# fraunhoferhhi/vvdec

Measured on NVIDIA H100. Metric: decoded frames/sec, 4K 10-bit Main10 RA, bit-exact YUV vs reference, higher is better.
Workload: dtype int16 samples / int32 accumulate

## Files before the change

include/vvdec_b200.h:

```cpp
#ifndef VVDEC_B200_H
#define VVDEC_B200_H
#include <stdint.h>
#include <stddef.h>

#ifdef __cplusplus
extern "C" {
#endif

#define B200_API __attribute__((visibility("default")))

enum {
  B200_OK            =  0,
  B200_ERR_CUDA      = -1,
  B200_ERR_PARAM     = -2,
  B200_ERR_NO_DEVICE = -3,
  B200_ERR_UNSUPPORTED = -4
};

B200_API const char* b200_last_error(void);
B200_API int         b200_device_count(void);
B200_API const char* b200_version(void);

enum { B200_TR_DCT2 = 0, B200_TR_DCT8 = 1, B200_TR_DST7 = 2 };
enum {
// ... 8 lines not shown
  uint16_t x, y;
  uint8_t  log2w, log2h;
  uint8_t  comp;
  uint8_t  flags;
  uint8_t  maxX, maxY;
  uint8_t  trType;
  uint8_t  lfnst;
  int8_t   ict;
  int8_t   rightShift;
  uint8_t  inBits;
  uint8_t  scale;
  uint32_t coefOff;
  uint32_t slOff;
  uint32_t rsv[2];
} b200_tu;

typedef struct b200_geom {
  int32_t width, height;
  int32_t chromaFormat;
  int32_t bitDepth;
  int32_t ctuSize;
  int32_t stride[3];
} b200_geom;

B200_API int b200_k1_residual(const b200_geom* g, int16_t* const planes[3],
                              const b200_tu* tus, size_t numTus,
                              const int16_t* coefs, size_t numCoefs,
                              const int32_t* scaling, size_t numScaling,
                              int mode);

typedef struct b200_lf_param {
  int8_t  qp[3];
  uint8_t bs;
  uint8_t sideMaxFiltLength;
  uint8_t flags;
} b200_lf_param;

typedef struct b200_lf_slice {
  int8_t  betaOffsetDiv2[3];
  int8_t  tcOffsetDiv2[3];
  uint8_t disable;
  uint8_t rsv;
} b200_lf_slice;

typedef struct b200_lf_seq {
  int32_t ladfEnabled, ladfNumIntervals;
  int32_t ladfQpOffset[5];
  int32_t ladfIntervalLowerBound[5];
} b200_lf_seq;

B200_API int b200_lf_deblock(const b200_geom* g, int16_t* const planes[3], const b200_lf_param* lfV, const b200_lf_param* lfH,
                             const uint8_t* ctuSlice, const b200_lf_slice* slices, int numSlices, const b200_lf_seq* seq, int dirs);

enum { B200_SAO_EO_0 = 0, B200_SAO_EO_90 = 1, B200_SAO_EO_135 = 2, B200_SAO_EO_45 = 3, B200_SAO_BO = 4, B200_SAO_OFF = 255 };
enum { B200_AVAIL_L = 1, B200_AVAIL_R = 2, B200_AVAIL_A = 4, B200_AVAIL_B = 8,
       B200_AVAIL_AL = 16, B200_AVAIL_AR = 32, B200_AVAIL_BL = 64, B200_AVAIL_BR = 128 };

typedef struct b200_sao_ctu {
  uint8_t type[3];
  uint8_t band[3];
  int8_t  offset[3][5];
  uint8_t avail;
  uint8_t rsv[2];
} b200_sao_ctu;

typedef struct b200_vb {
  int32_t numVer, numHor;
  int32_t posX[3], posY[3];
} b200_vb;

B200_API int b200_sao_picture(const b200_geom* g, const int16_t* const src[3], int16_t* const dst[3],
                              const b200_sao_ctu* ctus, const b200_vb* vb);

enum { B200_ALF_CLIP_TOP = 2, B200_ALF_CLIP_BOTTOM = 4, B200_ALF_CLIP_LEFT = 8, B200_ALF_CLIP_RIGHT = 16, B200_ALF_PAD_TL = 32, B200_ALF_PAD_BR = 64, B200_ALF_PAD_WIDE = 2 };
typedef struct b200_alf_ctu {
  uint8_t enable[3];
  uint8_t lumaSet;
  uint8_t chromaAlt[2];
  uint8_t ccIdx[2];
} b200_alf_ctu;

typedef struct b200_alf_tables {
  const int16_t* lumaCoeff;
  const int16_t* lumaClip;
  int32_t        numLumaSets;
  const int16_t* chromaCoeff;
  const int16_t* chromaClip;
  int32_t        numChromaAlts;
  const int16_t* ccCoeff[2];
  int32_t        numCc[2];
} b200_alf_tables;

B200_API int b200_alf_picture(const b200_geom* g, const int16_t* const src[3], int16_t* const dst[3],
                              const b200_alf_ctu* ctus, const b200_alf_tables* tabs);

enum {
  B200_PU_BDOF    = 1,
  B200_PU_DMVR    = 2,
  B200_PU_ALTHPEL = 4,
  B200_PU_AFFINE  = 8,
  B200_PU_AFFINE6 = 16,
  B200_PU_PROF0   = 32,
  B200_PU_PROF1   = 64,
  B200_PU_GEO     = 128
};

typedef struct b200_pu {
  uint16_t x, y;
  uint8_t  w, h;
  uint8_t  flags;
  int8_t   bcwW1;
  int8_t   refSlot[2];
  uint8_t  interDir;
  uint8_t  wpIdx;
  uint32_t dmvrOff;
  int32_t  mv[2][2];
  int32_t  cpmv[2][2][2];
} b200_pu;

typedef struct b200_wp {
  int16_t w0[3], w1[3];
  int16_t offset[3];
  uint8_t shift[3];
  uint8_t rsv[3];
} b200_wp;

B200_API int b200_mc_predict(const b200_geom* g, int16_t* const dst[3], const int16_t* const* refs, int numSlots,
                             const b200_pu* pus, size_t numPus, int32_t* dmvrMv, size_t numDmvr);
B200_API int b200_mc_predict_wp(const b200_geom* g, int16_t* const dst[3], const int16_t* const* refs, int numSlots,
                                const b200_pu* pus, size_t numPus, int32_t* dmvrMv, size_t numDmvr, const b200_wp* wp, int numWp);

enum { B200_INTRA_PLANAR = 0, B200_INTRA_DC = 1 , B200_INTRA_BDPCM_HOR = 67, B200_INTRA_BDPCM_VER = 68,
       B200_INTRA_MIP = 69 ,
       B200_INTRA_LM = 70, B200_INTRA_MDLM_L = 71, B200_INTRA_MDLM_T = 72  };
enum { B200_INTRA_FILTER_REF = 1, B200_INTRA_AVAIL_TL = 2, B200_INTRA_ADD_RESI = 4 ,
       B200_INTRA_LM_ABOVE = 8, B200_INTRA_LM_LEFT = 16 ,
       B200_INTRA_LM_COLLOCATED = 32 ,
       B200_INTRA_ISP = 64  };
typedef struct b200_intra_tu {
  uint16_t x, y;
  uint8_t  log2w, log2h;
  uint8_t  comp;
  uint8_t  mode;
  uint8_t  multiRefIdx;
  uint8_t  flags;
  uint8_t  numAbove;
  uint8_t  numLeft;
  uint8_t  mip;
  uint8_t  lmAbove, lmLeft;
  uint8_t  ciip;
} b200_intra_tu;
B200_API int b200_intra_predict(const b200_geom* g, int16_t* const planes[3], const b200_intra_tu* tus, size_t numTus);
B200_API int b200_intra_reconstruct(const b200_geom* g, int16_t* const planes[3], const int16_t* const resi[3], const b200_intra_tu* tus, size_t numTus);

typedef struct b200_ctx b200_ctx;

typedef struct b200_lmcs_vpdu { uint16_t x, y; uint8_t availLeft, availAbove; } b200_lmcs_vpdu;
typedef struct b200_lmcs {
  int32_t chromaAdj;
  int32_t minBinIdx, maxBinIdx;
  int32_t orgCW;
  int16_t reshapePivot[17];
  int16_t inputPivot[17];
  int16_t fwdScaleCoef[16];
  int32_t chromaAdjHelpLUT[16];
  const int16_t* invLUT;
  const b200_lmcs_vpdu* vpdus;
} b200_lmcs;

typedef struct b200_picture {
  int32_t dstSlot;
  int32_t flags;
  const int16_t* given[3];
  const b200_pu* pus; size_t numPus;
  size_t numDmvr;
  const b200_tu* tus; size_t numTus;
  const int16_t* coefs; size_t numCoefs;
  const int32_t* scaling; size_t numScaling;
  const b200_lf_param *lfV, *lfH;
  const uint8_t* ctuSlice; const b200_lf_slice* lfSlices; int32_t numLfSlices; const b200_lf_seq* lfSeq;
  const b200_sao_ctu* sao;
  const b200_vb* vb;
  const b200_alf_ctu* alf;
  const b200_alf_tables* alfTabs;
  const b200_wp* wp; int32_t numWp;
  const b200_lmcs* lmcs;
  const b200_intra_tu* intraTus;
  size_t numIntraTus;
} b200_picture;
enum { B200_PIC_DEBLOCK = 1, B200_PIC_SAO = 2, B200_PIC_ALF = 4, B200_PIC_LMCS = 8 };

B200_API int  b200_ctx_create(b200_ctx** ctx, const b200_geom* g, int numSlots, int numArenas, int device);
B200_API void b200_ctx_destroy(b200_ctx* ctx);
B200_API int  b200_ctx_load_slot(b200_ctx* ctx, int slot, const int16_t* const planes[3]);
B200_API int  b200_decompress_picture(b200_ctx* ctx, const b200_picture* pic);
B200_API int  b200_pic_upload(b200_ctx* ctx, const b200_picture* pic);
B200_API int  b200_pic_run(b200_ctx* ctx, int arena);
B200_API int  b200_wait_picture(b200_ctx* ctx, int arena, int32_t* dmvrMv, size_t numDmvr);
B200_API int  b200_get_frame(b200_ctx* ctx, int slot, int16_t* const planes[3]);
B200_API int  b200_ctx_load_slot_strided(b200_ctx* ctx, int slot, const int16_t* const planes[3], const ptrdiff_t strides[3]);
B200_API int  b200_get_frame_strided(b200_ctx* ctx, int slot, int16_t* const planes[3], const ptrdiff_t strides[3]);
B200_API int  b200_get_frame_async(b200_ctx* ctx, int slot, int16_t* const planes[3]);
B200_API int  b200_frame_wait(b200_ctx* ctx, int ticket);
B200_API int  b200_get_frame_device_async(b200_ctx* ctx, int slot, int16_t* const planesDev[3], void* cudaStream);
enum { B200_OUT_16 = 0, B200_OUT_PYUV = 1, B200_OUT_8 = 2 };
B200_API size_t b200_frame_bytes(const b200_geom* g, int fmt, int comp);
B200_API int  b200_get_frame_fmt_async(b200_ctx* ctx, int slot, int fmt, void* const planes[3]);
typedef struct b200_film_grain {
  const int8_t*   pattern;
  const uint8_t*  sLUT;
  const uint8_t*  pLUT;
  const uint32_t* lineSeeds;
  uint8_t         scaleShift;
  uint8_t         compPresent[3];
} b200_film_grain;
B200_API int  b200_get_frame_grain_async(b200_ctx* ctx, int slot, int fmt, void* const planes[3], const b200_film_grain* fg);
enum { B200_HASH_MD5 = 0, B200_HASH_CRC = 1, B200_HASH_CHECKSUM = 2 };
B200_API int  b200_frame_hash_async(b200_ctx* ctx, int slot, int method, uint8_t* digest);
B200_API int  b200_ctx_mark(b200_ctx* ctx, int which );
B200_API int  b200_ctx_elapsed_ms(b200_ctx* ctx, float* ms);
B200_API long long b200_ctx_kernel_launches(b200_ctx* ctx);
enum { B200_KF_MC_TILE = 0, B200_KF_MC_AFFINE, B200_KF_K1, B200_KF_LF_V, B200_KF_LF_H, B200_KF_SAO, B200_KF_ALF_LUMA, B200_KF_ALF_CHROMA,
       B200_KF_INTRA , B200_KF_LMCS , B200_KF_COUNT };
B200_API int  b200_ctx_set_profiling(b200_ctx* ctx, int on);
B200_API int  b200_ctx_get_kernel_ms(b200_ctx* ctx, float ms[8], int counts[8]);
B200_API int  b200_ctx_get_kernel_ms_n(b200_ctx* ctx, float* ms, int* counts, int n);
B200_API int  b200_host_register(void* ptr, size_t bytes);
B200_API int  b200_host_unregister(void* ptr);

#ifdef __cplusplus
}
#endif
#endif
```

vvdec_b200/bindings.py:

```python
import ctypes as C
import numpy as np
from . import abi

i16p = np.ctypeslib.ndpointer(np.int16, flags="C_CONTIGUOUS")
PLANES = C.POINTER(C.POINTER(C.c_int16))


def declare(lib):
    lib.b200_last_error.restype = C.c_char_p
    lib.b200_version.restype = C.c_char_p
    lib.b200_device_count.restype = C.c_int
    lib.b200_k1_residual.argtypes = [C.POINTER(abi.Geom), PLANES, C.c_void_p, C.c_size_t, C.c_void_p, C.c_size_t,
                                     C.c_void_p, C.c_size_t, C.c_int]
    lib.b200_k1_residual.restype = C.c_int


    lib.b200_lf_deblock.argtypes = [C.POINTER(abi.Geom), PLANES, C.c_void_p, C.c_void_p, C.c_void_p, C.c_void_p, C.c_int,
                                    C.c_void_p, C.c_int]
    lib.b200_lf_deblock.restype = C.c_int


    lib.b200_sao_picture.argtypes = [C.POINTER(abi.Geom), PLANES, PLANES, C.c_void_p, C.c_void_p]
    lib.b200_sao_picture.restype = C.c_int
    lib.b200_alf_picture.argtypes = [C.POINTER(abi.Geom), PLANES, PLANES, C.c_void_p, C.POINTER(abi.AlfTables)]
    lib.b200_alf_picture.restype = C.c_int


    lib.b200_mc_predict.argtypes = [C.POINTER(abi.Geom), PLANES, C.POINTER(C.c_void_p), C.c_int, C.c_void_p, C.c_size_t, C.c_void_p, C.c_size_t]
    lib.b200_mc_predict.restype = C.c_int
    lib.b200_mc_predict_wp.argtypes = [C.POINTER(abi.Geom), PLANES, C.POINTER(C.c_void_p), C.c_int, C.c_void_p, C.c_size_t, C.c_void_p, C.c_size_t, C.c_void_p, C.c_int]
    lib.b200_mc_predict_wp.restype = C.c_int


    CTX = C.c_void_p
    lib.b200_ctx_create.argtypes = [C.POINTER(CTX), C.POINTER(abi.Geom), C.c_int, C.c_int, C.c_int]
    lib.b200_ctx_destroy.argtypes = [CTX]; lib.b200_ctx_destroy.restype = None
    lib.b200_ctx_load_slot.argtypes = [CTX, C.c_int, PLANES]
    lib.b200_decompress_picture.argtypes = [CTX, C.POINTER(abi.Picture)]
    lib.b200_pic_upload.argtypes = [CTX, C.POINTER(abi.Picture)]
    lib.b200_pic_run.argtypes = [CTX, C.c_int]
    lib.b200_wait_picture.argtypes = [CTX, C.c_int, C.c_void_p, C.c_size_t]
    lib.b200_get_frame.argtypes = [CTX, C.c_int, PLANES]
    lib.b200_get_frame_async.argtypes = [CTX, C.c_int, PLANES]
    lib.b200_ctx_load_slot_strided.argtypes = [CTX, C.c_int, PLANES, C.POINTER(C.c_ssize_t)]
    lib.b200_get_frame_strided.argtypes = [CTX, C.c_int, PLANES, C.POINTER(C.c_ssize_t)]
    lib.b200_frame_wait.argtypes = [CTX, C.c_int]
    lib.b200_get_frame_device_async.argtypes = [CTX, C.c_int, C.POINTER(C.c_void_p), C.c_void_p]
    lib.b200_frame_bytes.argtypes = [C.POINTER(abi.Geom), C.c_int, C.c_int]; lib.b200_frame_bytes.restype = C.c_size_t
    lib.b200_get_frame_fmt_async.argtypes = [CTX, C.c_int, C.c_int, C.POINTER(C.c_void_p)]
    lib.b200_intra_predict.argtypes = [C.POINTER(abi.Geom), PLANES, C.c_void_p, C.c_size_t]
    lib.b200_intra_reconstruct.argtypes = [C.POINTER(abi.Geom), PLANES, PLANES, C.c_void_p, C.c_size_t]
    lib.b200_frame_hash_async.argtypes = [CTX, C.c_int, C.c_int, C.c_void_p]
    lib.b200_get_frame_grain_async.argtypes = [CTX, C.c_int, C.c_int, C.POINTER(C.c_void_p), C.POINTER(abi.FilmGrain)]
    lib.b200_ctx_mark.argtypes = [CTX, C.c_int]
    lib.b200_ctx_elapsed_ms.argtypes = [CTX, C.POINTER(C.c_float)]
    lib.b200_ctx_kernel_launches.argtypes = [CTX]; lib.b200_ctx_kernel_launches.restype = C.c_longlong
    lib.b200_ctx_set_profiling.argtypes = [CTX, C.c_int]
    lib.b200_ctx_get_kernel_ms.argtypes = [CTX, C.POINTER(C.c_float), C.POINTER(C.c_int)]
    lib.b200_ctx_get_kernel_ms_n.argtypes = [CTX, C.POINTER(C.c_float), C.POINTER(C.c_int), C.c_int]
    lib.b200_host_register.argtypes = [C.c_void_p, C.c_size_t]
    lib.b200_host_unregister.argtypes = [C.c_void_p]


EXPORTS = ["b200_ctx_create", "b200_ctx_destroy", "b200_ctx_load_slot", "b200_decompress_picture", "b200_pic_upload", "b200_pic_run",
           "b200_wait_picture", "b200_get_frame", "b200_ctx_load_slot_strided", "b200_get_frame_strided", "b200_get_frame_async", "b200_get_frame_device_async", "b200_frame_wait", "b200_frame_bytes", "b200_get_frame_fmt_async", "b200_frame_hash_async", "b200_intra_predict", "b200_intra_reconstruct", "b200_get_frame_grain_async", "b200_ctx_mark", "b200_ctx_elapsed_ms", "b200_ctx_kernel_launches", "b200_ctx_set_profiling", "b200_ctx_get_kernel_ms", "b200_ctx_get_kernel_ms_n", "b200_host_register", "b200_host_unregister",
           "b200_mc_predict", "b200_mc_predict_wp", "b200_last_error", "b200_version", "b200_device_count", "b200_k1_residual", "b200_lf_deblock",
           "b200_sao_picture", "b200_alf_picture"]
```

vvdec_b200/csrc/api.cu:

```cuda
#include "common.cuh"
#include <stdarg.h>
#include <string.h>
#include <mutex>

namespace b200 {

static thread_local char g_err[512] = "";

void set_error(const char* fmt, ...)
{
  va_list ap; va_start(ap, fmt);
  vsnprintf(g_err, sizeof(g_err), fmt, ap);
  va_end(ap);
}

int ensure_device()
{
  static std::once_flag once;
  static int status = 0;
  std::call_once(once, [] {
    int n = 0;
    if (cudaGetDeviceCount(&n) != cudaSuccess || n == 0) { set_error("no CUDA device: vvdec_b200 has no CPU fallback"); status = B200_ERR_NO_DEVICE; return; }
    int dev = 0; cudaGetDevice(&dev);
    cudaDeviceProp p; cudaGetDeviceProperties(&p, dev);
    if (p.major != 9 || p.minor != 0) { set_error("device %s is sm_%d%d; this library is built for sm_90a only", p.name, p.major, p.minor); status = B200_ERR_NO_DEVICE; }
  });
  if (status) set_error("no usable sm_90 device: vvdec_b200 has no CPU fallback");
  return status;
}

struct HostWrapScratch {
  DevBuf planes[3], tus, coefs, scaling, misc[8];
  cudaStream_t stream = nullptr;
  int init() { if (!stream) { B200_CUDA(cudaStreamCreateWithFlags(&stream, cudaStreamNonBlocking)); } return 0; }
};
static HostWrapScratch g_hw;
HostWrapScratch& host_scratch() { return g_hw; }

static int upload_planes(const b200_geom* g, int16_t* const planes[3], DevPlanes& dp, cudaStream_t s)
{
  const int nPlanes = g->chromaFormat ? 3 : 1;
  for (int c = 0; c < nPlanes; c++) {
    const int ph = c ? g->height >> 1 : g->height;
    const size_t bytes = (size_t)g->stride[c] * ph * sizeof(int16_t);
    if (int rc = g_hw.planes[c].reserve(bytes)) return rc;
    dp.p[c] = g_hw.planes[c].as<int16_t>(); dp.stride[c] = g->stride[c];
    B200_CUDA(cudaMemcpyAsync(dp.p[c], planes[c], bytes, cudaMemcpyHostToDevice, s));
  }
  return 0;
}
static int download_planes(const b200_geom* g, int16_t* const planes[3], const DevPlanes& dp, cudaStream_t s)
{
  const int nPlanes = g->chromaFormat ? 3 : 1;
  for (int c = 0; c < nPlanes; c++) {
    const int ph = c ? g->height >> 1 : g->height;
    B200_CUDA(cudaMemcpyAsync(planes[c], dp.p[c], (size_t)g->stride[c] * ph * sizeof(int16_t), cudaMemcpyDeviceToHost, s));
  }
  return 0;
}

int num_sms()
{
  static int cache[64] = {0};
  int dev = 0; cudaGetDevice(&dev);
  if (dev < 0 || dev >= 64) dev = 0;
  if (!cache[dev]) { int n = 0; if (cudaDeviceGetAttribute(&n, cudaDevAttrMultiProcessorCount, dev) != cudaSuccess || n <= 0) n = 132; cache[dev] = n; }
  return cache[dev];
}

int fetch_list_meta(const int* metaDev, int* cnt, int nLists, const char* what, cudaStream_t s)
{
  int h[LM_INTS];
  B200_CUDA(cudaMemcpyAsync(h, metaDev, sizeof(h), cudaMemcpyDeviceToHost, s));
  B200_CUDA(cudaStreamSynchronize(s));
  for (int i = 0; i < nLists; i++) cnt[i] = h[LM_CNT + i];
  B200_CHECK(!(h[LM_ERR] & 1), "%s: invalid record (reference slots, block size or flag combination)", what);
  B200_CHECK(!(h[LM_ERR] & 2), "%s: more tiles than the picture can hold (overlapping PUs?)", what);
  return 0;
}

}

using namespace b200;

extern "C" {

B200_API const char* b200_last_error(void) { return g_err; }
B200_API const char* b200_version(void) { return "vvdec_b200 0.1 (sm_90a)"; }
B200_API int b200_device_count(void) { int n = 0; return cudaGetDeviceCount(&n) == cudaSuccess ? n : 0; }

B200_API int b200_k1_residual(const b200_geom* g, int16_t* const planes[3], const b200_tu* tus, size_t numTus,
                              const int16_t* coefs, size_t numCoefs, const int32_t* scaling, size_t numScaling, int mode)
{
  B200_CHECK(g && planes && (tus || !numTus), "b200_k1_residual: null argument");
  B200_CHECK(g->bitDepth >= 8 && g->bitDepth <= 12, "b200_k1_residual: bit depth %d unsupported", g->bitDepth);
  if (int rc = ensure_device()) return rc;
  if (int rc = g_hw.init()) return rc;
  cudaStream_t s = g_hw.stream;
  K1Launch L; L.geom = *g; L.numTus = numTus; L.mode = mode;
  if (int rc = upload_planes(g, planes, L.planes, s)) return rc;
  if (int rc = g_hw.tus.reserve(numTus * sizeof(b200_tu))) return rc;
  if (int rc = g_hw.coefs.reserve(numCoefs * sizeof(int16_t) + 16)) return rc;
  if (int rc = g_hw.scaling.reserve(numScaling * sizeof(int32_t) + 16)) return rc;
  if (int rc = g_hw.misc[4].reserve(numTus * 4 + LM_INTS * sizeof(int) + 256)) return rc;
  if (numTus) B200_CUDA(cudaMemcpyAsync(g_hw.tus.p, tus, numTus * sizeof(b200_tu), cudaMemcpyHostToDevice, s));
  if (numCoefs) B200_CUDA(cudaMemcpyAsync(g_hw.coefs.p, coefs, numCoefs * sizeof(int16_t), cudaMemcpyHostToDevice, s));
  if (numScaling) B200_CUDA(cudaMemcpyAsync(g_hw.scaling.p, scaling, numScaling * sizeof(int32_t), cudaMemcpyHostToDevice, s));
  L.tus = g_hw.tus.as<b200_tu>(); L.coefs = g_hw.coefs.as<int16_t>(); L.scaling = g_hw.scaling.as<int32_t>();
  int* meta = g_hw.misc[4].as<int>(); uint32_t* idx = reinterpret_cast<uint32_t*>(meta + LM_INTS);
  if (int rc = launch_tu_bucket(L.tus, numTus, idx, meta, *g, numCoefs, numScaling, s)) return rc;
  L.idx = idx; L.meta = meta;
  if (int rc = fetch_list_meta(meta, L.cnt, K1_LISTS, "b200_k1_residual", s)) return rc;
  StreamSet ss(s);
  if (int rc = launch_k1_residual(L, ss)) return rc;
  if (int rc = download_planes(g, planes, L.planes, s)) return rc;
  B200_CUDA(cudaStreamSynchronize(s));
  return 0;
}

B200_API int b200_lf_deblock(const b200_geom* g, int16_t* const planes[3], const b200_lf_param* lfV, const b200_lf_param* lfH,
                             const uint8_t* ctuSlice, const b200_lf_slice* slices, int numSlices, const b200_lf_seq* seq, int dirs)
{
  B200_CHECK(g && planes && lfV && lfH && slices, "b200_lf_deblock: null argument");
  B200_CHECK(numSlices >= 1 && numSlices <= 64, "b200_lf_deblock: numSlices %d out of range 1..64", numSlices);
  B200_CHECK(g->ctuSize == 32 || g->ctuSize == 64 || g->ctuSize == 128, "b200_lf_deblock: CTU size %d", g->ctuSize);
  if (int rc = ensure_device()) return rc;
  if (int rc = g_hw.init()) return rc;
  cudaStream_t s = g_hw.stream;
  LfLaunch L; L.geom = *g; L.dirs = dirs;
  memset(&L.slices, 0, sizeof(L.slices)); memcpy(L.slices.s, slices, numSlices * sizeof(b200_lf_slice));
  if (seq) L.seq = *seq; else memset(&L.seq, 0, sizeof(L.seq));
  if (int rc = upload_planes(g, planes, L.planes, s)) return rc;
  const size_t n4 = (size_t)((g->width + 3) >> 2) * ((g->height + 3) >> 2);
  const size_t nCtu = (size_t)((g->width + g->ctuSize - 1) / g->ctuSize) * ((g->height + g->ctuSize - 1) / g->ctuSize);
  if (int rc = g_hw.misc[0].reserve(n4 * sizeof(b200_lf_param))) return rc;
  if (int rc = g_hw.misc[1].reserve(n4 * sizeof(b200_lf_param))) return rc;
  if (int rc = g_hw.misc[2].reserve(nCtu)) return rc;
  B200_CUDA(cudaMemcpyAsync(g_hw.misc[0].p, lfV, n4 * sizeof(b200_lf_param), cudaMemcpyHostToDevice, s));
  B200_CUDA(cudaMemcpyAsync(g_hw.misc[1].p, lfH, n4 * sizeof(b200_lf_param), cudaMemcpyHostToDevice, s));
  if (ctuSlice) B200_CUDA(cudaMemcpyAsync(g_hw.misc[2].p, ctuSlice, nCtu, cudaMemcpyHostToDevice, s));
  L.lfV = g_hw.misc[0].as<b200_lf_param>(); L.lfH = g_hw.misc[1].as<b200_lf_param>();
  L.ctuSlice = ctuSlice ? g_hw.misc[2].as<uint8_t>() : nullptr;
  if (int rc = launch_lf_deblock(L, s)) return rc;
  if (int rc = download_planes(g, planes, L.planes, s)) return rc;
  B200_CUDA(cudaStreamSynchronize(s));
  return 0;
}

static int upload_src_alloc_dst(const b200_geom* g, const int16_t* const src[3], DevPlanes& ds, DevPlanes& dd, cudaStream_t s)
{
  const int nPlanes = g->chromaFormat ? 3 : 1;
  for (int c = 0; c < nPlanes; c++) {
    const int ph = c ? g->height >> 1 : g->height;
    const size_t bytes = (size_t)g->stride[c] * ph * sizeof(int16_t);
    if (int rc = g_hw.planes[c].reserve(bytes)) return rc;
    if (int rc = g_hw.misc[3 + c].reserve(bytes)) return rc;
    ds.p[c] = g_hw.planes[c].as<int16_t>(); dd.p[c] = g_hw.misc[3 + c].as<int16_t>(); ds.stride[c] = dd.stride[c] = g->stride[c];
    B200_CUDA(cudaMemcpyAsync(ds.p[c], src[c], bytes, cudaMemcpyHostToDevice, s));
  }
  return 0;
}

B200_API int b200_sao_picture(const b200_geom* g, const int16_t* const src[3], int16_t* const dst[3], const b200_sao_ctu* ctus, const b200_vb* vb)
{
  B200_CHECK(g && src && dst && ctus, "b200_sao_picture: null argument");
  B200_CHECK((g->width & 7) == 0 && (g->stride[0] & 3) == 0 && (!g->chromaFormat || (g->stride[1] & 3) == 0), "b200_sao_picture: width must be a multiple of 8, strides of 4");
  if (int rc = ensure_device()) return rc;
  if (int rc = g_hw.init()) return rc;
  cudaStream_t s = g_hw.stream;
  SaoLaunch L; L.geom = *g;
  if (vb) L.vb = *vb; else memset(&L.vb, 0, sizeof(L.vb));
  if (int rc = upload_src_alloc_dst(g, src, L.src, L.dst, s)) return rc;
  const size_t nCtu = (size_t)((g->width + g->ctuSize - 1) / g->ctuSize) * ((g->height + g->ctuSize - 1) / g->ctuSize);
  if (int rc = g_hw.misc[0].reserve(nCtu * sizeof(b200_sao_ctu))) return rc;
  B200_CUDA(cudaMemcpyAsync(g_hw.misc[0].p, ctus, nCtu * sizeof(b200_sao_ctu), cudaMemcpyHostToDevice, s));
  L.ctus = g_hw.misc[0].as<b200_sao_ctu>();
  if (int rc = launch_sao(L, s)) return rc;
  if (int rc = download_planes(g, dst, L.dst, s)) return rc;
  B200_CUDA(cudaStreamSynchronize(s));
  return 0;
}

B200_API int b200_intra_reconstruct(const b200_geom* g, int16_t* const planes[3], const int16_t* const resi[3], const b200_intra_tu* tus, size_t numTus)
{
  B200_CHECK(g && planes && (tus || !numTus), "b200_intra_reconstruct: null argument");
  B200_CHECK(g->bitDepth >= 8 && g->bitDepth <= 12, "b200_intra_reconstruct: bit depth %d unsupported", g->bitDepth);
  const int nPl = g->chromaFormat ? 3 : 1;
  for (size_t i = 0; i < numTus; i++) {
    const b200_intra_tu& t = tus[i];
    const int w = 1 << t.log2w, h = 1 << t.log2h, pw = t.comp ? g->width >> 1 : g->width, ph = t.comp ? g->height >> 1 : g->height, unit = t.comp ? 2 : 4;
    const bool inCtu = intra_record_in_ctu(t, intra_ctu_log2(*g));
    if (t.flags & B200_INTRA_ISP) {
      B200_CHECK(intra_isp_record_ok(t, i ? &tus[i - 1] : nullptr, g->width, g->height), "b200_intra_reconstruct: record %zu: bad ISP region", i);
      B200_CHECK(inCtu, "b200_intra_reconstruct: intra block record %zu is not inside one CTU", i);
      continue;
    }
    B200_CHECK(t.comp < nPl && t.log2w >= 2 && t.log2w <= 6 && t.log2h >= 1 && t.log2h <= 6 && t.x + w <= pw && t.y + h <= ph && !(t.x % unit) && !(t.y % unit),
               "b200_intra_reconstruct: record %zu: bad geometry", i);
    B200_CHECK(inCtu, "b200_intra_reconstruct: intra block record %zu is not inside one CTU", i);
    B200_CHECK(t.mode <= B200_INTRA_MDLM_T && t.multiRefIdx <= 2 && (!t.multiRefIdx || !t.comp), "b200_intra_reconstruct: record %zu: bad mode / reference line", i);
    B200_CHECK(!t.ciip || (t.ciip <= 3 && t.mode == B200_INTRA_PLANAR), "b200_intra_reconstruct: record %zu: bad CIIP block", i);
    B200_CHECK(t.mode < B200_INTRA_LM || (t.comp && t.log2w <= 5 && t.log2h <= 5 && t.lmAbove <= w && t.lmLeft <= h && (!(t.flags & B200_INTRA_LM_ABOVE) || t.y >= 2) && (!(t.flags & B200_INTRA_LM_LEFT) || t.x >= 2)
                                        && t.x + std::max(w, 2 * (int)t.lmAbove) <= pw && t.y + std::max(h, 2 * (int)t.lmLeft) <= ph), "b200_intra_reconstruct: record %zu: bad CCLM block", i);
    B200_CHECK(t.mode != B200_INTRA_MIP || (!t.comp && !t.multiRefIdx && (t.mip & 0x7f) < ((w == 4 && h == 4) ? 16 : (w == 4 || h == 4 || (w == 8 && h == 8)) ? 8 : 6)),
               "b200_intra_reconstruct: record %zu: bad MIP mode", i);
    B200_CHECK(t.numAbove <= 2 * w / unit && t.numLeft <= 2 * h / unit && (!t.numAbove || t.y > t.multiRefIdx) && (!t.numLeft || t.x > t.multiRefIdx)
               && (!(t.flags & B200_INTRA_AVAIL_TL) || (t.x > t.multiRefIdx && t.y > t.multiRefIdx)) && t.x + (int)t.numAbove * unit <= pw && t.y + (int)t.numLeft * unit <= ph,
               "b200_intra_reconstruct: record %zu: availability outside the picture", i);
  }
  if (int rc = ensure_device()) return rc;
  if (int rc = g_hw.init()) return rc;
  cudaStream_t s = g_hw.stream;
  IntraLaunch L; L.geom = *g; L.numTus = numTus;
  if (int rc = upload_planes(g, planes, L.planes, s)) return rc;
  for (int c = 0; c < 3; c++) {
    L.resi[c] = nullptr; L.owner[c] = nullptr; L.ownerStride[c] = 0; L.ownerBytes[c] = 0;
    if (c >= nPl) continue;
    const int pw = c ? g->width >> 1 : g->width, ph = c ? g->height >> 1 : g->height, unit = c ? 2 : 4;
    L.ownerStride[c] = (pw + unit - 1) / unit; L.ownerBytes[c] = (size_t)L.ownerStride[c] * ((ph + unit - 1) / unit) * sizeof(int);
    if (int rc = g_hw.misc[c].reserve(L.ownerBytes[c])) return rc;
    L.owner[c] = g_hw.misc[c].as<int>();
    if (resi && resi[c]) {
      const size_t bytes = (size_t)g->stride[c] * ph * sizeof(int16_t);
      if (int rc = g_hw.misc[3 + c].reserve(bytes)) return rc;
      B200_CUDA(cudaMemcpyAsync(g_hw.misc[3 + c].p, resi[c], bytes, cudaMemcpyHostToDevice, s));
      L.resi[c] = g_hw.misc[3 + c].as<int16_t>();
    }
  }
  if (int rc = g_hw.tus.reserve(numTus * sizeof(b200_intra_tu) + 16)) return rc;
  if (int rc = g_hw.misc[6].reserve((numTus + 2) * sizeof(int))) return rc;
  if (int rc = g_hw.misc[7].reserve(intra_order_ints(*g, numTus) * sizeof(int))) return rc;
  if (numTus) B200_CUDA(cudaMemcpyAsync(g_hw.tus.p, tus, numTus * sizeof(b200_intra_tu), cudaMemcpyHostToDevice, s));
  L.tus = g_hw.tus.as<b200_intra_tu>(); L.sync = g_hw.misc[6].as<int>(); L.order = g_hw.misc[7].as<int>();
  if (int rc = launch_intra(L, s)) return rc;
  int err = 0;
  if (numTus) B200_CUDA(cudaMemcpyAsync(&err, L.sync + numTus + 1, sizeof(int), cudaMemcpyDeviceToHost, s));
  if (int rc = download_planes(g, planes, L.planes, s)) return rc;
  B200_CUDA(cudaStreamSynchronize(s));
  B200_CHECK(!(err & INTRA_ERR_CTU_BLOCKS), "b200_intra_reconstruct: a CTU holds more than %d intra block records (overlapping records?)", INTRA_MAX_CTU_BLOCKS);
  B200_CHECK(!err, "b200_intra_reconstruct: a block waited for a neighbour that never finished, or the blocks of a CTU are not contiguous (list not in decoding order?)");
  return 0;
}

B200_API int b200_intra_predict(const b200_geom* g, int16_t* const planes[3], const b200_intra_tu* tus, size_t numTus)
{
  return b200_intra_reconstruct(g, planes, nullptr, tus, numTus);
}

B200_API int b200_alf_picture(const b200_geom* g, const int16_t* const src[3], int16_t* const dst[3], const b200_alf_ctu* ctus, const b200_alf_tables* T)
{
  B200_CHECK(g && src && dst && ctus && T, "b200_alf_picture: null argument");
  B200_CHECK((g->width & 7) == 0 && (g->stride[0] & 3) == 0 && (!g->chromaFormat || (g->stride[1] & 3) == 0), "b200_alf_picture: width must be a multiple of 8, strides of 4");
  B200_CHECK(T->numLumaSets >= 16 && T->numLumaSets <= 24, "b200_alf_picture: numLumaSets %d", T->numLumaSets);
  if (int rc = ensure_device()) return rc;
  if (int rc = g_hw.init()) return rc;
  cudaStream_t s = g_hw.stream;
  AlfLaunch L; L.geom = *g;
  if (int rc = upload_src_alloc_dst(g, src, L.src, L.dst, s)) return rc;
  const size_t nCtu = (size_t)((g->width + g->ctuSize - 1) / g->ctuSize) * ((g->height + g->ctuSize - 1) / g->ctuSize);
  const size_t nL = (size_t)T->numLumaSets * 1300, nC = (size_t)T->numChromaAlts * 7, n0 = (size_t)T->numCc[0] * 7, n1 = (size_t)T->numCc[1] * 7;
  const size_t tabElems = 2 * nL + 2 * nC + n0 + n1 + 8;
  if (int rc = g_hw.misc[0].reserve(nCtu * sizeof(b200_alf_ctu))) return rc;
  if (int rc = g_hw.misc[1].reserve(tabElems * sizeof(int16_t))) return rc;
  B200_CUDA(cudaMemcpyAsync(g_hw.misc[0].p, ctus, nCtu * sizeof(b200_alf_ctu), cudaMemcpyHostToDevice, s));
  int16_t* d = g_hw.misc[1].as<int16_t>();
  auto up = [&](const int16_t* h, size_t n, const int16_t*& out) -> int {
    out = d; if (n) B200_CUDA(cudaMemcpyAsync(d, h, n * sizeof(int16_t), cudaMemcpyHostToDevice, s)); d += n; return 0; };
  if (int rc = up(T->lumaCoeff, nL, L.lumaCoeff)) return rc;
  if (int rc = up(T->lumaClip, nL, L.lumaClip)) return rc;
  if (int rc = up(T->chromaCoeff, nC, L.chromaCoeff)) return rc;
  if (int rc = up(T->chromaClip, nC, L.chromaClip)) return rc;
  if (int rc = up(T->ccCoeff[0], n0, L.cc[0])) return rc;
  if (int rc = up(T->ccCoeff[1], n1, L.cc[1])) return rc;
  L.ctus = g_hw.misc[0].as<b200_alf_ctu>();
  StreamSet ss(s);
  if (int rc = launch_alf(L, ss)) return rc;
  if (int rc = download_planes(g, dst, L.dst, s)) return rc;
  B200_CUDA(cudaStreamSynchronize(s));
  return 0;
}

B200_API int b200_mc_predict(const b200_geom* g, int16_t* const dst[3], const int16_t* const* refs, int numSlots,
                             const b200_pu* pus, size_t numPus, int32_t* dmvrMv, size_t numDmvr)
{
  return b200_mc_predict_wp(g, dst, refs, numSlots, pus, numPus, dmvrMv, numDmvr, nullptr, 0);
}

B200_API int b200_mc_predict_wp(const b200_geom* g, int16_t* const dst[3], const int16_t* const* refs, int numSlots,
                                const b200_pu* pus, size_t numPus, int32_t* dmvrMv, size_t numDmvr, const b200_wp* wp, int numWp)
{
  B200_CHECK(g && dst && refs && (pus || !numPus), "b200_mc_predict: null argument");
  B200_CHECK(numSlots >= 1 && numSlots <= B200_MAX_SLOTS, "b200_mc_predict: numSlots %d", numSlots);
  B200_CHECK(numPus < (1u << 26), "b200_mc_predict: too many PUs");
  for (size_t i = 0; i < numPus; i++) {
    B200_CHECK(pus[i].refSlot[0] < numSlots && pus[i].refSlot[1] < numSlots && (pus[i].refSlot[0] >= 0 || pus[i].refSlot[1] >= 0), "b200_mc_predict: PU %zu has invalid reference slots", i);
    B200_CHECK(!((pus[i].flags & B200_PU_DMVR) && g->bitDepth > 10), "b200_mc_predict: DMVR needs bit depth <= 10 (as the reference)");
  }
  if (int rc = ensure_device()) return rc;
  if (int rc = g_hw.init()) return rc;
  cudaStream_t s = g_hw.stream;
  McLaunch L; L.geom = *g;
  if (int rc = upload_planes(g, dst, L.dst, s)) return rc;
  const int nPlanes = g->chromaFormat ? 3 : 1;
  size_t planeBytes[3] = {0, 0, 0}, total = 0;
  for (int c = 0; c < nPlanes; c++) { planeBytes[c] = (((size_t)g->stride[c] * (c ? g->height >> 1 : g->height) * 2) + 255) & ~(size_t)255; total += planeBytes[c]; }
  if (int rc = g_hw.misc[3].reserve(total * numSlots)) return rc;
  std::vector<const int16_t*> ptrs(numSlots * 3, nullptr);
  char* base = g_hw.misc[3].as<char>();
  for (int sl = 0; sl < numSlots; sl++) {
    size_t off = 0;
    for (int c = 0; c < nPlanes; c++) {
      char* d = base + (size_t)sl * total + off;
      B200_CUDA(cudaMemcpyAsync(d, refs[sl * 3 + c], (size_t)g->stride[c] * (c ? g->height >> 1 : g->height) * 2, cudaMemcpyHostToDevice, s));
      ptrs[sl * 3 + c] = reinterpret_cast<const int16_t*>(d); off += planeBytes[c];
    }
  }
  const size_t capTiles = mc_tile_capacity(*g, numPus);
  if (int rc = g_hw.misc[5].reserve(numPus * sizeof(b200_pu) + 64)) return rc;
  if (int rc = g_hw.misc[6].reserve(capTiles * 4 + LM_INTS * sizeof(int) + 256)) return rc;
  if (int rc = g_hw.misc[7].reserve(numDmvr * 8 + 64)) return rc;
  if (numPus) B200_CUDA(cudaMemcpyAsync(g_hw.misc[5].p, pus, numPus * sizeof(b200_pu), cudaMemcpyHostToDevice, s));
  int* meta = g_hw.misc[6].as<int>(); uint32_t* tiles = reinterpret_cast<uint32_t*>(meta + LM_INTS);
  if (int rc = launch_mc_bucket(g_hw.misc[5].as<b200_pu>(), numPus, tiles, capTiles, meta, *g, numSlots, wp ? numWp : 0, numDmvr, s)) return rc;
  L.tiles = tiles; L.meta = meta;
  if (wp && numWp > 0) {
    B200_CHECK(numWp <= 255, "b200_mc_predict_wp: at most 255 weighted-prediction entries");
    if (int rc = g_hw.misc[2].reserve(numWp * sizeof(b200_wp))) return rc;
    B200_CUDA(cudaMemcpyAsync(g_hw.misc[2].p, wp, numWp * sizeof(b200_wp), cudaMemcpyHostToDevice, s));
    L.wp = g_hw.misc[2].as<b200_wp>();
  }
  if (int rc = fetch_list_meta(meta, L.cnt, MC_LISTS, "b200_mc_predict", s)) return rc;
  B200_CUDA(cudaMemsetAsync(g_hw.misc[7].p, 0, numDmvr * 8 + 64, s));
  memset(L.refs, 0, sizeof(L.refs)); for (size_t i = 0; i < ptrs.size(); i++) L.refs[i] = ptrs[i];
  for (int c = 0; c < 3; c++) L.refStride[c] = g->stride[c];
  L.pus = g_hw.misc[5].as<b200_pu>(); L.dmvrMv = dmvrMv ? g_hw.misc[7].as<int32_t>() : nullptr;
  StreamSet ss(s);
  if (int rc = launch_mc(L, ss)) return rc;
  if (int rc = download_planes(g, dst, L.dst, s)) return rc;
  if (dmvrMv && numDmvr) B200_CUDA(cudaMemcpyAsync(dmvrMv, g_hw.misc[7].p, numDmvr * 8, cudaMemcpyDeviceToHost, s));
  B200_CUDA(cudaStreamSynchronize(s));
  return 0;
}

}
```

vvdec_b200/csrc/common.cuh:

```cuda
#pragma once
#include <cuda_runtime.h>
#include <stdint.h>
#include <stdio.h>
#include <string>
#include <vector>
#include <algorithm>
#include "../../include/vvdec_b200.h"

namespace b200 {

void set_error(const char* fmt, ...);

#define B200_CUDA(call)                                                                         \
  do {                                                                                          \
    cudaError_t e_ = (call);                                                                    \
    if (e_ != cudaSuccess) {                                                                    \
      b200::set_error("%s:%d %s -> %s", __FILE__, __LINE__, #call, cudaGetErrorString(e_));     \
      (void)cudaGetLastError();                                                                 \
      return B200_ERR_CUDA;                                                                     \
    }                                                                                           \
  } while (0)

#define B200_CHECK(cond, ...)                                    \
  do {                                                           \
    if (!(cond)) { b200::set_error(__VA_ARGS__); return B200_ERR_PARAM; } \
  } while (0)

__device__ __forceinline__ int clip3(int lo, int hi, int v) { return min(max(v, lo), hi); }
__device__ __forceinline__ int clip16(int v) { return min(max(v, -32768), 32767); }

__device__ __forceinline__ int lmcs_fwd(const b200_lmcs* __restrict__ L, int log2OrgCW, int v, int pmax)
{
  const int idx = v >> log2OrgCW;
  return clip3(0, pmax, (int)__ldg(&L->reshapePivot[idx]) + (((int)__ldg(&L->fwdScaleCoef[idx]) * (v - (int)__ldg(&L->inputPivot[idx])) + (1 << 10)) >> 11));
}
__device__ __forceinline__ int lmcs_scale(int r, int scale, int maxAbs)
{
  r = clip3(-maxAbs - 1, maxAbs, r);
  const int a = abs(r), v = (a * scale + (1 << 10)) >> 11;
  return clip16(r >= 0 ? v : -v);
}

struct DevBuf {
  void*  p   = nullptr;
  size_t cap = 0;
  int reserve(size_t bytes) {
    if (bytes <= cap) return 0;
    if (p) cudaFree(p);
    p = nullptr; cap = 0;
    size_t want = bytes + (bytes >> 2) + 256;
    cudaError_t e = cudaMalloc(&p, want);
    if (e != cudaSuccess) { set_error("cudaMalloc(%zu) -> %s", want, cudaGetErrorString(e)); return B200_ERR_CUDA; }
    cap = want;
    return 0;
  }
  template <class T> T* as() const { return reinterpret_cast<T*>(p); }
  ~DevBuf() { if (p) cudaFree(p); }
};

struct DevPlanes {
  int16_t* p[3] = {nullptr, nullptr, nullptr};
  int      stride[3] = {0, 0, 0};
};

struct KProf { virtual void begin(int family, cudaStream_t s) = 0; virtual void end(int family, cudaStream_t s) = 0; virtual ~KProf() {} };

struct StreamSet {
  cudaStream_t main = nullptr; cudaStream_t aux[4] = {nullptr, nullptr, nullptr, nullptr}; int nAux = 0;
  cudaEvent_t forkEv = nullptr, joinEv[4] = {nullptr, nullptr, nullptr, nullptr};
  bool used[4] = {false, false, false, false};
  StreamSet() {}
  explicit StreamSet(cudaStream_t s) : main(s) {}
  cudaStream_t pick(int i) {
    if (nAux == 0) return main;
    const int k = i % (nAux + 1);
    if (k == nAux) return main;
    if (!used[k]) { cudaEventRecord(forkEv, main); cudaStreamWaitEvent(aux[k], forkEv, 0); used[k] = true; }
    return aux[k];
  }
  void join() { for (int k = 0; k < nAux; k++) if (used[k]) { cudaEventRecord(joinEv[k], aux[k]); cudaStreamWaitEvent(main, joinEv[k], 0); used[k] = false; } }
};

constexpr int MC_LISTS = 17;
constexpr int K1_LISTS = 4;
constexpr int LM_CNT = 0, LM_OFF = 32, LM_CUR = 64, LM_DONE = 96, LM_ERR = 97, LM_INTS = 128;
int launch_mc_bucket(const b200_pu* pus, size_t numPus, uint32_t* tiles, size_t capTiles, int* meta, const b200_geom& g, int numSlots, int numWp, size_t numDmvr, cudaStream_t s);
int launch_tu_bucket(const b200_tu* tus, size_t numTus, uint32_t* idx, int* meta, const b200_geom& g, size_t numCoefs, size_t numScaling, cudaStream_t s);
struct CtuLimits { int numLumaSets, numChromaAlts, numCc[2], numLfSlices; };
int launch_ctu_validate(const b200_sao_ctu* sao, const b200_alf_ctu* alf, const uint8_t* ctuSlice, int nCtu, const CtuLimits& lim, int* meta, cudaStream_t s);
size_t mc_tile_capacity(const b200_geom& g, size_t numPus);
int num_sms();
int fetch_list_meta(const int* metaDev, int* cnt, int nLists, const char* what, cudaStream_t s);

struct K1Launch {
  b200_geom      geom;
  DevPlanes      planes;
  const b200_tu* tus;
  size_t         numTus;
  const uint32_t* idx;
  const int*     meta;
  int            cnt[K1_LISTS];
  const int16_t* coefs;
  const int32_t* scaling;
  int            mode;
  int            compSel = 0;
  const int*     vpduScale = nullptr;
  int16_t*       resi[3] = {nullptr, nullptr, nullptr};
};
int launch_k1_residual(const K1Launch& L, StreamSet& ss, KProf* prof = nullptr);

struct LfSliceTab { b200_lf_slice s[64]; };
struct LfLaunch {
  b200_geom geom; DevPlanes planes;
  const b200_lf_param *lfV, *lfH;
  const uint8_t* ctuSlice;
  LfSliceTab slices; b200_lf_seq seq; int dirs;
};
int launch_lf_deblock(const LfLaunch& L, cudaStream_t s, KProf* prof = nullptr);

struct SaoLaunch { b200_geom geom; DevPlanes src, dst; const b200_sao_ctu* ctus; b200_vb vb; };
int launch_sao(const SaoLaunch& L, cudaStream_t s, KProf* prof = nullptr);

struct AlfLaunch {
  b200_geom geom; DevPlanes src, dst; const b200_alf_ctu* ctus;
  const int16_t *lumaCoeff, *lumaClip, *chromaCoeff, *chromaClip, *cc[2];
};
int launch_alf(const AlfLaunch& L, StreamSet& ss, KProf* prof = nullptr);

constexpr int B200_MAX_SLOTS = 32;
struct McLaunch {
  b200_geom geom; DevPlanes dst;
  const int16_t* refs[B200_MAX_SLOTS * 3];
  int refStride[3];
  const b200_pu* pus;
  const uint32_t* tiles;
  const int* meta;
  int cnt[MC_LISTS];
  int32_t* dmvrMv;
  const b200_wp* wp = nullptr;
  const b200_lmcs* lmcs = nullptr;
  const void* tmaps = nullptr; uint8_t tmapBuf[B200_MAX_SLOTS] = {};
};
int make_mc_tensor_maps(const b200_geom& g, int16_t* const* bufPlanes , int nBufs, void** out);
int launch_mc(const McLaunch& L, StreamSet& ss, KProf* prof = nullptr);
int mc_launch_count(const McLaunch& L);
int k1_launch_count(const K1Launch& L);

struct LmcsLaunch { b200_geom geom; DevPlanes planes; const b200_lmcs* lmcs; const b200_lmcs_vpdu* vpdus; const int16_t* invLut; int* scale; };
int launch_lmcs_vpdu(const LmcsLaunch& L, cudaStream_t s);
int launch_lmcs_inv(const LmcsLaunch& L, cudaStream_t s);

int launch_pack(const DevPlanes& src, const b200_geom& g, int fmt, uint8_t* const dst[3], cudaStream_t s);

struct IntraLaunch { b200_geom geom; DevPlanes planes; const int16_t* resi[3]; const b200_intra_tu* tus; size_t numTus; int* owner[3]; int ownerStride[3]; size_t ownerBytes[3]; int* sync;
                     int* order = nullptr;
                     int compSel = 0;
                   };
inline size_t intra_order_ints(const b200_geom& g, size_t numTus) { return numTus + 8 + 3 * (size_t)((g.width + g.ctuSize - 1) / g.ctuSize) * ((g.height + g.ctuSize - 1) / g.ctuSize); }
inline int intra_ctu_log2(const b200_geom& g) { return g.ctuSize == 128 ? 7 : g.ctuSize == 64 ? 6 : 5; }
__host__ __device__ inline bool intra_record_in_ctu(const b200_intra_tu& t, int ctuLog2)
{
  const int cl = ctuLog2 - (t.comp ? 1 : 0);
  return (t.x >> cl) == ((t.x + (1 << t.log2w) - 1) >> cl) && (t.y >> cl) == ((t.y + (1 << t.log2h) - 1) >> cl);
}
__host__ __device__ inline bool intra_isp_record_ok(const b200_intra_tu& t, const b200_intra_tu* prev, int W, int H)
{
  const int sp = t.mip & 3, k = (t.mip >> 2) & 3, l2n = (t.mip >> 4) & 3, nReg = 1 << l2n, rw = 1 << t.log2w, rh = 1 << t.log2h;
  if (t.comp || t.mode > 66 || t.multiRefIdx || (sp != 1 && sp != 2) || l2n > 2 || (l2n == 0 && (sp != 2 || rw != 4))  || k >= nReg || (t.mip >> 6) || t.log2w < 2 || t.log2w > 6 || t.log2h > 6) return false;
  const int cw = sp == 2 ? rw * nReg : rw, ch = sp == 1 ? rh * nReg : rh, cx = t.x - (sp == 2 ? k * rw : 0), cy = t.y - (sp == 1 ? k * rh : 0);
  if (cw > 64 || ch > 64 || ch < 4 || cw * ch < 32 || cx < 0 || cy < 0 || (cx & 3) || (cy & 3) || cx + cw > W || cy + ch > H) return false;
  if (t.numAbove > 2 * cw / 4 || t.numLeft > 2 * ch / 4 || (t.numAbove && !cy) || (t.numLeft && !cx) || ((t.flags & B200_INTRA_AVAIL_TL) && (!cx || !cy))
      || cx + (int)t.numAbove * 4 > W || cy + (int)t.numLeft * 4 > H || (t.lmLeft && !cx) || (t.lmAbove && !cy)) return false;
  if (k) {
    if (!prev || !(prev->flags & B200_INTRA_ISP) || prev->mip != (uint8_t)(t.mip - 4) || prev->log2w != t.log2w || prev->log2h != t.log2h || prev->mode != t.mode
        || prev->x != t.x - (sp == 2 ? rw : 0) || prev->y != t.y - (sp == 1 ? rh : 0)) return false;
  }
  return true;
}
int launch_intra(const IntraLaunch& L, cudaStream_t s);
int launch_intra_ciip_clear(const b200_intra_tu* tus, size_t numTus, int16_t* const resi[3], const int stride[3], cudaStream_t s);
int launch_intra_validate(const b200_intra_tu* tus, size_t numTus, const b200_geom& g, int* meta, cudaStream_t s);
constexpr int INTRA_ERR_ORDER = 2, INTRA_ERR_CTU_BLOCKS = 4, INTRA_MAX_CTU_BLOCKS = 3072;
int launch_film_grain(const DevPlanes& src, const DevPlanes& dst, const b200_geom& g, const int8_t* pattern, const uint8_t* sLUT, const uint8_t* pLUT,
                      const uint32_t* lineSeeds, uint32_t* seeds, int scaleShift, const uint8_t present[3], cudaStream_t s);
int launch_hash(const DevPlanes& src, const b200_geom& g, int method, uint32_t* acc, uint8_t* digest, cudaStream_t s);

int ensure_device();

}
```

vvdec_b200/csrc/k6_intra.cu:

```cuda
#include "common.cuh"
#include <stdlib.h>
#include <string.h>
#define VVC_TABLE_QUAL static __device__ const __align__(16)
#include "vvc_tables.h"

namespace b200 {

constexpr int IT_THREADS = 128;
constexpr int IT_REF = 2 * 64 + 8;
constexpr int IT_ORG = 72;
constexpr int IT_ARR = IT_ORG + 2 * 64 + 80;

__constant__ int cAng[32] = {0, 1, 2, 3, 4, 6, 8, 10, 12, 14, 16, 18, 20, 23, 26, 29, 32, 35, 39, 45, 51, 57, 64, 73, 86, 102, 128, 171, 256, 341, 512, 1024};
__constant__ int cInvAng[32] = {0, 16384, 8192, 5461, 4096, 2731, 2048, 1638, 1365, 1170, 1024, 910, 819, 712, 630, 565,
                                512, 468, 420, 364, 321, 287, 256, 224, 191, 161, 128, 96, 64, 48, 32, 16};
__constant__ int cIntraFilterThr[8] = {24, 24, 24, 14, 2, 0, 0, 0};

struct IntraParams {
  int16_t* planes[3]; const int16_t* resi[3]; int stride[3]; int W, H, bitDepth;
  const b200_intra_tu* tus; int numTus;
  int* owner[3]; int ownerStride[3];
  int* done; int* ticket; int* err;
  const int* perm;
  int* ctuCnt; int* ctuFirst; int* ctuBase; int ctuLog2, ctusW, ctusH;
  int compSel;
};

__device__ __forceinline__ int wide_angle(int w, int h, int mode)
{
  if (mode > 1 && mode <= 66) {
    const int d = abs((31 - __clz(w)) - (31 - __clz(h)));
    const int shift = (int)((0x0F0E0C0A0600ull >> (8 * d)) & 0xff);
    if (w > h && mode < 2 + shift) mode += 65;
    else if (h > w && mode > 66 - shift) mode -= 65;
  }
  return mode;
}

__global__ void __launch_bounds__(256) intra_owner_kernel(const IntraParams P)
{
  const int i = blockIdx.x;
  const b200_intra_tu t = P.tus[i];
  const int c = t.comp, unit = c ? 2 : 4, uw = max(1, (1 << t.log2w) / unit), uh = max(1, (1 << t.log2h) / unit);
  for (int k = threadIdx.x; k < uw * uh; k += blockDim.x) atomicMax(&P.owner[c][(t.y / unit + k / uw) * P.ownerStride[c] + t.x / unit + k % uw], i);
}

__device__ __forceinline__ int intra_ctu_of(const IntraParams& P, const b200_intra_tu& t)
{
  const int sh = t.comp ? 1 : 0;
  return (((int)t.y << sh) >> P.ctuLog2) * P.ctusW + (((int)t.x << sh) >> P.ctuLog2);
}
__global__ void __launch_bounds__(256) intra_ctu_count_kernel(const IntraParams P)
{
  const int i = blockIdx.x * 256 + threadIdx.x;
  if (i >= P.numTus) return;
  const int c = intra_ctu_of(P, P.tus[i]);
  atomicAdd(&P.ctuCnt[c], 1); atomicMin(&P.ctuFirst[c], i);
}
__global__ void intra_ctu_base_kernel(const IntraParams P)
{
  int run = 0;
  for (int d = 0; d < P.ctusW + 2 * P.ctusH; d++)
    for (int y = 0; y < P.ctusH; y++) { const int x = d - 2 * y; if (x >= 0 && x < P.ctusW) { P.ctuBase[y * P.ctusW + x] = run; run += P.ctuCnt[y * P.ctusW + x]; } }
}
__global__ void __launch_bounds__(256) intra_perm_kernel(const IntraParams P, int* perm)
{
  const int i = blockIdx.x * 256 + threadIdx.x;
  if (i >= P.numTus) return;
  const int c = intra_ctu_of(P, P.tus[i]), r = i - P.ctuFirst[c];
  if (r >= P.ctuCnt[c]) { atomicOr(P.err, 2); return; }
  perm[P.ctuBase[c] + r] = i;
}

__device__ __forceinline__ int pix(const int16_t* __restrict__ plane, int stride, int x, int y) { return __ldcg(plane + (size_t)y * stride + x); }

#define ISP_GEOMETRY \
    const bool isp = t.flags & B200_INTRA_ISP; \
    int bx = x0, by = y0, bw = w, bh = h, ispK = 0, ispSplit = 0, resiMask = 0xff, l2tu = 16; \
    if (isp) { \
      ispSplit = t.mip & 3; ispK = (t.mip >> 2) & 3; const int nReg_ = 1 << ((t.mip >> 4) & 3); \
      if (ispSplit == 1) { bh = h * nReg_; by = y0 - ispK * h; } else { bw = w * nReg_; bx = x0 - ispK * w; } \
      int tuW_ = w; if (ispSplit == 2 && (bw == 4 || (bw == 8 && bh > 4))) tuW_ = max(bw >> 2, bh < 16 ? 16 / bh : 1);       \
      l2tu = 31 - __clz(tuW_); resiMask = t.ciip; \
    } \
    const int topLen = isp ? bw + w : 2 * w, sideLen = isp ? bh + h : 2 * h;

#define ISP_REFERENCE_LAMBDAS \
    auto refT = [&](int j) -> int {                               \
      if (n == 0) return 1 << (P.bitDepth - 1); \
      if (n == totalUnits) return PIXR(bx - 1 - mrl + j, by - 1 - mrl); \
      if (j <= mrl) {                                             \
        if (numLeft > 0) return availTL ? PIXR(bx - 1 - mrl + j, by - 1 - mrl) : PIXR(bx - 1 - mrl, by); \
        return PIXR(bx, by - 1 - mrl); \
      } \
      if (numAbove) return PIXR(bx + min(j - 1 - mrl, aboveLen - 1), by - 1 - mrl); \
      return availTL ? PIXR(bx - 1, by - 1 - mrl) : PIXR(bx - 1 - mrl, by);       \
    }; \
    auto refL = [&](int i) -> int {                               \
      if (n == 0) return 1 << (P.bitDepth - 1); \
      if (n == totalUnits) return PIXR(bx - 1 - mrl, by - 1 - mrl + i); \
      if (numLeft > 0) { \
        if (i <= mrl) return availTL ? PIXR(bx - 1 - mrl, by - 1 - mrl + i) : PIXR(bx - 1 - mrl, by); \
        return PIXR(bx - 1 - mrl, by + min(i - 1 - mrl, leftLen - 1)); \
      } \
      return PIXR(bx, by - 1 - mrl); \
    }; \
    auto regT = [&](int j) -> int { \
      if (!ispK) return refT(j); \
      if (ispSplit == 1) return j == 0 ? (t.lmLeft ? refL(y0 - by) : PIXR(x0, y0 - 1)) : PIXR(x0 + min(j - 1, w - 1), y0 - 1); \
      return t.lmAbove ? refT(x0 - bx + j) : PIXR(x0 - 1, y0); \
    }; \
    auto regL = [&](int i) -> int { \
      if (!ispK) return refL(i); \
      if (ispSplit == 1) return t.lmLeft ? refL(y0 - by + i) : PIXR(x0, y0 - 1); \
      return PIXR(x0 - 1, y0 + min(i - 1, h - 1)); \
    };

__global__ void __launch_bounds__(IT_THREADS, 12) intra_kernel(const IntraParams P)
{
  __shared__ int16_t sT[2][IT_REF], sL[2][IT_REF];
  __shared__ int16_t sM[IT_ARR], sS[IT_ARR];
  __shared__ int sTicket, sSum;
  __shared__ int16_t sLm[32 * 32], sLmTop[64], sLmLeft[64];
  __shared__ int sLmPar[3];
  const int tid = threadIdx.x;
  for (;;) {
    __syncthreads();
    if (tid == 0) { sTicket = atomicAdd(P.ticket, 1); sSum = 0; }
    __syncthreads();
    if (sTicket >= P.numTus) return;
    if (P.perm && (*(volatile int*)P.err & 2)) return;
    const int me = P.perm ? P.perm[sTicket] : sTicket;
    const b200_intra_tu t = P.tus[me];
    if ((P.compSel == 1 && t.comp != 0) || (P.compSel == 2 && t.comp == 0)) continue;
    const int c = t.comp, w = 1 << t.log2w, h = 1 << t.log2h, mrl = c ? 0 : t.multiRefIdx, unit = c ? 2 : 4;
    const int x0 = t.x, y0 = t.y, ps = P.stride[c], pmax = (1 << P.bitDepth) - 1;
    const int16_t* plane = P.planes[c];
    const int availTL = (t.flags & B200_INTRA_AVAIL_TL) ? 1 : 0, numAbove = t.numAbove, numLeft = t.numLeft;
    ISP_GEOMETRY

    {
      if (ispK && tid == 0) {
        const volatile int* d = P.done + me - 1; const volatile int* e = P.err; int spins = 0;
        while (*d == 0) { __nanosleep(64); if (*e || ++spins > (1 << 22)) { atomicOr(P.err, 1); break; } }
      }
      for (int dep = tid; dep < 96; dep += IT_THREADS) {
      int ux = -1, uy = -1;
      if (dep == 0) { if (availTL) { ux = bx - 1; uy = by - 1; } }
      else if (dep <= numAbove) { ux = bx + (dep - 1) * unit; uy = by - 1; }
      else if (dep - 64 >= 0 && dep - 64 < numLeft) { ux = bx - 1; uy = by + (dep - 64) * unit; }
      if (ux >= 0 && uy >= 0) {
        const int o = P.owner[c][(uy / unit) * P.ownerStride[c] + ux / unit];
        if (o >= 0 && o < me) {
          const volatile int* d = P.done + o;
          int spins = 0;
          const volatile int* e = P.err;
          while (*d == 0) { __nanosleep(64); if (*e || ++spins > (1 << 22)) { atomicOr(P.err, 1); break; } }
        }
      }
      }
      if (t.mode >= B200_INTRA_LM) {
        const bool aCu = t.flags & B200_INTRA_LM_ABOVE, lCu = t.flags & B200_INTRA_LM_LEFT;
        const int nA = max(w, aCu ? (t.mode == B200_INTRA_MDLM_T ? 2 * t.lmAbove : w) : 0), nL = max(h, lCu ? (t.mode == B200_INTRA_MDLM_L ? 2 * t.lmLeft : h) : 0);
        const int ux0 = max(0, (2 * x0 - (lCu ? 4 : 0)) >> 2), ux1 = min(P.W - 1, 2 * x0 + 2 * nA - 1) >> 2;
        const int uy0 = max(0, (2 * y0 - (aCu ? 4 : 0)) >> 2), uy1 = min(P.H - 1, 2 * y0 + 2 * nL - 1) >> 2;
        const int uw = ux1 - ux0 + 1, nU = uw * (uy1 - uy0 + 1);
        for (int u = tid; u < nU; u += IT_THREADS) {
          const int o = P.owner[0][(uy0 + u / uw) * P.ownerStride[0] + ux0 + u % uw];
          if (o >= 0 && o < me) {
            const volatile int* d = P.done + o; const volatile int* e = P.err;
            int spins = 0;
            while (*d == 0) { __nanosleep(64); if (*e || ++spins > (1 << 22)) { atomicOr(P.err, 1); break; } }
          }
        }
      }
      __threadfence();
    }
    __syncthreads();

    const int predSize = 2 * bw, predHSize = 2 * bh;
    const int totalUnits = (predSize + unit - 1) / unit + (predHSize + unit - 1) / unit + 1, n = availTL + numAbove + numLeft;
    const int aboveLen = min(numAbove * unit, predSize), leftLen = min(numLeft * unit, predHSize);
    int16_t *T = sT[0], *L = sL[0];
#define PIXR(x, y) pix(plane, ps, (x), (y))
    ISP_REFERENCE_LAMBDAS
    for (int j = tid; j <= topLen + mrl; j += IT_THREADS) T[j] = (int16_t)regT(j);
    for (int i = tid + 1; i <= sideLen + mrl; i += IT_THREADS) L[i] = (int16_t)regL(i);
#undef PIXR
    __syncthreads();
    if (tid == 0) L[0] = T[0];
    __syncthreads();
    if ((t.flags & B200_INTRA_FILTER_REF) && !c && !mrl) {
      int16_t *FT = sT[1], *FL = sL[1];
      for (int j = tid; j <= predSize; j += IT_THREADS)
        FT[j] = j == 0 ? (int16_t)((L[1] + 2 * T[0] + T[1] + 2) >> 2) : j == predSize ? T[j] : (int16_t)((T[j + 1] + 2 * T[j] + T[j - 1] + 2) >> 2);
      for (int i = tid + 1; i <= predHSize; i += IT_THREADS)
        FL[i] = i == predHSize ? L[i] : (int16_t)((L[i + 1] + 2 * L[i] + L[i - 1] + 2) >> 2);
      __syncthreads();
      if (tid == 0) FL[0] = FT[0];
      T = FT; L = FL;
      __syncthreads();
    }

    const int mode = t.mode;
    const bool doPDPC = w >= 4 && h >= 4 && mrl == 0;
    int16_t* dst = P.planes[c] + (size_t)y0 * ps + x0;
    const int16_t* rs = (P.resi[c] && (t.flags & B200_INTRA_ADD_RESI)) ? P.resi[c] + (size_t)y0 * ps + x0 : nullptr;
    const int ciipW = isp ? 0 : t.ciip;
#define IT_STORE(x, y, v) do { int v_ = (v); int16_t* d_ = dst + (size_t)(y) * ps + (x); if (ciipW) v_ = ((4 - ciipW) * (int)*d_ + ciipW * v_ + 2) >> 2; \
                               if (rs && ((resiMask >> ((x) >> l2tu)) & 1)) v_ = clip3(0, pmax, v_ + rs[(size_t)(y) * ps + (x)]); *d_ = (int16_t)v_; } while (0)

    if (mode == B200_INTRA_PLANAR || mode == B200_INTRA_DC) {
      int dc = 0;
      if (mode == B200_INTRA_DC) {
        int part = 0;
        for (int i = tid; i < w + h; i += IT_THREADS) {
          if (i < w) { if (w >= h) part += T[mrl + 1 + i]; }
          else if (w <= h) part += L[mrl + 1 + i - w];
        }
        for (int o = 16; o; o >>= 1) part += __shfl_down_sync(0xffffffffu, part, o);
        if ((tid & 31) == 0) atomicAdd(&sSum, part);
        __syncthreads();
        const int denom = w == h ? w << 1 : max(w, h);
        dc = (sSum + (denom >> 1)) >> (31 - __clz(denom));
      }
      const int l2w = t.log2w, l2h = t.log2h, scale = (l2w - 2 + l2h - 2 + 2) >> 2;
      const int bl = L[h + 1], tr = T[w + 1];
      for (int k = tid; k < w * h; k += IT_THREADS) {
        const int y = k >> l2w, x = k & (w - 1);
        int v;
        if (mode == B200_INTRA_PLANAR) {
          const int hor = (L[y + 1] << l2w) + (x + 1) * (tr - L[y + 1]), vert = (T[x + 1] << l2h) + (y + 1) * (bl - T[x + 1]);
          v = ((hor << l2h) + (vert << l2w) + (1 << (l2w + l2h))) >> (1 + l2w + l2h);
        } else v = dc;
        v = (int16_t)v;
        if (doPDPC) {
          const int wT = 32 >> min(31, (y << 1) >> scale), wL = 32 >> min(31, (x << 1) >> scale);
          v = (int16_t)(v + ((wL * (L[y + 1] - v) + wT * (T[x + 1] - v) + 32) >> 6));
        }
        IT_STORE(x, y, v);
      }
    } else if (mode >= B200_INTRA_LM) {
      const bool aCu = t.flags & B200_INTRA_LM_ABOVE, lCu = t.flags & B200_INTRA_LM_LEFT, colloc = t.flags & B200_INTRA_LM_COLLOCATED;
      const int ls = P.stride[0];
      const int16_t* rec = P.planes[0] + (size_t)(2 * y0) * ls + 2 * x0;
      const bool firstRowOfCtu = ((2 * y0) & ((1 << P.ctuLog2) - 1)) == 0;
      const int nTop = aCu ? (mode == B200_INTRA_MDLM_T ? 2 * t.lmAbove : w) : 0, nLeft = lCu ? (mode == B200_INTRA_MDLM_L ? 2 * t.lmLeft : h) : 0;
#define LUMA(p_, o_) ((int)__ldcg((p_) + (o_)))
      for (int k = tid; k < nTop + nLeft + w * h; k += IT_THREADS) {
        if (k < nTop) {
          const int i = k, m = (i == 0 && !lCu) ? 0 : 1;
          int v;
          if (firstRowOfCtu) { const int16_t* p = rec - ls; v = (LUMA(p, 2 * i) * 2 + LUMA(p, 2 * i - m) + LUMA(p, 2 * i + 1) + 2) >> 2; }
          else if (colloc) { const int16_t* p = rec - 2 * ls; v = (LUMA(p, 2 * i - ls) + LUMA(p, 2 * i) * 4 + LUMA(p, 2 * i - m) + LUMA(p, 2 * i + 1) + LUMA(p, 2 * i + ls) + 4) >> 3; }
          else { const int16_t* p = rec - 2 * ls; v = (LUMA(p, 2 * i) * 2 + LUMA(p, 2 * i - m) + LUMA(p, 2 * i + 1) + LUMA(p, 2 * i + ls) * 2 + LUMA(p, 2 * i - m + ls) + LUMA(p, 2 * i + 1 + ls) + 4) >> 3; }
          sLmTop[i] = (int16_t)v;
        } else if (k < nTop + nLeft) {
          const int j = k - nTop; const int16_t* p = rec - 3 + (size_t)(2 * j) * ls;
          int v;
          if (colloc) v = (LUMA(p, 1 - ((j == 0 && !aCu) ? 0 : ls)) + LUMA(p, 1) * 4 + LUMA(p, 0) + LUMA(p, 2) + LUMA(p, 1 + ls) + 4) >> 3;
          else v = (LUMA(p, 1) * 2 + LUMA(p, 0) + LUMA(p, 2) + LUMA(p, 1 + ls) * 2 + LUMA(p, ls) + LUMA(p, 2 + ls) + 4) >> 3;
          sLmLeft[j] = (int16_t)v;
        } else {
          const int q = k - nTop - nLeft, j = q >> t.log2w, i = q & (w - 1), m = (i == 0 && !lCu) ? 0 : 1;
          const int16_t* p = rec + (size_t)(2 * j) * ls;
          int v;
          if (colloc) { const int up = (j == 0 && !aCu) ? 0 : ls; v = (LUMA(p, 2 * i - up) + LUMA(p, 2 * i) * 4 + LUMA(p, 2 * i - m) + LUMA(p, 2 * i + 1) + LUMA(p, 2 * i + ls) + 4) >> 3; }
          else v = (LUMA(p, 2 * i) * 2 + LUMA(p, 2 * i + 1) + LUMA(p, 2 * i - m) + LUMA(p, 2 * i + ls) * 2 + LUMA(p, 2 * i + 1 + ls) + LUMA(p, 2 * i - m + ls) + 4) >> 3;
          sLm[q] = (int16_t)v;
        }
      }
#undef LUMA
      __syncthreads();
      if (tid == 0) {
        const int tuWU = w >> 1, tuHU = h >> 1;
        bool aboveAvail = false, leftAvail = false; int topNum = 0, leftNum = 0;
        if (mode == B200_INTRA_MDLM_T) { aboveAvail = t.lmAbove >= tuWU; topNum = 2 * t.lmAbove; }
        else if (mode == B200_INTRA_MDLM_L) { leftAvail = t.lmLeft >= tuHU; leftNum = 2 * t.lmLeft; }
        else { aboveAvail = aCu; leftAvail = lCu; topNum = w; leftNum = h; }
        const int aboveIs4 = leftAvail ? 0 : 1, leftIs4 = aboveAvail ? 0 : 1;
        const int start0 = topNum >> (2 + aboveIs4), step0 = max(1, topNum >> (1 + aboveIs4)), start1 = leftNum >> (2 + leftIs4), step1 = max(1, leftNum >> (1 + leftIs4));
        int sl[4] = {0, 0, 0, 0}, sc[4] = {0, 0, 0, 0}, cntT = 0, cntL = 0;
        if (aboveAvail) { cntT = min(topNum, (1 + aboveIs4) << 1); for (int k = 0, pos = start0; k < cntT; k++, pos += step0) { sl[k] = sLmTop[pos]; sc[k] = T[1 + pos]; } }
        if (leftAvail) { cntL = min(leftNum, (1 + leftIs4) << 1); for (int k = 0, pos = start1; k < cntL; k++, pos += step1) { sl[k + cntT] = sLmLeft[pos]; sc[k + cntT] = L[1 + pos]; } }
        if (cntT + cntL == 2) { sl[3] = sl[0]; sc[3] = sc[0]; sl[2] = sl[1]; sc[2] = sc[1]; sl[0] = sl[1]; sc[0] = sc[1]; sl[1] = sl[3]; sc[1] = sc[3]; }
        int mn0 = 0, mn1 = 2, mx0 = 1, mx1 = 3, tt;
        if (sl[mn0] > sl[mn1]) { tt = mn0; mn0 = mn1; mn1 = tt; }
        if (sl[mx0] > sl[mx1]) { tt = mx0; mx0 = mx1; mx1 = tt; }
        if (sl[mn0] > sl[mx1]) { tt = mn0; mn0 = mx0; mx0 = tt; tt = mn1; mn1 = mx1; mx1 = tt; }
        if (sl[mn1] > sl[mx0]) { tt = mn1; mn1 = mx0; mx0 = tt; }
        const int minL = (sl[mn0] + sl[mn1] + 1) >> 1, minC = (sc[mn0] + sc[mn1] + 1) >> 1, maxL = (sl[mx0] + sl[mx1] + 1) >> 1, maxC = (sc[mx0] + sc[mx1] + 1) >> 1;
        int a = 0, b = 1 << (P.bitDepth - 1), shift = 0;
        if (leftAvail || aboveAvail) {
          const int diff = maxL - minL;
          if (diff > 0) {
            const int diffC = maxC - minC;
            int x = 31 - __clz(diff);
            const int normDiff = (diff << 4 >> x) & 15;
            const int v = (int)((0x0765544332211110ull >> (4 * (15 - normDiff))) & 15) | 8;
            x += normDiff != 0;
            const int y = diffC == 0 ? 0 : (31 - __clz(abs(diffC))) + 1, add = 1 << y >> 1;
            a = (diffC * v + add) >> y; shift = 3 + x - y;
            if (shift < 1) { shift = 1; a = a == 0 ? 0 : a < 0 ? -15 : 15; }
            b = minC - ((a * minL) >> shift);
          } else { a = 0; b = minC; shift = 0; }
        }
        sLmPar[0] = a; sLmPar[1] = b; sLmPar[2] = shift;
      }
      __syncthreads();
      const int a = sLmPar[0], b = sLmPar[1], shift = sLmPar[2];
      for (int k = tid; k < w * h; k += IT_THREADS) { const int y = k >> t.log2w, x = k & (w - 1); IT_STORE(x, y, clip3(0, pmax, ((a * sLm[k]) >> shift) + b)); }
    } else if (mode == B200_INTRA_MIP) {
      const int sizeId = (w == 4 && h == 4) ? 0 : (w == 4 || h == 4 || (w == 8 && h == 8)) ? 1 : 2;
      const int bdry = sizeId == 0 ? 2 : 4, red = sizeId < 2 ? 4 : 8, upH = w / red, upV = h / red, inSize = 2 * bdry;
      const int modeIdx = t.mip & 0x7f; const bool transpose = t.mip >> 7;
      int16_t* in = sS;
      if (tid < inSize) {
        const bool fromLeft = (tid >= bdry) != transpose; const int d = tid % bdry, len = fromLeft ? h : w;
        const int16_t* full = (fromLeft ? L : T) + 1;
        int v;
        if (bdry < len) { const int f = len / bdry; int sum = 0; for (int j = 0; j < f; j++) sum += full[d * f + j]; v = (sum + (f >> 1)) >> (31 - __clz(f)); }
        else v = full[d];
        in[tid] = (int16_t)v;
      }
      __syncthreads();
      const int inputOffset = in[0];
      __syncthreads();
      if (tid < inSize) in[tid] = (int16_t)(tid == 0 ? (sizeId < 2 ? (1 << (P.bitDepth - 1)) - inputOffset : 0) : in[tid] - inputOffset);
      __syncthreads();
      if (tid < red * red) {
        const int redSize = sizeId == 2, stride = inSize - redSize;
        const uint8_t* wgt = (sizeId == 0 ? kMip4x4 + modeIdx * 64 : sizeId == 1 ? kMip8x8 + modeIdx * 128 : kMip16x16 + modeIdx * 448) + tid * stride;
        int sum = 0, acc = 0;
        for (int i = 0; i < inSize; i++) sum += in[i];
        for (int i = redSize; i < inSize; i++) acc += in[i] * wgt[i - redSize];
        const int v = clip3(0, pmax, ((acc + 32 - 32 * sum) >> 6) + inputOffset);
        sM[transpose ? (tid % red) * red + tid / red : tid] = (int16_t)v;
      }
      __syncthreads();
      const int l2H = 31 - __clz(upH), l2V = 31 - __clz(upV);
      for (int k = tid; k < w * h; k += IT_THREADS) {
        const int y = k >> t.log2w, x = k & (w - 1), kr = y / upV, i = y % upV;
        int hv[2];
#pragma unroll
        for (int q = 0; q < 2; q++) {
          const int kk = kr - 1 + q;
          if (kk < 0) hv[q] = T[x + 1];
          else if (upH == 1) hv[q] = sM[kk * red + x];
          else {
            const int j = x / upH, ii = x % upH, before = j == 0 ? L[(kk + 1) * upV] : sM[kk * red + j - 1], behind = sM[kk * red + j];
            hv[q] = (int16_t)(before * upH + (upH >> 1) + (ii + 1) * (behind - before)) >> l2H;
          }
        }
        IT_STORE(x, y, upV == 1 ? hv[1] : (int16_t)(hv[0] * upV + (upV >> 1) + (i + 1) * (hv[1] - hv[0])) >> l2V);
      }
    } else if (mode >= B200_INTRA_BDPCM_HOR) {
      for (int k = tid; k < w * h; k += IT_THREADS) { const int y = k >> t.log2w, x = k & (w - 1); IT_STORE(x, y, mode == B200_INTRA_BDPCM_HOR ? L[y + 1] : T[x + 1]); }
    } else {
      const int predMode = wide_angle(bw, bh, mode);
      const bool ver = predMode >= 34;
      const int angMode = ver ? predMode - 50 : -(predMode - 18), absMode = abs(angMode);
      const int invAngle = cInvAng[absMode], absAng = cAng[absMode], angle = angMode < 0 ? -absAng : absAng;
      const int16_t *mainSrc = ver ? T : L, *sideSrc = ver ? L : T;
      const int mw = ver ? w : h, mh = ver ? h : w;
      int16_t *M = sM + IT_ORG, *S = sS + IT_ORG;
      if (angle < 0) {
        for (int k = tid - mh; k <= mw + 1 + mrl; k += IT_THREADS) M[k] = k >= 0 ? mainSrc[k] : sideSrc[min((-k * invAngle + 256) >> 9, mh)];
        for (int k = tid; k <= mh + 1 + mrl; k += IT_THREADS) S[k] = sideSrc[k];
      } else {
        const int l2r = (31 - __clz(mw)) - (31 - __clz(mh)), s = max(0, l2r), maxIndex = (mrl << s) + 2, refLength = ver ? topLen : sideLen;
        for (int k = tid; k <= refLength + mrl + maxIndex; k += IT_THREADS) M[k] = mainSrc[min(k, refLength + mrl)];
        for (int k = tid; k <= (ver ? sideLen : topLen) + mrl; k += IT_THREADS) S[k] = sideSrc[k];
      }
      __syncthreads();
      const int16_t *Mp = M + mrl, *Sp = S + mrl;
      const int l2mw = 31 - __clz(mw), l2mh = 31 - __clz(mh);
      const int topLeft = T[0];
      const int scale0 = (l2mw - 2 + l2mh - 2 + 2) >> 2;
      const int lev = min(3 << scale0, mw);
      const bool frac = (absAng & 31) != 0;
      const int diff = min(abs(predMode - 18), abs(predMode - 50));
      const bool cubic = isp || !(diff > cIntraFilterThr[(l2mw + l2mh) >> 1]) || mrl > 0;
      int angularScale = -1;
      if (angle > 0 && doPDPC) angularScale = min(2, l2mh - ((31 - __clz(3 * invAngle - 2)) - 8));
      for (int k = tid; k < mw * mh; k += IT_THREADS) {
        const int yy = k >> l2mw, xx = k & (mw - 1);
        int v;
        if (angle == 0) {
          if (doPDPC && xx < lev) { const int wL = 32 >> min(31, (xx << 1) >> scale0); v = clip3(0, pmax, (wL * (Sp[yy + 1] - topLeft) + Mp[xx + 1] * 64 + 32) >> 6); }
          else v = Mp[xx + 1];
        } else {
          const int deltaPos = angle * (1 + mrl + yy), dI = deltaPos >> 5, dF = deltaPos & 31;
          if (!frac) v = Mp[dI + 1 + xx];
          else if (c) v = (int16_t)(((32 - dF) * Mp[dI + 1 + xx] + dF * Mp[dI + 2 + xx] + 16) >> 5);
          else {
            const int16_t* p = Mp + dI + xx;
            int f0, f1, f2, f3;
            if (cubic) { f0 = kIfChroma[dF * 4]; f1 = kIfChroma[dF * 4 + 1]; f2 = kIfChroma[dF * 4 + 2]; f3 = kIfChroma[dF * 4 + 3]; }
            else { f0 = 16 - (dF >> 1); f1 = 32 - (dF >> 1); f2 = 16 + (dF >> 1); f3 = dF >> 1; }
            v = (int16_t)((f0 * p[0] + f1 * p[1] + f2 * p[2] + f3 * p[3] + 32) >> 6);
            if (cubic) v = clip3(0, pmax, v);
          }
          if (angularScale >= 0 && xx < min(3 << angularScale, mw)) {
            const int invAngleSum = 256 + (xx + 1) * invAngle, wL = 32 >> (2 * xx >> angularScale), left = Sp[yy + (invAngleSum >> 9) + 1];
            v = (int16_t)(v + ((wL * (left - v) + 32) >> 6));
          }
        }
        if (ver) IT_STORE(xx, yy, v); else IT_STORE(yy, xx, v);
      }
    }
#undef IT_STORE
    __threadfence();
    __syncthreads();
    if (tid == 0) atomicExch(P.done + me, 1);
  }
}


constexpr int V2_LS = 136, V2_CS = 72;
constexpr int V2_TILE = 128 * V2_LS + 2 * 64 * V2_CS;
constexpr int V2_RECS = 1024;
constexpr int V2_FLAGS = 128 * 128 / 16 + 2 * (64 * 64 / 4);
static_assert(V2_FLAGS == INTRA_MAX_CTU_BLOCKS, "the documented per-CTU block limit is the number of done bytes");
struct V2Scratch { int16_t T[2][IT_REF], L[2][IT_REF], M[IT_ARR], S[IT_ARR], Lm[32 * 32], LmTop[64], LmLeft[64]; int LmPar[4]; int next[2], sum; };
constexpr int V2_OWN = 3 * 32 * 32;
constexpr size_t v2_smem(int groups) { return (size_t)2 * V2_TILE * sizeof(int16_t) + groups * sizeof(V2Scratch) + V2_RECS * sizeof(b200_intra_tu) + V2_OWN * sizeof(int) + V2_FLAGS + 64; }
__device__ __forceinline__ void v2_cp4(void* smemDst, const void* gmemSrc)
{
  const unsigned d = (unsigned)__cvta_generic_to_shared(smemDst);
  asm volatile("cp.async.ca.shared.global [%0], [%1], 4;\n" :: "r"(d), "l"(gmemSrc));
}
__device__ __forceinline__ void v2_cp16(void* smemDst, const void* gmemSrc)
{
  const unsigned d = (unsigned)__cvta_generic_to_shared(smemDst);
  asm volatile("cp.async.cg.shared.global [%0], [%1], 16;\n" :: "r"(d), "l"(gmemSrc));
}
__device__ __forceinline__ void v2_cp_wait() { asm volatile("cp.async.wait_all;\n" ::: "memory"); }

__device__ __forceinline__ int v2_tile_off(int c) { return c == 0 ? 0 : c == 1 ? 128 * V2_LS : 128 * V2_LS + 64 * V2_CS; }

__global__ void __launch_bounds__(1024) intra_ctu_order_kernel(const IntraParams P, int* ctuOrder, int* counters)
{
  extern __shared__ int sCnt[];
  const int n = P.ctusW * P.ctusH;
  for (int i = threadIdx.x; i < n; i += blockDim.x) sCnt[i] = P.ctuCnt[i];
  __syncthreads();
  for (int i = threadIdx.x; i < n; i += blockDim.x) {
    if (sCnt[i] <= 0) continue;
    const int y = i / P.ctusW, x = i - y * P.ctusW, key = x + 2 * y;
    int rank = 0;
    for (int j = 0; j < n; j++) { const int yj = j / P.ctusW, kj = (j - yj * P.ctusW) + 2 * yj; rank += (sCnt[j] > 0) && (kj < key || (kj == key && yj < y)); }
    ctuOrder[rank] = i;
  }
  if (threadIdx.x == 0) { int m = 0; for (int j = 0; j < n; j++) m += sCnt[j] > 0; counters[0] = m; counters[1] = 0; }
}
__global__ void __launch_bounds__(256) intra_ctu_check_kernel(const IntraParams P)
{
  const int i = blockIdx.x * 256 + threadIdx.x;
  if (i >= P.numTus) return;
  const int c = intra_ctu_of(P, P.tus[i]);
  if (i - P.ctuFirst[c] >= P.ctuCnt[c]) atomicOr(P.err, INTRA_ERR_ORDER);
  if (i == P.ctuFirst[c] && P.ctuCnt[c] > V2_FLAGS) atomicOr(P.err, INTRA_ERR_CTU_BLOCKS);
}

__device__ __forceinline__ int v2_ld_acquire(const int* p) { int v; asm volatile("ld.acquire.gpu.global.b32 %0, [%1];" : "=r"(v) : "l"(p) : "memory"); return v; }
__device__ __forceinline__ void v2_st_release(int* p, int v) { asm volatile("st.release.gpu.global.b32 [%0], %1;" :: "l"(p), "r"(v) : "memory"); }

__device__ __forceinline__ void v2_wait(const IntraParams& P, const volatile uint8_t* sflag, int o, int me, int first)
{
  if (o < 0 || o >= me) return;
  int spins = 0;
  if (o >= first) {
    while (sflag[o - first] == 0) { if (++spins > 64) __nanosleep(20); if (spins > (1 << 24)) { atomicOr(P.err, 1); break; } }
    __threadfence_block();
    return;
  }
  const volatile int* e = P.err;
  while (v2_ld_acquire(P.done + o) == 0) { __nanosleep(32); if (*e || ++spins > (1 << 22)) { atomicOr(P.err, 1); break; } }
}

#ifdef B200_K6_PROF
__device__ unsigned long long gK6Prof[48];
#define K6P(i, t0) do { if (lane == 0) atomicAdd(&gK6Prof[i], (unsigned long long)(clock64() - (t0))); } while (0)
#define K6C(i) do { if (lane == 0) atomicAdd(&gK6Prof[i], 1ull); } while (0)
#else
#define K6P(i, t0) do {} while (0)
#define K6C(i) do {} while (0)
#endif
template <int V2_GROUP, int V2_GROUPS>
__global__ void __launch_bounds__(V2_GROUP * V2_GROUPS, 1) intra_ctu_kernel(const IntraParams P, const int* __restrict__ ctuOrder, int* counters)
{
  constexpr int V2_THREADS = V2_GROUP * V2_GROUPS;
  extern __shared__ __align__(16) unsigned char smem[];
  int16_t* tileRec = reinterpret_cast<int16_t*>(smem);
  int16_t* tileRes = tileRec + V2_TILE;
  V2Scratch* scratch = reinterpret_cast<V2Scratch*>(tileRes + V2_TILE);
  b200_intra_tu* srec = reinterpret_cast<b200_intra_tu*>(scratch + V2_GROUPS);
  int* sown = reinterpret_cast<int*>(srec + V2_RECS);
  volatile uint8_t* sflag = reinterpret_cast<volatile uint8_t*>(sown + V2_OWN);
  __shared__ int sCtu, sNext;
  const int tid = threadIdx.x, lane = tid & (V2_GROUP - 1), grp = tid / V2_GROUP;
  const int nComp = P.planes[1] ? 3 : 1;
  const int ctuSize = 1 << P.ctuLog2;
  for (;;) {
    __syncthreads();
    if (tid == 0) { sCtu = atomicAdd(&counters[1], 1); sNext = V2_GROUPS; }
    __syncthreads();
    if (sCtu >= counters[0] || (*(volatile int*)P.err & (INTRA_ERR_ORDER | INTRA_ERR_CTU_BLOCKS))) return;
    const int ctu = ctuOrder[sCtu], first = P.ctuFirst[ctu], cnt = P.ctuCnt[ctu];
    long long tp = clock64(); (void)tp;
    const int cx = (ctu % P.ctusW) << P.ctuLog2, cy = (ctu / P.ctusW) << P.ctuLog2, cw = min(ctuSize, P.W - cx), ch = min(ctuSize, P.H - cy);
    for (int c = 0; c < nComp; c++) {
      const int sh = c ? 1 : 0, ox = cx >> sh, oy = cy >> sh, tw = cw >> sh, th = ch >> sh, ts = c ? V2_CS : V2_LS;
      int16_t* rec = tileRec + v2_tile_off(c); int16_t* res = tileRes + v2_tile_off(c);
      const int16_t* src = P.planes[c] + (size_t)oy * P.stride[c] + ox;
      const int16_t* rsrc = P.resi[c] ? P.resi[c] + (size_t)oy * P.stride[c] + ox : nullptr;
      if (!(P.stride[c] & 7) && !(tw & 7) && !((uintptr_t)src & 15) && !((uintptr_t)rsrc & 15)) {
        const int wv = tw >> 3, n = wv * th;
        for (int k = tid; k < n; k += V2_THREADS) {
          const int y = k / wv, x = (k - y * wv) * 8;
          v2_cp16(rec + y * ts + x, src + (size_t)y * P.stride[c] + x);
          if (rsrc) v2_cp16(res + y * ts + x, rsrc + (size_t)y * P.stride[c] + x);
        }
      } else {
        const int wWords = tw >> 1, n = wWords * th;
        for (int k = tid; k < n; k += V2_THREADS) {
          const int y = k / wWords, x = (k - y * wWords) * 2;
          v2_cp4(rec + y * ts + x, src + (size_t)y * P.stride[c] + x);
          if (rsrc) v2_cp4(res + y * ts + x, rsrc + (size_t)y * P.stride[c] + x);
        }
      }
      const int unit = c ? 2 : 4, uw = tw / unit, uh = th / unit;
      const int* osrc = P.owner[c] + (size_t)(oy / unit) * P.ownerStride[c] + ox / unit;
      for (int k = tid; k < uw * uh; k += V2_THREADS) { const int y = k / uw, x = k - y * uw; v2_cp4(sown + c * 1024 + y * 32 + x, osrc + (size_t)y * P.ownerStride[c] + x); }
    }
    for (int k = tid; k < min(cnt, V2_RECS) * 4; k += V2_THREADS) v2_cp4(reinterpret_cast<uint32_t*>(srec) + k, reinterpret_cast<const uint32_t*>(P.tus + first) + k);
    for (int k = tid; k < cnt; k += V2_THREADS) sflag[k] = P.compSel == 2 ? (uint8_t)(P.tus[first + k].comp == 0) : 0;
    v2_cp_wait();
    __syncthreads();
    K6P(0, tp); K6C(8);

    V2Scratch& SC = scratch[grp];
#define V2_SYNC() do { if (V2_GROUP == 32) __syncwarp(); else asm volatile("bar.sync %0, %1;" :: "r"(grp + 1), "r"(V2_GROUP) : "memory"); } while (0)
    int slot = 0;
    for (int k = grp; k < cnt; k = SC.next[slot], slot ^= 1) {
      if (lane == 0) { SC.next[slot] = atomicAdd(&sNext, 1); SC.sum = 0; }
      tp = clock64(); const long long tb0 = tp; (void)tb0;
      const int me = first + k;
      const b200_intra_tu t = k < V2_RECS ? srec[k] : P.tus[me];
      if ((P.compSel == 1 && t.comp != 0) || (P.compSel == 2 && t.comp == 0)) { V2_SYNC(); continue; }
      const int c = t.comp, w = 1 << t.log2w, h = 1 << t.log2h, mrl = c ? 0 : t.multiRefIdx, unit = c ? 2 : 4;
      const int x0 = t.x, y0 = t.y, ps = P.stride[c], pmax = (1 << P.bitDepth) - 1;
      const int availTL = (t.flags & B200_INTRA_AVAIL_TL) ? 1 : 0, numAbove = t.numAbove, numLeft = t.numLeft;
      ISP_GEOMETRY
      const int csh = c ? 1 : 0, tox = cx >> csh, toy = cy >> csh, ttw = cw >> csh, tth = ch >> csh, tts = c ? V2_CS : V2_LS;
      int16_t* trec = tileRec + v2_tile_off(c); const int16_t* tplane = P.planes[c];
      auto pixC = [&](int x, int y) -> int {
        return ((unsigned)(x - tox) < (unsigned)ttw && (unsigned)(y - toy) < (unsigned)tth) ? (int)trec[(y - toy) * tts + (x - tox)] : (int)__ldcg(tplane + (size_t)y * ps + x);
      };
      if (ispK && lane == 0) v2_wait(P, sflag, me - 1, me, first);
      for (int dep = lane; dep < 96; dep += V2_GROUP) {
        int ux = -1, uy = -1;
        if (dep == 0) { if (availTL) { ux = bx - 1; uy = by - 1; } }
        else if (dep <= numAbove) { ux = bx + (dep - 1) * unit; uy = by - 1; }
        else if (dep - 64 >= 0 && dep - 64 < numLeft) { ux = bx - 1; uy = by + (dep - 64) * unit; }
        if (ux >= 0 && uy >= 0) {
          const int ush = c ? 1 : 2, ox = (ux >> ush) - (tox >> ush), oy = (uy >> ush) - (toy >> ush);
          const int o = ((unsigned)ox < 32u && (unsigned)oy < 32u && ux < tox + ttw && uy < toy + tth) ? sown[c * 1024 + oy * 32 + ox] : __ldcg(P.owner[c] + (size_t)(uy >> ush) * P.ownerStride[c] + (ux >> ush));
          v2_wait(P, sflag, o, me, first);
        }
      }
      if (t.mode >= B200_INTRA_LM) {
        const bool aCu = t.flags & B200_INTRA_LM_ABOVE, lCu = t.flags & B200_INTRA_LM_LEFT;
        const int nA = max(w, aCu ? (t.mode == B200_INTRA_MDLM_T ? 2 * t.lmAbove : w) : 0), nL = max(h, lCu ? (t.mode == B200_INTRA_MDLM_L ? 2 * t.lmLeft : h) : 0);
        const int ux0 = max(0, (2 * x0 - (lCu ? 4 : 0)) >> 2), ux1 = min(P.W - 1, 2 * x0 + 2 * nA - 1) >> 2;
        const int uy0 = max(0, (2 * y0 - (aCu ? 4 : 0)) >> 2), uy1 = min(P.H - 1, 2 * y0 + 2 * nL - 1) >> 2;
        const int uw = ux1 - ux0 + 1, nU = uw * (uy1 - uy0 + 1);
        for (int u = lane; u < nU; u += V2_GROUP) {
          const int gx = ux0 + u % uw, gy = uy0 + u / uw, ox = gx - cx / 4, oy = gy - cy / 4;
          const int o = ((unsigned)ox < 32u && (unsigned)oy < 32u && gx * 4 < cx + cw && gy * 4 < cy + ch) ? sown[oy * 32 + ox] : __ldcg(P.owner[0] + (size_t)gy * P.ownerStride[0] + gx);
          v2_wait(P, sflag, o, me, first);
        }
      }
      V2_SYNC();
      const int pb = c ? 16 : 0; (void)pb;
      K6P(pb + 1, tp); tp = clock64();

      const int predSize = 2 * bw, predHSize = 2 * bh;
      const int totalUnits = (predSize + unit - 1) / unit + (predHSize + unit - 1) / unit + 1, n = availTL + numAbove + numLeft;
      const int aboveLen = min(numAbove * unit, predSize), leftLen = min(numLeft * unit, predHSize);
      int16_t *T = SC.T[0], *L = SC.L[0];
#define PIXR(x, y) pixC((x), (y))
      ISP_REFERENCE_LAMBDAS
      if (!isp && n == totalUnits) {
        const int rx = bx - 1 - mrl, ry = by - 1 - mrl;
        for (int j = lane; j <= max(topLen, sideLen) + mrl; j += V2_GROUP) {
          const bool doT = j <= topLen + mrl, doL = j <= sideLen + mrl;
          const int vt = doT ? pixC(rx + j, ry) : 0, vl = doL ? pixC(rx, ry + j) : 0;
          if (doT) T[j] = (int16_t)vt;
          if (doL) L[j] = (int16_t)vl;
        }
      } else {
        for (int j = lane; j <= max(topLen, sideLen) + mrl; j += V2_GROUP) {
          const bool doT = j <= topLen + mrl, doL = j >= 1 && j <= sideLen + mrl;
          const int vt = doT ? regT(j) : 0, vl = doL ? regL(j) : 0;
          if (doT) T[j] = (int16_t)vt;
          if (doL) L[j] = (int16_t)vl;
          if (j == 0) L[0] = (int16_t)vt;
        }
      }
#undef PIXR
      V2_SYNC();
      if ((t.flags & B200_INTRA_FILTER_REF) && !c && !mrl) {
        int16_t *FT = SC.T[1], *FL = SC.L[1];
        for (int j = lane; j <= predSize; j += V2_GROUP)
          FT[j] = j == 0 ? (int16_t)((L[1] + 2 * T[0] + T[1] + 2) >> 2) : j == predSize ? T[j] : (int16_t)((T[j + 1] + 2 * T[j] + T[j - 1] + 2) >> 2);
        for (int i = lane + 1; i <= predHSize; i += V2_GROUP)
          FL[i] = i == predHSize ? L[i] : (int16_t)((L[i + 1] + 2 * L[i] + L[i - 1] + 2) >> 2);
        V2_SYNC();
        if (lane == 0) FL[0] = FT[0];
        T = FT; L = FL;
        V2_SYNC();
      }

      K6P(pb + 2, tp); tp = clock64();
      const int mode = t.mode;
      const bool doPDPC = w >= 4 && h >= 4 && mrl == 0;
      int16_t* dstG = P.planes[c] + (size_t)y0 * ps + x0;
      int16_t* dstT = trec + (y0 - toy) * tts + (x0 - tox);
      const int tsC = tts;
      const int16_t* rsT = (P.resi[c] && (t.flags & B200_INTRA_ADD_RESI)) ? tileRes + v2_tile_off(c) + (y0 - toy) * tsC + (x0 - tox) : nullptr;
      const int ciipW = isp ? 0 : t.ciip;
#define V2_STORE(x, y, v) do { int v_ = (v); int16_t* d_ = dstT + (y) * tsC + (x); if (ciipW) v_ = ((4 - ciipW) * (int)*d_ + ciipW * v_ + 2) >> 2; \
                               if (rsT && ((resiMask >> ((x) >> l2tu)) & 1)) v_ = clip3(0, pmax, v_ + rsT[(y) * tsC + (x)]); *d_ = (int16_t)v_; dstG[(size_t)(y) * ps + (x)] = (int16_t)v_; } while (0)

      if (mode == B200_INTRA_PLANAR || mode == B200_INTRA_DC) {
        int dc = 0;
        if (mode == B200_INTRA_DC) {
          int part = 0;
          for (int i = lane; i < w + h; i += V2_GROUP) {
            if (i < w) { if (w >= h) part += T[mrl + 1 + i]; }
            else if (w <= h) part += L[mrl + 1 + i - w];
          }
          for (int o = 16; o; o >>= 1) part += __shfl_down_sync(0xffffffffu, part, o);
          if ((lane & 31) == 0 && part) atomicAdd(&SC.sum, part);
          V2_SYNC();
          const int denom = w == h ? w << 1 : max(w, h);
          dc = (SC.sum + (denom >> 1)) >> (31 - __clz(denom));
        }
        const int l2w = t.log2w, l2h = t.log2h, scale = (l2w - 2 + l2h - 2 + 2) >> 2;
        const int bl = L[h + 1], tr = T[w + 1];
#pragma unroll 2
        for (int kk = lane; kk < w * h; kk += V2_GROUP) {
          const int y = kk >> l2w, x = kk & (w - 1);
          int v;
          if (mode == B200_INTRA_PLANAR) {
            const int hor = (L[y + 1] << l2w) + (x + 1) * (tr - L[y + 1]), vert = (T[x + 1] << l2h) + (y + 1) * (bl - T[x + 1]);
            v = ((hor << l2h) + (vert << l2w) + (1 << (l2w + l2h))) >> (1 + l2w + l2h);
          } else v = dc;
          v = (int16_t)v;
          if (doPDPC) {
            const int wT = 32 >> min(31, (y << 1) >> scale), wL = 32 >> min(31, (x << 1) >> scale);
            v = (int16_t)(v + ((wL * (L[y + 1] - v) + wT * (T[x + 1] - v) + 32) >> 6));
          }
          V2_STORE(x, y, v);
        }
      } else if (mode >= B200_INTRA_LM) {
        const bool aCu = t.flags & B200_INTRA_LM_ABOVE, lCu = t.flags & B200_INTRA_LM_LEFT, colloc = t.flags & B200_INTRA_LM_COLLOCATED;
        const int lx0 = 2 * x0, ly0 = 2 * y0;
        const bool firstRowOfCtu = ((2 * y0) & ((1 << P.ctuLog2) - 1)) == 0;
        const int nTop = aCu ? (mode == B200_INTRA_MDLM_T ? 2 * t.lmAbove : w) : 0, nLeft = lCu ? (mode == B200_INTRA_MDLM_L ? 2 * t.lmLeft : h) : 0;
        const int16_t* lplane = P.planes[0]; const int lps = P.stride[0];
        auto pixY = [&](int x, int y) -> int {
          return ((unsigned)(x - cx) < (unsigned)cw && (unsigned)(y - cy) < (unsigned)ch) ? (int)tileRec[(y - cy) * V2_LS + (x - cx)] : (int)__ldcg(lplane + (size_t)y * lps + x);
        };
#define LY(dx, dy) pixY(lx0 + (dx), ly0 + (dy))
        for (int kk = lane; kk < nTop + nLeft + w * h; kk += V2_GROUP) {
          if (kk < nTop) {
            const int i = kk, m = (i == 0 && !lCu) ? 0 : 1;
            int v;
            if (firstRowOfCtu) v = (LY(2 * i, -1) * 2 + LY(2 * i - m, -1) + LY(2 * i + 1, -1) + 2) >> 2;
            else if (colloc) v = (LY(2 * i, -3) + LY(2 * i, -2) * 4 + LY(2 * i - m, -2) + LY(2 * i + 1, -2) + LY(2 * i, -1) + 4) >> 3;
            else v = (LY(2 * i, -2) * 2 + LY(2 * i - m, -2) + LY(2 * i + 1, -2) + LY(2 * i, -1) * 2 + LY(2 * i - m, -1) + LY(2 * i + 1, -1) + 4) >> 3;
            SC.LmTop[i] = (int16_t)v;
          } else if (kk < nTop + nLeft) {
            const int j = kk - nTop;
            int v;
            if (colloc) v = (LY(-2, 2 * j - ((j == 0 && !aCu) ? 0 : 1)) + LY(-2, 2 * j) * 4 + LY(-3, 2 * j) + LY(-1, 2 * j) + LY(-2, 2 * j + 1) + 4) >> 3;
            else v = (LY(-2, 2 * j) * 2 + LY(-3, 2 * j) + LY(-1, 2 * j) + LY(-2, 2 * j + 1) * 2 + LY(-3, 2 * j + 1) + LY(-1, 2 * j + 1) + 4) >> 3;
            SC.LmLeft[j] = (int16_t)v;
          } else {
            const int q = kk - nTop - nLeft, j = q >> t.log2w, i = q & (w - 1), m = (i == 0 && !lCu) ? 0 : 1;
            int v;
            if (colloc) { const int up = (j == 0 && !aCu) ? 0 : 1; v = (LY(2 * i, 2 * j - up) + LY(2 * i, 2 * j) * 4 + LY(2 * i - m, 2 * j) + LY(2 * i + 1, 2 * j) + LY(2 * i, 2 * j + 1) + 4) >> 3; }
            else v = (LY(2 * i, 2 * j) * 2 + LY(2 * i + 1, 2 * j) + LY(2 * i - m, 2 * j) + LY(2 * i, 2 * j + 1) * 2 + LY(2 * i + 1, 2 * j + 1) + LY(2 * i - m, 2 * j + 1) + 4) >> 3;
            SC.Lm[q] = (int16_t)v;
          }
        }
#undef LY
        V2_SYNC();
        if (lane == 0) {
          const int tuWU = w >> 1, tuHU = h >> 1;
          bool aboveAvail = false, leftAvail = false; int topNum = 0, leftNum = 0;
          if (mode == B200_INTRA_MDLM_T) { aboveAvail = t.lmAbove >= tuWU; topNum = 2 * t.lmAbove; }
          else if (mode == B200_INTRA_MDLM_L) { leftAvail = t.lmLeft >= tuHU; leftNum = 2 * t.lmLeft; }
          else { aboveAvail = aCu; leftAvail = lCu; topNum = w; leftNum = h; }
          const int aboveIs4 = leftAvail ? 0 : 1, leftIs4 = aboveAvail ? 0 : 1;
          const int start0 = topNum >> (2 + aboveIs4), step0 = max(1, topNum >> (1 + aboveIs4)), start1 = leftNum >> (2 + leftIs4), step1 = max(1, leftNum >> (1 + leftIs4));
          int sl[4] = {0, 0, 0, 0}, sc[4] = {0, 0, 0, 0}, cntT = 0, cntL = 0;
          if (aboveAvail) { cntT = min(topNum, (1 + aboveIs4) << 1); for (int q = 0, pos = start0; q < cntT; q++, pos += step0) { sl[q] = SC.LmTop[pos]; sc[q] = T[1 + pos]; } }
          if (leftAvail) { cntL = min(leftNum, (1 + leftIs4) << 1); for (int q = 0, pos = start1; q < cntL; q++, pos += step1) { sl[q + cntT] = SC.LmLeft[pos]; sc[q + cntT] = L[1 + pos]; } }
          if (cntT + cntL == 2) { sl[3] = sl[0]; sc[3] = sc[0]; sl[2] = sl[1]; sc[2] = sc[1]; sl[0] = sl[1]; sc[0] = sc[1]; sl[1] = sl[3]; sc[1] = sc[3]; }
          int mn0 = 0, mn1 = 2, mx0 = 1, mx1 = 3, tt;
          if (sl[mn0] > sl[mn1]) { tt = mn0; mn0 = mn1; mn1 = tt; }
          if (sl[mx0] > sl[mx1]) { tt = mx0; mx0 = mx1; mx1 = tt; }
          if (sl[mn0] > sl[mx1]) { tt = mn0; mn0 = mx0; mx0 = tt; tt = mn1; mn1 = mx1; mx1 = tt; }
          if (sl[mn1] > sl[mx0]) { tt = mn1; mn1 = mx0; mx0 = tt; }
          const int minL = (sl[mn0] + sl[mn1] + 1) >> 1, minC = (sc[mn0] + sc[mn1] + 1) >> 1, maxL = (sl[mx0] + sl[mx1] + 1) >> 1, maxC = (sc[mx0] + sc[mx1] + 1) >> 1;
          int a = 0, b = 1 << (P.bitDepth - 1), shift = 0;
          if (leftAvail || aboveAvail) {
            const int diff = maxL - minL;
            if (diff > 0) {
              const int diffC = maxC - minC;
              int x = 31 - __clz(diff);
              const int normDiff = (diff << 4 >> x) & 15;
              const int v = (int)((0x0765544332211110ull >> (4 * (15 - normDiff))) & 15) | 8;
              x += normDiff != 0;
              const int y = diffC == 0 ? 0 : (31 - __clz(abs(diffC))) + 1, add = 1 << y >> 1;
              a = (diffC * v + add) >> y; shift = 3 + x - y;
              if (shift < 1) { shift = 1; a = a == 0 ? 0 : a < 0 ? -15 : 15; }
              b = minC - ((a * minL) >> shift);
            } else { a = 0; b = minC; shift = 0; }
          }
          SC.LmPar[0] = a; SC.LmPar[1] = b; SC.LmPar[2] = shift;
        }
        V2_SYNC();
        const int a = SC.LmPar[0], b = SC.LmPar[1], shift = SC.LmPar[2];
        for (int kk = lane; kk < w * h; kk += V2_GROUP) { const int y = kk >> t.log2w, x = kk & (w - 1); V2_STORE(x, y, clip3(0, pmax, ((a * SC.Lm[kk]) >> shift) + b)); }
      } else if (mode == B200_INTRA_MIP) {
        const int sizeId = (w == 4 && h == 4) ? 0 : (w == 4 || h == 4 || (w == 8 && h == 8)) ? 1 : 2;
        const int bdry = sizeId == 0 ? 2 : 4, red = sizeId < 2 ? 4 : 8, upH = w / red, upV = h / red, inSize = 2 * bdry;
        const int modeIdx = t.mip & 0x7f; const bool transpose = t.mip >> 7;
        int16_t* in = SC.S; int16_t* sM = SC.M;
        if (lane < inSize) {
          const bool fromLeft = (lane >= bdry) != transpose; const int d = lane % bdry, len = fromLeft ? h : w;
          const int16_t* full = (fromLeft ? L : T) + 1;
          int v;
          if (bdry < len) { const int f = len / bdry; int sum = 0; for (int j = 0; j < f; j++) sum += full[d * f + j]; v = (sum + (f >> 1)) >> (31 - __clz(f)); }
          else v = full[d];
          in[lane] = (int16_t)v;
        }
        V2_SYNC();
        const int inputOffset = in[0];
        V2_SYNC();
        if (lane < inSize) in[lane] = (int16_t)(lane == 0 ? (sizeId < 2 ? (1 << (P.bitDepth - 1)) - inputOffset : 0) : in[lane] - inputOffset);
        V2_SYNC();
        for (int o = lane; o < red * red; o += V2_GROUP) {
          const int redSize = sizeId == 2, stride = inSize - redSize;
          const uint8_t* wgt = (sizeId == 0 ? kMip4x4 + modeIdx * 64 : sizeId == 1 ? kMip8x8 + modeIdx * 128 : kMip16x16 + modeIdx * 448) + o * stride;
          int sum = 0, acc = 0;
          for (int i = 0; i < inSize; i++) sum += in[i];
          for (int i = redSize; i < inSize; i++) acc += in[i] * wgt[i - redSize];
          const int v = clip3(0, pmax, ((acc + 32 - 32 * sum) >> 6) + inputOffset);
          sM[transpose ? (o % red) * red + o / red : o] = (int16_t)v;
        }
        V2_SYNC();
        const int l2H = 31 - __clz(upH), l2V = 31 - __clz(upV);
        for (int kk = lane; kk < w * h; kk += V2_GROUP) {
          const int y = kk >> t.log2w, x = kk & (w - 1), kr = y / upV, i = y % upV;
          int hv[2];
#pragma unroll
          for (int q = 0; q < 2; q++) {
            const int k2 = kr - 1 + q;
            if (k2 < 0) hv[q] = T[x + 1];
            else if (upH == 1) hv[q] = sM[k2 * red + x];
            else {
              const int j = x / upH, ii = x % upH, before = j == 0 ? L[(k2 + 1) * upV] : sM[k2 * red + j - 1], behind = sM[k2 * red + j];
              hv[q] = (int16_t)(before * upH + (upH >> 1) + (ii + 1) * (behind - before)) >> l2H;
            }
          }
          V2_STORE(x, y, upV == 1 ? hv[1] : (int16_t)(hv[0] * upV + (upV >> 1) + (i + 1) * (hv[1] - hv[0])) >> l2V);
        }
      } else if (mode >= B200_INTRA_BDPCM_HOR) {
        for (int kk = lane; kk < w * h; kk += V2_GROUP) { const int y = kk >> t.log2w, x = kk & (w - 1); V2_STORE(x, y, mode == B200_INTRA_BDPCM_HOR ? L[y + 1] : T[x + 1]); }
      } else {
        const int predMode = wide_angle(bw, bh, mode);
        const bool ver = predMode >= 34;
        const int angMode = ver ? predMode - 50 : -(predMode - 18), absMode = abs(angMode);
        const int invAngle = cInvAng[absMode], absAng = cAng[absMode], angle = angMode < 0 ? -absAng : absAng;
        const int16_t *mainSrc = ver ? T : L, *sideSrc = ver ? L : T;
        const int mw = ver ? w : h, mh = ver ? h : w;
        const int16_t *Mp, *Sp = sideSrc + mrl;
        int mEnd;
        if (angle < 0) {
          int16_t* M = SC.M + IT_ORG;
          for (int kk = lane - mh; kk <= mw + 1 + mrl; kk += V2_GROUP) M[kk] = kk >= 0 ? mainSrc[kk] : sideSrc[min((-kk * invAngle + 256) >> 9, mh)];
          V2_SYNC();
          Mp = M + mrl; mEnd = 1 << 20;
        } else { Mp = mainSrc + mrl; mEnd = ver ? topLen : sideLen; }
#define MAIN(i) Mp[min((i), mEnd)]
        const int l2mw = 31 - __clz(mw), l2mh = 31 - __clz(mh);
        const int topLeft = T[0];
        const int scale0 = (l2mw - 2 + l2mh - 2 + 2) >> 2;
        const int lev = min(3 << scale0, mw);
        const bool frac = (absAng & 31) != 0;
        const int diff = min(abs(predMode - 18), abs(predMode - 50));
        const bool cubic = isp || !(diff > cIntraFilterThr[(l2mw + l2mh) >> 1]) || mrl > 0;
        int angularScale = -1;
        if (angle > 0 && doPDPC) angularScale = min(2, l2mh - ((31 - __clz(3 * invAngle - 2)) - 8));
#pragma unroll 2
        for (int kk = lane; kk < mw * mh; kk += V2_GROUP) {
          const int yy = kk >> l2mw, xx = kk & (mw - 1);
          int v;
          if (angle == 0) {
            if (doPDPC && xx < lev) { const int wL = 32 >> min(31, (xx << 1) >> scale0); v = clip3(0, pmax, (wL * (Sp[yy + 1] - topLeft) + MAIN(xx + 1) * 64 + 32) >> 6); }
            else v = MAIN(xx + 1);
          } else {
            const int deltaPos = angle * (1 + mrl + yy), dI = deltaPos >> 5, dF = deltaPos & 31;
            if (!frac) v = MAIN(dI + 1 + xx);
            else if (c) v = (int16_t)(((32 - dF) * MAIN(dI + 1 + xx) + dF * MAIN(dI + 2 + xx) + 16) >> 5);
            else {
              const int p = dI + xx;
              int f0, f1, f2, f3;
              if (cubic) { f0 = kIfChroma[dF * 4]; f1 = kIfChroma[dF * 4 + 1]; f2 = kIfChroma[dF * 4 + 2]; f3 = kIfChroma[dF * 4 + 3]; }
              else { f0 = 16 - (dF >> 1); f1 = 32 - (dF >> 1); f2 = 16 + (dF >> 1); f3 = dF >> 1; }
              v = (int16_t)((f0 * MAIN(p) + f1 * MAIN(p + 1) + f2 * MAIN(p + 2) + f3 * MAIN(p + 3) + 32) >> 6);
              if (cubic) v = clip3(0, pmax, v);
            }
            if (angularScale >= 0 && xx < min(3 << angularScale, mw)) {
              const int invAngleSum = 256 + (xx + 1) * invAngle, wL = 32 >> (2 * xx >> angularScale), left = Sp[yy + (invAngleSum >> 9) + 1];
              v = (int16_t)(v + ((wL * (left - v) + 32) >> 6));
            }
          }
          if (ver) V2_STORE(xx, yy, v); else V2_STORE(yy, xx, v);
        }
#undef MAIN
      }
#undef V2_STORE
      V2_SYNC();
      K6P(pb + 3, tp); tp = clock64();
      if (lane == 0) {
        __threadfence_block();
        sflag[k] = 1;
        if (x0 + w == tox + ttw || y0 + h == toy + tth) v2_st_release(P.done + me, 1);
      }
      K6P(pb + 4, tp); K6C(pb + 9); K6P(pb + 10 + min(4, max(0, ((int)t.log2w + (int)t.log2h - 4) >> 1)), tb0);
    }
#undef V2_SYNC
  }
}

__global__ void __launch_bounds__(256) intra_validate_kernel(const b200_intra_tu* __restrict__ tus, int n, int W, int H, int chroma, int ctuLog2, int* meta)
{
  const int i = blockIdx.x * 256 + threadIdx.x;
  if (i >= n) return;
  const b200_intra_tu t = tus[i];
  if (!intra_record_in_ctu(t, ctuLog2)) { atomicOr(&meta[LM_ERR], 8); return; }
  if (t.flags & B200_INTRA_ISP) { b200_intra_tu prev; if (i) prev = tus[i - 1]; if (!intra_isp_record_ok(t, i ? &prev : nullptr, W, H)) atomicOr(&meta[LM_ERR], 8); return; }
  const int w = 1 << t.log2w, h = 1 << t.log2h, pw = t.comp ? W >> 1 : W, ph = t.comp ? H >> 1 : H, unit = t.comp ? 2 : 4, m = t.multiRefIdx;
  bool ok = t.comp < (chroma ? 3 : 1) && t.log2w >= 2 && t.log2w <= 6 && t.log2h >= 1 && t.log2h <= 6 && t.x + w <= pw && t.y + h <= ph && !(t.x % unit) && !(t.y % unit);
  ok = ok && t.mode <= B200_INTRA_MDLM_T && m <= 2 && (!m || !t.comp);
  if (t.ciip) ok = ok && t.ciip <= 3 && t.mode == B200_INTRA_PLANAR;
  if (t.mode >= B200_INTRA_LM) ok = ok && t.comp && t.log2w <= 5 && t.log2h <= 5 && t.lmAbove <= w && t.lmLeft <= h && (!(t.flags & B200_INTRA_LM_ABOVE) || t.y >= 2) && (!(t.flags & B200_INTRA_LM_LEFT) || t.x >= 2)
                                  && t.x + max(w, 2 * t.lmAbove) <= pw && t.y + max(h, 2 * t.lmLeft) <= ph;
  if (t.mode == B200_INTRA_MIP) ok = ok && !t.comp && !m && (t.mip & 0x7f) < ((w == 4 && h == 4) ? 16 : (w == 4 || h == 4 || (w == 8 && h == 8)) ? 8 : 6);
  ok = ok && t.numAbove <= 2 * w / unit && t.numLeft <= 2 * h / unit && (!t.numAbove || t.y > m) && (!t.numLeft || t.x > m)
          && (!(t.flags & B200_INTRA_AVAIL_TL) || (t.x > m && t.y > m)) && t.x + (int)t.numAbove * unit <= pw && t.y + (int)t.numLeft * unit <= ph;
  if (!ok) atomicOr(&meta[LM_ERR], 8);
}

#ifdef B200_K6_PROF
extern "C" __attribute__((visibility("default"))) void b200_k6_prof_dump(int reset)
{
  unsigned long long h[48]; cudaDeviceSynchronize(); cudaMemcpyFromSymbol(h, gK6Prof, sizeof(h));
  const double nc = (double)(h[8] ? h[8] : 1);
  fprintf(stderr, "K6 prof: %.0f group-CTUs, set-up %.0f cyc each\n", nc, h[0] / nc);
  for (int c = 0; c < 2; c++) {
    const int b = c * 16; const double nb = (double)(h[b + 9] ? h[b + 9] : 1);
    fprintf(stderr, "  %s: %.0f blocks | wait %.0f, refs %.0f, predict %.0f, publish %.0f cyc | whole block by size class (<=32, <=128, <=512, <=2048, more samples): %.0f %.0f %.0f %.0f %.0f cyc-sums/blocks\n", c ? "chroma" : "luma", nb,
            h[b + 1] / nb, h[b + 2] / nb, h[b + 3] / nb, h[b + 4] / nb, h[b + 10] / nb, h[b + 11] / nb, h[b + 12] / nb, h[b + 13] / nb, h[b + 14] / nb);
  }
  if (reset) { memset(h, 0, sizeof(h)); cudaMemcpyToSymbol(gK6Prof, h, sizeof(h)); }
}
#endif
__global__ void __launch_bounds__(128) intra_ciip_clear_kernel(const b200_intra_tu* __restrict__ tus, int numTus, int16_t* r0, int16_t* r1, int16_t* r2, int s0, int s1, int s2)
{
  for (int k = blockIdx.x; k < numTus; k += gridDim.x) {
    const b200_intra_tu t = tus[k];
    if (!t.ciip || (t.flags & B200_INTRA_ISP) || !(t.flags & B200_INTRA_ADD_RESI)) continue;
    int16_t* r = t.comp == 0 ? r0 : t.comp == 1 ? r1 : r2;
    const int s = t.comp == 0 ? s0 : t.comp == 1 ? s1 : s2, w = 1 << t.log2w, n = w << t.log2h;
    for (int i = threadIdx.x; i < n; i += blockDim.x) r[(size_t)(t.y + (i >> t.log2w)) * s + t.x + (i & (w - 1))] = 0;
  }
}

int launch_intra_ciip_clear(const b200_intra_tu* tus, size_t numTus, int16_t* const resi[3], const int stride[3], cudaStream_t s)
{
  if (!numTus) return 0;
  const int grid = (int)std::min<size_t>(numTus, (size_t)2 * num_sms());
  intra_ciip_clear_kernel<<<grid, 128, 0, s>>>(tus, (int)numTus, resi[0], resi[1], resi[2], stride[0], stride[1], stride[2]);
  B200_CUDA(cudaGetLastError());
  return 0;
}

int launch_intra_validate(const b200_intra_tu* tus, size_t numTus, const b200_geom& g, int* meta, cudaStream_t s)
{
  if (!numTus) return 0;
  intra_validate_kernel<<<(unsigned)((numTus + 255) / 256), 256, 0, s>>>(tus, (int)numTus, g.width, g.height, g.chromaFormat != 0, intra_ctu_log2(g), meta);
  B200_CUDA(cudaGetLastError());
  return 0;
}

constexpr int kWaveCtasPerDiag2 = 6;

int launch_intra(const IntraLaunch& L, cudaStream_t s)
{
  if (!L.numTus) return 0;
  IntraParams P;
  for (int c = 0; c < 3; c++) { P.planes[c] = L.planes.p[c]; P.resi[c] = L.resi[c]; P.stride[c] = L.planes.stride[c]; P.owner[c] = L.owner[c]; P.ownerStride[c] = L.ownerStride[c]; }
  if (!L.geom.chromaFormat) { P.planes[1] = P.planes[2] = nullptr; }
  P.W = L.geom.width; P.H = L.geom.height; P.bitDepth = L.geom.bitDepth; P.tus = L.tus; P.numTus = (int)L.numTus;
  P.done = L.sync; P.ticket = L.sync + L.numTus; P.err = L.sync + L.numTus + 1; P.compSel = L.compSel;
  const bool cont = L.compSel == 2;
  if (cont) B200_CUDA(cudaMemsetAsync(P.ticket, 0, sizeof(int), s));
  else {
    B200_CUDA(cudaMemsetAsync(L.sync, 0, (L.numTus + 2) * sizeof(int), s));
    for (int c = 0; c < (L.geom.chromaFormat ? 3 : 1); c++) B200_CUDA(cudaMemsetAsync(L.owner[c], 0xff, L.ownerBytes[c], s));
  }
  P.perm = nullptr; P.ctuCnt = P.ctuFirst = P.ctuBase = nullptr;
  P.ctuLog2 = intra_ctu_log2(L.geom); P.ctusW = (L.geom.width + L.geom.ctuSize - 1) / L.geom.ctuSize; P.ctusH = (L.geom.height + L.geom.ctuSize - 1) / L.geom.ctuSize;
  const char* variant = getenv("B200_INTRA_KERNEL");
  const bool force1 = variant && !strcmp(variant, "v1"), force2 = variant && !strcmp(variant, "v2");
  const bool dense = L.numTus >= 48 * std::max<size_t>(1, (size_t)L.geom.width * L.geom.height >> 14);
  const bool v1 = !L.order || force1 || (!force2 && !dense) || ((P.stride[0] | P.stride[1] | P.stride[2]) & 1);
  const unsigned grid = (unsigned)((L.numTus + 255) / 256);
  if (!cont) intra_owner_kernel<<<(unsigned)L.numTus, 64, 0, s>>>(P);
  if (!v1) {
    const size_t nCtu = (size_t)P.ctusW * P.ctusH;
    int* base = L.order; P.ctuCnt = base; P.ctuFirst = base + nCtu; int* ctuOrder = base + 2 * nCtu; int* counters = base + 3 * nCtu;
    if (cont) B200_CUDA(cudaMemsetAsync(counters + 1, 0, sizeof(int), s));
    else {
      B200_CUDA(cudaMemsetAsync(P.ctuCnt, 0, nCtu * sizeof(int), s));
      B200_CUDA(cudaMemsetAsync(P.ctuFirst, 0x7f, nCtu * sizeof(int), s));
      intra_ctu_count_kernel<<<grid, 256, 0, s>>>(P);
      intra_ctu_check_kernel<<<grid, 256, 0, s>>>(P);
      intra_ctu_order_kernel<<<1, 1024, nCtu * sizeof(int), s>>>(P, ctuOrder, counters);
    }
    int diag = 1;
    for (int key = 0; key < P.ctusW + 2 * P.ctusH; key++) {
      int n = 0;
      for (int y = 0; y < P.ctusH; y++) n += key - 2 * y >= 0 && key - 2 * y < P.ctusW;
      diag = std::max(diag, n);
    }
    const int ctas = (int)std::min<size_t>({nCtu, (size_t)num_sms(), (size_t)(kWaveCtasPerDiag2 * diag + 1) / 2});
    static const int shape = getenv("B200_INTRA_GROUP") ? atoi(getenv("B200_INTRA_GROUP")) : 0;
#define V2_GO(G, N) do { static bool attr = false; if (!attr) { B200_CUDA(cudaFuncSetAttribute(intra_ctu_kernel<G, N>, cudaFuncAttributeMaxDynamicSharedMemorySize, (int)v2_smem(N))); attr = true; } \
                         intra_ctu_kernel<G, N><<<ctas, G * N, v2_smem(N), s>>>(P, ctuOrder, counters); } while (0)
    if (shape == 1284) V2_GO(128, 4); else if (shape == 32) V2_GO(32, 8); else V2_GO(128, 5);
#undef V2_GO
    B200_CUDA(cudaGetLastError());
    return 0;
  }
  const char* order = getenv("B200_INTRA_ORDER");
  const bool listOrder = order && !strcmp(order, "decode");
  if (L.order && !listOrder && L.numTus >= 100 * std::max<size_t>(1, (size_t)L.geom.width * L.geom.height >> 14)) {
    const size_t nCtu = (size_t)P.ctusW * P.ctusH;
    int* perm = L.order; P.ctuCnt = perm + L.numTus; P.ctuFirst = P.ctuCnt + nCtu; P.ctuBase = P.ctuFirst + nCtu;
    if (!cont) {
      B200_CUDA(cudaMemsetAsync(P.ctuCnt, 0, nCtu * sizeof(int), s));
      B200_CUDA(cudaMemsetAsync(P.ctuFirst, 0x7f, nCtu * sizeof(int), s));
      intra_ctu_count_kernel<<<grid, 256, 0, s>>>(P);
      intra_ctu_base_kernel<<<1, 1, 0, s>>>(P);
      intra_perm_kernel<<<grid, 256, 0, s>>>(P, perm);
    }
    P.perm = perm;
  }
  const int ctas = (int)std::min<size_t>(L.numTus, (size_t)num_sms() * 12);
  intra_kernel<<<ctas, IT_THREADS, 0, s>>>(P);
  B200_CUDA(cudaGetLastError());
  return 0;
}

}
```

vvdec_b200/csrc/picture.cu:

```cuda
#include "common.cuh"
#include <string.h>
#include <vector>

namespace b200 {

static inline size_t align256(size_t v) { return (v + 255) & ~(size_t)255; }

struct Arena {
  DevBuf buf;
  const b200_pu* pus = nullptr; size_t numPus = 0; const uint32_t* tiles = nullptr; int* mcMeta = nullptr;
  int* hMeta = nullptr;
  const b200_tu* tus = nullptr; size_t numTus = 0; const uint32_t* tuIdx = nullptr; int* tuMeta = nullptr; const int16_t* coefs = nullptr; const int32_t* scaling = nullptr;
  const b200_lf_param *lfV = nullptr, *lfH = nullptr; const uint8_t* ctuSlice = nullptr; LfSliceTab lfSlices; b200_lf_seq lfSeq;
  const b200_sao_ctu* sao = nullptr; b200_vb vb;
  const b200_alf_ctu* alf = nullptr; const int16_t *lumaCoeff = nullptr, *lumaClip = nullptr, *chromaCoeff = nullptr, *chromaClip = nullptr, *cc[2] = {nullptr, nullptr};
  int32_t* dmvrMv = nullptr; size_t numDmvr = 0;
  const b200_wp* wp = nullptr;
  const b200_lmcs* lmcs = nullptr; const int16_t* lmcsInv = nullptr; const b200_lmcs_vpdu* lmcsVpdus = nullptr; int* lmcsScale = nullptr; bool lmcsChromaAdj = false;
  int16_t* given[3] = {nullptr, nullptr, nullptr};
  const b200_intra_tu* intraTus = nullptr; size_t numIntraTus = 0; int* intraOwner[3] = {nullptr, nullptr, nullptr}; int intraOwnerStride[3] = {0, 0, 0}; size_t intraOwnerBytes[3] = {0, 0, 0}; int* intraSync = nullptr; int* intraOrder = nullptr;
  int dstSlot = 0, flags = 0;
  bool ciipResi = false;
  bool valid = false;
  cudaEvent_t uploaded = nullptr, done = nullptr; bool donePending = false;
};

}

using namespace b200;

struct CtxProf : b200::KProf {
  struct Rec { int family; cudaEvent_t a, b; };
  std::vector<Rec> recs; std::vector<cudaEvent_t> pool; Rec cur{};
  cudaEvent_t get() { cudaEvent_t e; if (!pool.empty()) { e = pool.back(); pool.pop_back(); } else cudaEventCreate(&e); return e; }
  void begin(int f, cudaStream_t s) override { cur.family = f; cur.a = get(); cur.b = get(); cudaEventRecord(cur.a, s); }
  void end(int, cudaStream_t s) override { cudaEventRecord(cur.b, s); recs.push_back(cur); }
};

struct b200_ctx {
  b200_geom g;
  CtxProf prof; bool profiling = false;
  int numSlots = 0, numArenas = 0, device = 0;
  cudaStream_t stream = nullptr, copyStream = nullptr, upStream = nullptr;
  StreamSet ss;
  cudaEvent_t ev[2] = {nullptr, nullptr};
  std::vector<cudaEvent_t> readDone; std::vector<char> readPending;
  cudaEvent_t ticketEv[16]; cudaEvent_t finalEv = nullptr; int nextTicket = 0;
  DevBuf outStage[2]; int nextStage = 0;
  size_t planeBytes[3] = {0, 0, 0}, picBytes = 0;
  std::vector<int16_t*> bufs;
  std::vector<int> slotBuf;
  int work[2] = {0, 0};
  std::vector<Arena> arenas;
  int nextArena = 0;
  long long launches = 0;
  DevBuf grainStage[2], grainTab;
  DevBuf resiBuf;
  DevBuf hashBuf;
  void* tmaps = nullptr;

  DevPlanes planes(int buf) const {
    DevPlanes d; char* b = reinterpret_cast<char*>(bufs[buf]);
    d.p[0] = reinterpret_cast<int16_t*>(b); d.p[1] = reinterpret_cast<int16_t*>(b + planeBytes[0]); d.p[2] = reinterpret_cast<int16_t*>(b + planeBytes[0] + planeBytes[1]);
    for (int c = 0; c < 3; c++) d.stride[c] = g.stride[c];
    return d;
  }
};

extern "C" {

B200_API int b200_ctx_create(b200_ctx** out, const b200_geom* g, int numSlots, int numArenas, int device)
{
  B200_CHECK(out && g, "b200_ctx_create: null argument");
  B200_CHECK(numSlots >= 1 && numSlots <= B200_MAX_SLOTS && numArenas >= 1 && numArenas <= 256, "b200_ctx_create: numSlots %d / numArenas %d out of range", numSlots, numArenas);
  B200_CHECK((g->width & 7) == 0 && (g->height & 7) == 0, "b200_ctx_create: picture size must be a multiple of 8");
  B200_CHECK(g->chromaFormat == 0 || g->chromaFormat == 1, "b200_ctx_create: only 4:0:0 and 4:2:0");
  B200_CHECK(g->ctuSize == 32 || g->ctuSize == 64 || g->ctuSize == 128, "b200_ctx_create: CTU size %d", g->ctuSize);
  if (int rc = ensure_device()) return rc;
  if (device >= 0) B200_CUDA(cudaSetDevice(device));
  b200_ctx* c = new b200_ctx;
  c->g = *g; c->numSlots = numSlots; c->numArenas = numArenas;
  B200_CUDA(cudaGetDevice(&c->device));
  B200_CUDA(cudaStreamCreateWithFlags(&c->stream, cudaStreamNonBlocking));
  B200_CUDA(cudaStreamCreateWithFlags(&c->copyStream, cudaStreamNonBlocking));
  B200_CUDA(cudaStreamCreateWithFlags(&c->upStream, cudaStreamNonBlocking));
  c->ss.main = c->stream; c->ss.nAux = 3;
  B200_CUDA(cudaEventCreateWithFlags(&c->ss.forkEv, cudaEventDisableTiming));
  for (int k = 0; k < c->ss.nAux; k++) { B200_CUDA(cudaStreamCreateWithFlags(&c->ss.aux[k], cudaStreamNonBlocking)); B200_CUDA(cudaEventCreateWithFlags(&c->ss.joinEv[k], cudaEventDisableTiming)); }
  B200_CUDA(cudaEventCreate(&c->ev[0])); B200_CUDA(cudaEventCreate(&c->ev[1]));
  B200_CUDA(cudaEventCreateWithFlags(&c->finalEv, cudaEventDisableTiming));
  for (auto& e : c->ticketEv) B200_CUDA(cudaEventCreateWithFlags(&e, cudaEventDisableTiming));
  for (int k = 0; k < 3; k++) c->planeBytes[k] = (k == 0 || g->chromaFormat) ? align256((size_t)g->stride[k] * (k ? g->height >> 1 : g->height) * 2) : 0;
  c->picBytes = c->planeBytes[0] + c->planeBytes[1] + c->planeBytes[2];
  c->bufs.resize(numSlots + 2); c->slotBuf.resize(numSlots);
  c->readDone.resize(numSlots + 2); c->readPending.assign(numSlots + 2, 0);
  for (auto& e : c->readDone) B200_CUDA(cudaEventCreateWithFlags(&e, cudaEventDisableTiming));
  for (int i = 0; i < numSlots + 2; i++) { B200_CUDA(cudaMalloc(&c->bufs[i], c->picBytes)); B200_CUDA(cudaMemset(c->bufs[i], 0, c->picBytes)); }
  for (int s = 0; s < numSlots; s++) c->slotBuf[s] = s;
  {
    std::vector<int16_t*> pl;
    for (int i = 0; i < numSlots + 2; i++) { DevPlanes d = c->planes(i); for (int k = 0; k < 3; k++) pl.push_back(d.p[k]); }
    if (int rc = make_mc_tensor_maps(*g, pl.data(), numSlots + 2, &c->tmaps)) return rc;
  }
  c->work[0] = numSlots; c->work[1] = numSlots + 1;
  c->arenas.resize(numArenas);
  for (auto& A : c->arenas) { B200_CUDA(cudaEventCreateWithFlags(&A.uploaded, cudaEventDisableTiming)); B200_CUDA(cudaEventCreateWithFlags(&A.done, cudaEventDisableTiming)); B200_CUDA(cudaHostAlloc(reinterpret_cast<void**>(&A.hMeta), (2 * LM_INTS + 4) * sizeof(int), cudaHostAllocDefault)); }
  *out = c;
  return 0;
}

B200_API void b200_ctx_destroy(b200_ctx* c)
{
  if (!c) return;
  cudaStreamSynchronize(c->stream); cudaStreamSynchronize(c->copyStream); cudaStreamSynchronize(c->upStream);
  for (auto& A : c->arenas) { cudaEventDestroy(A.uploaded); cudaEventDestroy(A.done); if (A.hMeta) cudaFreeHost(A.hMeta); }
  cudaStreamDestroy(c->upStream);
  for (auto p : c->bufs) cudaFree(p);
  if (c->tmaps) cudaFree(c->tmaps);
  for (auto e : c->readDone) cudaEventDestroy(e);
  for (auto e : c->ticketEv) cudaEventDestroy(e);
  cudaEventDestroy(c->finalEv); cudaStreamDestroy(c->copyStream);
  for (int k = 0; k < c->ss.nAux; k++) { cudaStreamSynchronize(c->ss.aux[k]); cudaStreamDestroy(c->ss.aux[k]); cudaEventDestroy(c->ss.joinEv[k]); }
  cudaEventDestroy(c->ss.forkEv);
  cudaEventDestroy(c->ev[0]); cudaEventDestroy(c->ev[1]);
  cudaStreamDestroy(c->stream);
  delete c;
}

B200_API int b200_ctx_load_slot(b200_ctx* c, int slot, const int16_t* const planes[3])
{
  B200_CHECK(c && planes && slot >= 0 && slot < c->numSlots, "b200_ctx_load_slot: bad argument");
  DevPlanes d = c->planes(c->slotBuf[slot]);
  for (int k = 0; k < (c->g.chromaFormat ? 3 : 1); k++)
    B200_CUDA(cudaMemcpyAsync(d.p[k], planes[k], (size_t)c->g.stride[k] * (k ? c->g.height >> 1 : c->g.height) * 2, cudaMemcpyHostToDevice, c->stream));
  B200_CUDA(cudaStreamSynchronize(c->stream));
  return 0;
}

B200_API int b200_pic_upload(b200_ctx* c, const b200_picture* p)
{
  B200_CHECK(c && p, "b200_pic_upload: null argument");
  B200_CHECK(p->dstSlot >= 0 && p->dstSlot < c->numSlots, "b200_pic_upload: dstSlot %d", p->dstSlot);
  B200_CHECK(!(p->flags & B200_PIC_DEBLOCK) || (p->lfV && p->lfH && p->lfSlices && p->numLfSlices >= 1 && p->numLfSlices <= 64), "b200_pic_upload: deblocking data missing");
  B200_CHECK(!(p->flags & B200_PIC_SAO) || p->sao, "b200_pic_upload: SAO data missing");
  B200_CHECK(!(p->flags & B200_PIC_ALF) || (p->alf && p->alfTabs && p->alfTabs->numLumaSets >= 16), "b200_pic_upload: ALF data missing");
  B200_CHECK(p->numPus < (1u << 26) && p->numTus < (1u << 31), "b200_pic_upload: too many records");
  B200_CHECK(p->numWp >= 0 && p->numWp <= 255 && (p->wp || !p->numWp), "b200_pic_upload: weighted-prediction table (at most 255 entries)");
  B200_CHECK(!(p->flags & B200_PIC_LMCS) || (p->lmcs && p->lmcs->invLUT && (!p->lmcs->chromaAdj || p->lmcs->vpdus) && p->lmcs->orgCW == (1 << c->g.bitDepth) / 16), "b200_pic_upload: LMCS data missing or inconsistent");
  B200_CHECK(!p->numIntraTus || (p->intraTus && p->numIntraTus < (1u << 30)), "b200_pic_upload: intra list missing");
  B200_CUDA(cudaSetDevice(c->device));
  const int ai = c->nextArena; c->nextArena = (c->nextArena + 1) % c->numArenas;
  Arena& A = c->arenas[ai];
  A.valid = false;
  const b200_geom& g = c->g;
  const size_t n4 = (size_t)((g.width + 3) >> 2) * ((g.height + 3) >> 2);
  const size_t nCtu = (size_t)((g.width + g.ctuSize - 1) / g.ctuSize) * ((g.height + g.ctuSize - 1) / g.ctuSize);
  const size_t capTiles = mc_tile_capacity(g, 0);
  const b200_alf_tables* T = p->alfTabs;
  const size_t nL = (p->flags & B200_PIC_ALF) ? (size_t)T->numLumaSets * 1300 : 0, nC = (p->flags & B200_PIC_ALF) ? (size_t)T->numChromaAlts * 7 : 0;
  const size_t n0 = (p->flags & B200_PIC_ALF) ? (size_t)T->numCc[0] * 7 : 0, n1 = (p->flags & B200_PIC_ALF) ? (size_t)T->numCc[1] * 7 : 0;
  size_t off = 0;
  auto take = [&](size_t bytes) { size_t o = off; off += align256(bytes + 16); return o; };
  const size_t oPus = take(p->numPus * sizeof(b200_pu)), oT = take(capTiles * 4), oMeta = take(2 * LM_INTS * sizeof(int)), oIdx = take(p->numTus * 4);
  const size_t oTus = take(p->numTus * sizeof(b200_tu)), oCoef = take(p->numCoefs * 2), oScal = take(p->numScaling * 4);
  const size_t oLfV = take((p->flags & B200_PIC_DEBLOCK) ? n4 * 6 : 0), oLfH = take((p->flags & B200_PIC_DEBLOCK) ? n4 * 6 : 0), oCs = take(nCtu);
  const size_t oSao = take((p->flags & B200_PIC_SAO) ? nCtu * sizeof(b200_sao_ctu) : 0);
  const size_t oAlf = take((p->flags & B200_PIC_ALF) ? nCtu * sizeof(b200_alf_ctu) : 0), oTab = take((2 * nL + 2 * nC + n0 + n1) * 2);
  const size_t oDm = take(p->numDmvr * 8);
  const size_t oWp = take((size_t)p->numWp * sizeof(b200_wp));
  const bool lm = p->flags & B200_PIC_LMCS;
  const int vs = g.ctuSize == 128 ? 64 : g.ctuSize; const size_t nVpdu = (size_t)((g.width + vs - 1) / vs) * ((g.height + vs - 1) / vs);
  const size_t oLm = take(lm ? sizeof(b200_lmcs) : 0), oLmLut = take(lm ? sizeof(int16_t) << g.bitDepth : 0), oLmVp = take(lm ? nVpdu * sizeof(b200_lmcs_vpdu) : 0), oLmSc = take(lm ? nVpdu * sizeof(int) : 0);
  const bool hasGiven = p->given[0] != nullptr;
  const size_t oGiven = take(hasGiven ? c->picBytes : 0);
  size_t oOwn[3] = {0, 0, 0}, ownBytes[3] = {0, 0, 0}; int ownStride[3] = {0, 0, 0};
  const size_t oIntra = take(p->numIntraTus * sizeof(b200_intra_tu)), oSync = take(p->numIntraTus ? (p->numIntraTus + 2) * sizeof(int) : 0), oOrder = take(p->numIntraTus ? intra_order_ints(g, p->numIntraTus) * sizeof(int) : 0);
  for (int k = 0; k < (g.chromaFormat ? 3 : 1) && p->numIntraTus; k++) {
    const int pw = k ? g.width >> 1 : g.width, ph = k ? g.height >> 1 : g.height, unit = k ? 2 : 4;
    ownStride[k] = (pw + unit - 1) / unit; ownBytes[k] = (size_t)ownStride[k] * ((ph + unit - 1) / unit) * sizeof(int); oOwn[k] = take(ownBytes[k]);
  }
  if (p->numIntraTus) if (int rc = c->resiBuf.reserve(c->picBytes)) return rc;
  if (off > A.buf.cap) { B200_CUDA(cudaStreamSynchronize(c->stream)); B200_CUDA(cudaStreamSynchronize(c->upStream)); A.donePending = false; }
  if (int rc = A.buf.reserve(off)) return rc;
  char* base = A.buf.as<char>();
  cudaStream_t s = c->upStream;
  if (A.donePending) { B200_CUDA(cudaStreamWaitEvent(s, A.done, 0)); A.donePending = false; }
  auto h2d = [&](size_t o, const void* src, size_t bytes) -> int { if (bytes) B200_CUDA(cudaMemcpyAsync(base + o, src, bytes, cudaMemcpyHostToDevice, s)); return 0; };
  if (int rc = h2d(oPus, p->pus, p->numPus * sizeof(b200_pu))) return rc;
  if (int rc = h2d(oTus, p->tus, p->numTus * sizeof(b200_tu))) return rc;
  if (int rc = h2d(oCoef, p->coefs, p->numCoefs * 2)) return rc;
  if (int rc = h2d(oScal, p->scaling, p->numScaling * 4)) return rc;
  if (p->flags & B200_PIC_DEBLOCK) {
    if (int rc = h2d(oLfV, p->lfV, n4 * 6)) return rc;
    if (int rc = h2d(oLfH, p->lfH, n4 * 6)) return rc;
    if (p->ctuSlice) if (int rc = h2d(oCs, p->ctuSlice, nCtu)) return rc;
    memset(&A.lfSlices, 0, sizeof(A.lfSlices)); memcpy(A.lfSlices.s, p->lfSlices, p->numLfSlices * sizeof(b200_lf_slice));
    if (p->lfSeq) A.lfSeq = *p->lfSeq; else memset(&A.lfSeq, 0, sizeof(A.lfSeq));
  }
  if (p->flags & B200_PIC_SAO) { if (int rc = h2d(oSao, p->sao, nCtu * sizeof(b200_sao_ctu))) return rc; if (p->vb) A.vb = *p->vb; else memset(&A.vb, 0, sizeof(A.vb)); }
  if (p->flags & B200_PIC_ALF) {
    if (int rc = h2d(oAlf, p->alf, nCtu * sizeof(b200_alf_ctu))) return rc;
    size_t o = oTab;
    auto up = [&](const int16_t* src, size_t n, const int16_t*& view) -> int { view = reinterpret_cast<const int16_t*>(base + o); int rc = h2d(o, src, n * 2); o += n * 2; return rc; };
    if (int rc = up(T->lumaCoeff, nL, A.lumaCoeff)) return rc;
    if (int rc = up(T->lumaClip, nL, A.lumaClip)) return rc;
    if (int rc = up(T->chromaCoeff, nC, A.chromaCoeff)) return rc;
    if (int rc = up(T->chromaClip, nC, A.chromaClip)) return rc;
    if (int rc = up(T->ccCoeff[0], n0, A.cc[0])) return rc;
    if (int rc = up(T->ccCoeff[1], n1, A.cc[1])) return rc;
  }
  if (int rc = h2d(oWp, p->wp, (size_t)p->numWp * sizeof(b200_wp))) return rc;
  A.wp = p->numWp ? reinterpret_cast<const b200_wp*>(base + oWp) : nullptr;
  if (lm) {
    if (int rc = h2d(oLm, p->lmcs, sizeof(b200_lmcs))) return rc;
    if (int rc = h2d(oLmLut, p->lmcs->invLUT, sizeof(int16_t) << g.bitDepth)) return rc;
    if (p->lmcs->chromaAdj) if (int rc = h2d(oLmVp, p->lmcs->vpdus, nVpdu * sizeof(b200_lmcs_vpdu))) return rc;
    A.lmcs = reinterpret_cast<const b200_lmcs*>(base + oLm); A.lmcsInv = reinterpret_cast<const int16_t*>(base + oLmLut);
    A.lmcsVpdus = reinterpret_cast<const b200_lmcs_vpdu*>(base + oLmVp); A.lmcsScale = reinterpret_cast<int*>(base + oLmSc); A.lmcsChromaAdj = p->lmcs->chromaAdj != 0;
  } else { A.lmcs = nullptr; A.lmcsChromaAdj = false; }
  if (hasGiven) {
    size_t o = oGiven;
    for (int k = 0; k < (g.chromaFormat ? 3 : 1); k++) {
      A.given[k] = reinterpret_cast<int16_t*>(base + o);
      if (int rc = h2d(o, p->given[k], (size_t)g.stride[k] * (k ? g.height >> 1 : g.height) * 2)) return rc;
      o += c->planeBytes[k];
    }
  } else A.given[0] = A.given[1] = A.given[2] = nullptr;
  A.pus = reinterpret_cast<const b200_pu*>(base + oPus); A.numPus = p->numPus;
  A.tus = reinterpret_cast<const b200_tu*>(base + oTus); A.numTus = p->numTus;
  A.coefs = reinterpret_cast<const int16_t*>(base + oCoef); A.scaling = reinterpret_cast<const int32_t*>(base + oScal);
  A.lfV = reinterpret_cast<const b200_lf_param*>(base + oLfV); A.lfH = reinterpret_cast<const b200_lf_param*>(base + oLfH);
  A.ctuSlice = p->ctuSlice ? reinterpret_cast<const uint8_t*>(base + oCs) : nullptr;
  A.sao = reinterpret_cast<const b200_sao_ctu*>(base + oSao); A.alf = reinterpret_cast<const b200_alf_ctu*>(base + oAlf);
  A.dmvrMv = p->numDmvr ? reinterpret_cast<int32_t*>(base + oDm) : nullptr; A.numDmvr = p->numDmvr;
  if (p->numDmvr) B200_CUDA(cudaMemsetAsync(base + oDm, 0, p->numDmvr * 8, s));
  if (int rc = h2d(oIntra, p->intraTus, p->numIntraTus * sizeof(b200_intra_tu))) return rc;
  A.intraTus = reinterpret_cast<const b200_intra_tu*>(base + oIntra); A.numIntraTus = p->numIntraTus; A.intraSync = reinterpret_cast<int*>(base + oSync); A.intraOrder = reinterpret_cast<int*>(base + oOrder);
  for (int k = 0; k < 3; k++) { A.intraOwner[k] = ownBytes[k] ? reinterpret_cast<int*>(base + oOwn[k]) : nullptr; A.intraOwnerStride[k] = ownStride[k]; A.intraOwnerBytes[k] = ownBytes[k]; }
  A.ciipResi = false;
  for (size_t i = 0; i < p->numIntraTus && !A.ciipResi; i++) { const b200_intra_tu& t = p->intraTus[i]; A.ciipResi = t.ciip && !(t.flags & B200_INTRA_ISP) && (t.flags & B200_INTRA_ADD_RESI); }
  A.dstSlot = p->dstSlot; A.flags = p->flags; A.valid = true;
  A.mcMeta = reinterpret_cast<int*>(base + oMeta); A.tuMeta = A.mcMeta + LM_INTS;
  if (int rc = launch_mc_bucket(reinterpret_cast<const b200_pu*>(base + oPus), p->numPus, reinterpret_cast<uint32_t*>(base + oT), capTiles, A.mcMeta, g, c->numSlots, p->numWp, p->numDmvr, s)) return rc;
  if (int rc = launch_tu_bucket(reinterpret_cast<const b200_tu*>(base + oTus), p->numTus, reinterpret_cast<uint32_t*>(base + oIdx), A.tuMeta, g, p->numCoefs, p->numScaling, s)) return rc;
  A.tiles = reinterpret_cast<const uint32_t*>(base + oT); A.tuIdx = reinterpret_cast<const uint32_t*>(base + oIdx);
  c->launches += 4;
  {
    CtuLimits lim; const bool alfOn = p->flags & B200_PIC_ALF;
    lim.numLumaSets = alfOn ? T->numLumaSets : 0; lim.numChromaAlts = alfOn ? T->numChromaAlts : 0; lim.numCc[0] = alfOn ? T->numCc[0] : 0; lim.numCc[1] = alfOn ? T->numCc[1] : 0;
    lim.numLfSlices = p->numLfSlices;
    const bool any = (p->flags & (B200_PIC_SAO | B200_PIC_ALF)) || ((p->flags & B200_PIC_DEBLOCK) && p->ctuSlice);
    if (int rc = launch_ctu_validate((p->flags & B200_PIC_SAO) ? A.sao : nullptr, alfOn ? A.alf : nullptr, (p->flags & B200_PIC_DEBLOCK) ? A.ctuSlice : nullptr, (int)nCtu, lim, A.mcMeta, s)) return rc;
    if (any) c->launches += 1;
  }
  if (A.numIntraTus) { if (int rc = launch_intra_validate(A.intraTus, A.numIntraTus, g, A.mcMeta, s)) return rc; c->launches += 1; }
  B200_CUDA(cudaMemcpyAsync(A.hMeta, A.mcMeta, 2 * LM_INTS * sizeof(int), cudaMemcpyDeviceToHost, s));
  B200_CUDA(cudaEventRecord(A.uploaded, s));
  return ai;
}

B200_API int b200_pic_run(b200_ctx* c, int ai)
{
  B200_CHECK(c && ai >= 0 && ai < c->numArenas && c->arenas[ai].valid, "b200_pic_run: bad arena %d", ai);
  B200_CUDA(cudaSetDevice(c->device));
  Arena& A = c->arenas[ai];
  cudaStream_t s = c->stream;
  B200_CUDA(cudaEventSynchronize(A.uploaded));
  B200_CHECK(!(A.hMeta[LM_ERR] & 1), "b200_pic_run: the picture's PU list holds an invalid record (reference slots, block size or flag combination)");
  B200_CHECK(!(A.hMeta[LM_ERR] & 2), "b200_pic_run: more MC tiles than the picture can hold (overlapping PUs?)");
  B200_CHECK(!(A.hMeta[LM_ERR] & 8), "b200_pic_run: an intra block record is invalid (geometry, mode, or availability reaching outside the picture)");
  B200_CHECK(!(A.hMeta[LM_ERR] & 4), "b200_pic_run: a CTU record (SAO type / band, ALF filter index, slice index) is out of range");
  B200_CHECK(!A.hMeta[LM_INTS + LM_ERR], "b200_pic_run: the picture's TU list holds an invalid record");
  B200_CUDA(cudaStreamWaitEvent(s, A.uploaded, 0));
  const b200_geom& g = c->g;
  int cur = c->work[0], other = c->work[1];
  for (int b : {cur, other}) if (c->readPending[b]) { B200_CUDA(cudaStreamWaitEvent(s, c->readDone[b], 0)); c->readPending[b] = 0; }
  DevPlanes P = c->planes(cur);
  if (A.given[0]) {
    for (int k = 0; k < (g.chromaFormat ? 3 : 1); k++)
      B200_CUDA(cudaMemcpyAsync(P.p[k], A.given[k], (size_t)g.stride[k] * (k ? g.height >> 1 : g.height) * 2, cudaMemcpyDeviceToDevice, s));
  }
  if (A.numPus) {
    McLaunch L; L.geom = g; L.dst = P; memset(L.refs, 0, sizeof(L.refs));
    for (int sl = 0; sl < c->numSlots; sl++) { DevPlanes d = c->planes(c->slotBuf[sl]); for (int k = 0; k < 3; k++) L.refs[sl * 3 + k] = d.p[k]; }
    for (int k = 0; k < 3; k++) L.refStride[k] = g.stride[k];
    L.tmaps = c->tmaps; for (int sl = 0; sl < c->numSlots; sl++) L.tmapBuf[sl] = (uint8_t)c->slotBuf[sl];
    L.pus = A.pus; L.tiles = A.tiles; L.meta = A.mcMeta; L.dmvrMv = A.dmvrMv; L.lmcs = A.lmcs; L.wp = A.wp;
    for (int l = 0; l < MC_LISTS; l++) L.cnt[l] = A.hMeta[LM_CNT + l];
    if (int rc = launch_mc(L, c->ss, c->profiling ? &c->prof : nullptr)) return rc;
    c->launches += mc_launch_count(L);
  }
  LmcsLaunch LM; LM.geom = g; LM.planes = P; LM.lmcs = A.lmcs; LM.vpdus = A.lmcsVpdus; LM.invLut = A.lmcsInv; LM.scale = A.lmcsScale;
  const bool twoPass = A.lmcs && A.lmcsChromaAdj;
  A.hMeta[2 * LM_INTS] = 0;
  int16_t* resiPl[3] = {nullptr, nullptr, nullptr};
  if (A.numIntraTus) {
    uint8_t* rb = c->resiBuf.as<uint8_t>(); resiPl[0] = reinterpret_cast<int16_t*>(rb); resiPl[1] = reinterpret_cast<int16_t*>(rb + c->planeBytes[0]); resiPl[2] = reinterpret_cast<int16_t*>(rb + c->planeBytes[0] + c->planeBytes[1]);
    if (A.ciipResi) { if (int rc = launch_intra_ciip_clear(A.intraTus, A.numIntraTus, resiPl, P.stride, s)) return rc; c->launches += 1; }
  }
  auto runK1 = [&](int compSel, const int* vpduScale) -> int {
    if (!A.numTus) return 0;
    K1Launch L; L.geom = g; L.planes = P; L.tus = A.tus; L.numTus = A.numTus; L.idx = A.tuIdx; L.meta = A.tuMeta; L.coefs = A.coefs; L.scaling = A.scaling; L.mode = 0;
    for (int k = 0; k < 3; k++) L.resi[k] = resiPl[k];
    for (int l = 0; l < K1_LISTS; l++) L.cnt[l] = A.hMeta[LM_INTS + LM_CNT + l];
    L.compSel = compSel; L.vpduScale = vpduScale;
    if (int rc = launch_k1_residual(L, c->ss, c->profiling ? &c->prof : nullptr)) return rc;
    c->launches += k1_launch_count(L);
    return 0;
  };
  auto runK6 = [&](int compSel) -> int {
    if (!A.numIntraTus) return 0;
    IntraLaunch L; L.geom = g; L.planes = P; L.tus = A.intraTus; L.numTus = A.numIntraTus; L.sync = A.intraSync; L.order = A.intraOrder; L.compSel = compSel;
    for (int k = 0; k < 3; k++) { L.resi[k] = resiPl[k]; L.owner[k] = A.intraOwner[k]; L.ownerStride[k] = A.intraOwnerStride[k]; L.ownerBytes[k] = A.intraOwnerBytes[k]; }
    if (c->profiling) c->prof.begin(B200_KF_INTRA, s);
    if (int rc = launch_intra(L, s)) return rc;
    if (c->profiling) c->prof.end(B200_KF_INTRA, s);
    c->launches += compSel == 2 ? 1 : 5;
    return 0;
  };
  if (twoPass) {
    if (int rc = runK1(1, nullptr)) return rc;
    if (int rc = runK6(1)) return rc;
    if (c->profiling) c->prof.begin(B200_KF_LMCS, s);
    if (int rc = launch_lmcs_vpdu(LM, s)) return rc;
    if (c->profiling) c->prof.end(B200_KF_LMCS, s);
    c->launches += 1;
    if (int rc = runK1(2, A.lmcsScale)) return rc;
    if (int rc = runK6(2)) return rc;
  } else {
    if (int rc = runK1(0, nullptr)) return rc;
    if (int rc = runK6(0)) return rc;
  }
  if (A.numIntraTus) B200_CUDA(cudaMemcpyAsync(A.hMeta + 2 * LM_INTS, A.intraSync + A.numIntraTus + 1, sizeof(int), cudaMemcpyDeviceToHost, s));
  if (A.lmcs) { if (c->profiling) c->prof.begin(B200_KF_LMCS, s); if (int rc = launch_lmcs_inv(LM, s)) return rc; if (c->profiling) c->prof.end(B200_KF_LMCS, s); c->launches += 1; }
  if (A.flags & B200_PIC_DEBLOCK) {
    LfLaunch L; L.geom = g; L.planes = P; L.lfV = A.lfV; L.lfH = A.lfH; L.ctuSlice = A.ctuSlice; L.slices = A.lfSlices; L.seq = A.lfSeq; L.dirs = 3;
    if (int rc = launch_lf_deblock(L, s, c->profiling ? &c->prof : nullptr)) return rc;
    c->launches += 2;
  }
  if (A.flags & B200_PIC_SAO) {
    SaoLaunch L; L.geom = g; L.src = P; L.dst = c->planes(other); L.ctus = A.sao; L.vb = A.vb;
    if (int rc = launch_sao(L, s, c->profiling ? &c->prof : nullptr)) return rc;
    c->launches += 1;
    std::swap(cur, other); P = c->planes(cur);
  }
  if (A.flags & B200_PIC_ALF) {
    AlfLaunch L; L.geom = g; L.src = P; L.dst = c->planes(other); L.ctus = A.alf;
    L.lumaCoeff = A.lumaCoeff; L.lumaClip = A.lumaClip; L.chromaCoeff = A.chromaCoeff; L.chromaClip = A.chromaClip; L.cc[0] = A.cc[0]; L.cc[1] = A.cc[1];
    if (int rc = launch_alf(L, c->ss, c->profiling ? &c->prof : nullptr)) return rc;
    c->launches += g.chromaFormat ? 2 : 1;
    std::swap(cur, other);
  }
  B200_CUDA(cudaEventRecord(A.done, s)); A.donePending = true;
  const int old = c->slotBuf[A.dstSlot];
  c->slotBuf[A.dstSlot] = cur;
  c->work[0] = old; c->work[1] = other;
  return 0;
}

B200_API int b200_decompress_picture(b200_ctx* c, const b200_picture* p)
{
  const int ai = b200_pic_upload(c, p);
  if (ai < 0) return ai;
  if (int rc = b200_pic_run(c, ai)) return rc;
  return ai;
}

B200_API int b200_wait_picture(b200_ctx* c, int ai, int32_t* dmvrMv, size_t numDmvr)
{
  B200_CHECK(c, "b200_wait_picture: null context");
  if (dmvrMv && ai >= 0 && ai < c->numArenas && c->arenas[ai].dmvrMv) {
    const size_t n = numDmvr < c->arenas[ai].numDmvr ? numDmvr : c->arenas[ai].numDmvr;
    B200_CUDA(cudaMemcpyAsync(dmvrMv, c->arenas[ai].dmvrMv, n * 8, cudaMemcpyDeviceToHost, c->stream));
  }
  B200_CUDA(cudaStreamSynchronize(c->upStream));
  B200_CUDA(cudaStreamSynchronize(c->stream));
  if (ai >= 0 && ai < c->numArenas && c->arenas[ai].numIntraTus) {
    const int err = c->arenas[ai].hMeta[2 * LM_INTS];
    B200_CHECK(!(err & INTRA_ERR_CTU_BLOCKS), "b200_wait_picture: a CTU holds more than %d intra block records (overlapping records?)", INTRA_MAX_CTU_BLOCKS);
    B200_CHECK(!err, "b200_wait_picture: an intra block waited for a neighbour that never finished (intra list not in decoding order?)");
  }
  return 0;
}

B200_API int b200_get_frame(b200_ctx* c, int slot, int16_t* const planes[3])
{
  B200_CHECK(c && planes && slot >= 0 && slot < c->numSlots, "b200_get_frame: bad argument");
  DevPlanes d = c->planes(c->slotBuf[slot]);
  for (int k = 0; k < (c->g.chromaFormat ? 3 : 1); k++)
    B200_CUDA(cudaMemcpyAsync(planes[k], d.p[k], (size_t)c->g.stride[k] * (k ? c->g.height >> 1 : c->g.height) * 2, cudaMemcpyDeviceToHost, c->stream));
  B200_CUDA(cudaStreamSynchronize(c->stream));
  return 0;
}

static int copy2d_host(void* dst, size_t dpitch, const void* src, size_t spitch, size_t wBytes, size_t h, cudaMemcpyKind kind, cudaStream_t s)
{
  const cudaError_t e = cudaMemcpy2DAsync(dst, dpitch, src, spitch, wBytes, h, kind, s);
  if (e != cudaErrorInvalidValue) { B200_CUDA(e); return 0; }
  (void)cudaGetLastError();
  void* stage = nullptr;
  B200_CUDA(cudaMallocHost(&stage, wBytes * h));
  int rc = 0;
  if (kind == cudaMemcpyHostToDevice) {
    for (size_t y = 0; y < h; y++) memcpy((char*)stage + y * wBytes, (const char*)src + y * spitch, wBytes);
    const cudaError_t e2 = cudaMemcpy2DAsync(dst, dpitch, stage, wBytes, wBytes, h, kind, s);
    const cudaError_t e3 = e2 == cudaSuccess ? cudaStreamSynchronize(s) : e2;
    if (e3 != cudaSuccess) { set_error("copy2d_host: staged H2D copy -> %s", cudaGetErrorString(e3)); (void)cudaGetLastError(); rc = B200_ERR_CUDA; }
  } else {
    const cudaError_t e2 = cudaMemcpy2DAsync(stage, wBytes, src, spitch, wBytes, h, kind, s);
    const cudaError_t e3 = e2 == cudaSuccess ? cudaStreamSynchronize(s) : e2;
    if (e3 != cudaSuccess) { set_error("copy2d_host: staged D2H copy -> %s", cudaGetErrorString(e3)); (void)cudaGetLastError(); rc = B200_ERR_CUDA; }
    else for (size_t y = 0; y < h; y++) memcpy((char*)dst + y * dpitch, (const char*)stage + y * wBytes, wBytes);
  }
  cudaFreeHost(stage);
  return rc;
}

B200_API int b200_ctx_load_slot_strided(b200_ctx* c, int slot, const int16_t* const planes[3], const ptrdiff_t strides[3])
{
  B200_CHECK(c && planes && strides && slot >= 0 && slot < c->numSlots, "b200_ctx_load_slot_strided: bad argument");
  DevPlanes d = c->planes(c->slotBuf[slot]);
  for (int k = 0; k < (c->g.chromaFormat ? 3 : 1); k++) {
    const size_t w = k ? c->g.width >> 1 : c->g.width, h = k ? c->g.height >> 1 : c->g.height;
    B200_CHECK(planes[k] && strides[k] >= (ptrdiff_t)w, "b200_ctx_load_slot_strided: plane %d", k);
    if (int rc = copy2d_host(d.p[k], (size_t)c->g.stride[k] * 2, planes[k], (size_t)strides[k] * 2, w * 2, h, cudaMemcpyHostToDevice, c->stream)) return rc;
  }
  B200_CUDA(cudaStreamSynchronize(c->stream));
  return 0;
}

B200_API int b200_get_frame_strided(b200_ctx* c, int slot, int16_t* const planes[3], const ptrdiff_t strides[3])
{
  B200_CHECK(c && planes && strides && slot >= 0 && slot < c->numSlots, "b200_get_frame_strided: bad argument");
  DevPlanes d = c->planes(c->slotBuf[slot]);
  for (int k = 0; k < (c->g.chromaFormat ? 3 : 1); k++) {
    const size_t w = k ? c->g.width >> 1 : c->g.width, h = k ? c->g.height >> 1 : c->g.height;
    B200_CHECK(planes[k] && strides[k] >= (ptrdiff_t)w, "b200_get_frame_strided: plane %d", k);
    if (int rc = copy2d_host(planes[k], (size_t)strides[k] * 2, d.p[k], (size_t)c->g.stride[k] * 2, w * 2, h, cudaMemcpyDeviceToHost, c->stream)) return rc;
  }
  B200_CUDA(cudaStreamSynchronize(c->stream));
  return 0;
}

B200_API int b200_get_frame_async(b200_ctx* c, int slot, int16_t* const planes[3])
{
  B200_CHECK(c && planes && slot >= 0 && slot < c->numSlots, "b200_get_frame_async: bad argument");
  const int buf = c->slotBuf[slot];
  DevPlanes d = c->planes(buf);
  B200_CUDA(cudaEventRecord(c->finalEv, c->stream));
  B200_CUDA(cudaStreamWaitEvent(c->copyStream, c->finalEv, 0));
  for (int k = 0; k < (c->g.chromaFormat ? 3 : 1); k++)
    B200_CUDA(cudaMemcpyAsync(planes[k], d.p[k], (size_t)c->g.stride[k] * (k ? c->g.height >> 1 : c->g.height) * 2, cudaMemcpyDeviceToHost, c->copyStream));
  B200_CUDA(cudaEventRecord(c->readDone[buf], c->copyStream)); c->readPending[buf] = 1;
  const int t = c->nextTicket; c->nextTicket = (c->nextTicket + 1) & 15;
  B200_CUDA(cudaEventRecord(c->ticketEv[t], c->copyStream));
  return t;
}

B200_API int b200_get_frame_device_async(b200_ctx* c, int slot, int16_t* const planesDev[3], void* cudaStream)
{
  B200_CHECK(c && planesDev && slot >= 0 && slot < c->numSlots, "b200_get_frame_device_async: bad argument");
  cudaStream_t st = static_cast<cudaStream_t>(cudaStream);
  const int buf = c->slotBuf[slot];
  DevPlanes d = c->planes(buf);
  B200_CUDA(cudaEventRecord(c->finalEv, c->stream));
  B200_CUDA(cudaStreamWaitEvent(st, c->finalEv, 0));
  for (int k = 0; k < (c->g.chromaFormat ? 3 : 1); k++) {
    B200_CHECK(planesDev[k], "b200_get_frame_device_async: plane %d", k);
    B200_CUDA(cudaMemcpyAsync(planesDev[k], d.p[k], (size_t)c->g.stride[k] * (k ? c->g.height >> 1 : c->g.height) * 2, cudaMemcpyDeviceToDevice, st));
  }
// ... 140 lines not shown
```

Before: 1132.

## Precompute intra block dependency lists at upload and wait only on those

Adds a dependency-building kernel that, for each intra block, gathers the deduplicated earlier blocks owning its reference samples into a compact pool. The owner-map and dependency kernels move to the picture upload stage, so they run before the timed reconstruction and can overlap other work. The intra kernel then waits only on those listed predecessors instead of recomputing neighbour ownership. It also uses cp.async and acquire/release flags. In exchange it costs extra device memory, a capacity check with a new error path, and a new public API for reading the dependencies.

```diff
diff --git a/include/vvdec_b200.h b/include/vvdec_b200.h
--- a/include/vvdec_b200.h
+++ b/include/vvdec_b200.h
@@ -184,6 +184,7 @@
 } b200_intra_tu;
 B200_API int b200_intra_predict(const b200_geom* g, int16_t* const planes[3], const b200_intra_tu* tus, size_t numTus);
 B200_API int b200_intra_reconstruct(const b200_geom* g, int16_t* const planes[3], const int16_t* const resi[3], const b200_intra_tu* tus, size_t numTus);
+B200_API int b200_intra_deps(const b200_geom* g, const b200_intra_tu* tus, size_t numTus, int32_t* counts, int32_t* deps, size_t capacity);
 
 typedef struct b200_ctx b200_ctx;
 
diff --git a/vvdec_b200/bindings.py b/vvdec_b200/bindings.py
--- a/vvdec_b200/bindings.py
+++ b/vvdec_b200/bindings.py
@@ -50,6 +50,7 @@
     lib.b200_get_frame_fmt_async.argtypes = [CTX, C.c_int, C.c_int, C.POINTER(C.c_void_p)]
     lib.b200_intra_predict.argtypes = [C.POINTER(abi.Geom), PLANES, C.c_void_p, C.c_size_t]
     lib.b200_intra_reconstruct.argtypes = [C.POINTER(abi.Geom), PLANES, PLANES, C.c_void_p, C.c_size_t]
+    lib.b200_intra_deps.argtypes = [C.POINTER(abi.Geom), C.c_void_p, C.c_size_t, C.c_void_p, C.c_void_p, C.c_size_t]
     lib.b200_frame_hash_async.argtypes = [CTX, C.c_int, C.c_int, C.c_void_p]
     lib.b200_get_frame_grain_async.argtypes = [CTX, C.c_int, C.c_int, C.POINTER(C.c_void_p), C.POINTER(abi.FilmGrain)]
     lib.b200_ctx_mark.argtypes = [CTX, C.c_int]
@@ -63,6 +64,6 @@
 
 
 EXPORTS = ["b200_ctx_create", "b200_ctx_destroy", "b200_ctx_load_slot", "b200_decompress_picture", "b200_pic_upload", "b200_pic_run",
-           "b200_wait_picture", "b200_get_frame", "b200_ctx_load_slot_strided", "b200_get_frame_strided", "b200_get_frame_async", "b200_get_frame_device_async", "b200_frame_wait", "b200_frame_bytes", "b200_get_frame_fmt_async", "b200_frame_hash_async", "b200_intra_predict", "b200_intra_reconstruct", "b200_get_frame_grain_async", "b200_ctx_mark", "b200_ctx_elapsed_ms", "b200_ctx_kernel_launches", "b200_ctx_set_profiling", "b200_ctx_get_kernel_ms", "b200_ctx_get_kernel_ms_n", "b200_host_register", "b200_host_unregister",
+           "b200_wait_picture", "b200_get_frame", "b200_ctx_load_slot_strided", "b200_get_frame_strided", "b200_get_frame_async", "b200_get_frame_device_async", "b200_frame_wait", "b200_frame_bytes", "b200_get_frame_fmt_async", "b200_frame_hash_async", "b200_intra_predict", "b200_intra_reconstruct", "b200_intra_deps", "b200_get_frame_grain_async", "b200_ctx_mark", "b200_ctx_elapsed_ms", "b200_ctx_kernel_launches", "b200_ctx_set_profiling", "b200_ctx_get_kernel_ms", "b200_ctx_get_kernel_ms_n", "b200_host_register", "b200_host_unregister",
            "b200_mc_predict", "b200_mc_predict_wp", "b200_last_error", "b200_version", "b200_device_count", "b200_k1_residual", "b200_lf_deblock",
            "b200_sao_picture", "b200_alf_picture"]
diff --git a/vvdec_b200/csrc/api.cu b/vvdec_b200/csrc/api.cu
--- a/vvdec_b200/csrc/api.cu
+++ b/vvdec_b200/csrc/api.cu
@@ -2,6 +2,7 @@
 #include <stdarg.h>
 #include <string.h>
 #include <mutex>
+#include <vector>
 
 namespace b200 {
 
@@ -30,7 +31,7 @@
 }
 
 struct HostWrapScratch {
-  DevBuf planes[3], tus, coefs, scaling, misc[8];
+  DevBuf planes[3], tus, coefs, scaling, misc[9];
   cudaStream_t stream = nullptr;
   int init() { if (!stream) { B200_CUDA(cudaStreamCreateWithFlags(&stream, cudaStreamNonBlocking)); } return 0; }
 };
@@ -181,10 +182,8 @@
   return 0;
 }
 
-B200_API int b200_intra_reconstruct(const b200_geom* g, int16_t* const planes[3], const int16_t* const resi[3], const b200_intra_tu* tus, size_t numTus)
-{
-  B200_CHECK(g && planes && (tus || !numTus), "b200_intra_reconstruct: null argument");
-  B200_CHECK(g->bitDepth >= 8 && g->bitDepth <= 12, "b200_intra_reconstruct: bit depth %d unsupported", g->bitDepth);
+static int intra_check_records(const b200_geom* g, const b200_intra_tu* tus, size_t numTus)
+{
   const int nPl = g->chromaFormat ? 3 : 1;
   for (size_t i = 0; i < numTus; i++) {
     const b200_intra_tu& t = tus[i];
@@ -208,18 +207,39 @@
                && (!(t.flags & B200_INTRA_AVAIL_TL) || (t.x > t.multiRefIdx && t.y > t.multiRefIdx)) && t.x + (int)t.numAbove * unit <= pw && t.y + (int)t.numLeft * unit <= ph,
                "b200_intra_reconstruct: record %zu: availability outside the picture", i);
   }
-  if (int rc = ensure_device()) return rc;
-  if (int rc = g_hw.init()) return rc;
-  cudaStream_t s = g_hw.stream;
-  IntraLaunch L; L.geom = *g; L.numTus = numTus;
-  if (int rc = upload_planes(g, planes, L.planes, s)) return rc;
+  return 0;
+}
+
+static int intra_scratch(const b200_geom* g, size_t numTus, IntraLaunch& L)
+{
   for (int c = 0; c < 3; c++) {
     L.resi[c] = nullptr; L.owner[c] = nullptr; L.ownerStride[c] = 0; L.ownerBytes[c] = 0;
-    if (c >= nPl) continue;
+    if (c >= (g->chromaFormat ? 3 : 1)) continue;
     const int pw = c ? g->width >> 1 : g->width, ph = c ? g->height >> 1 : g->height, unit = c ? 2 : 4;
     L.ownerStride[c] = (pw + unit - 1) / unit; L.ownerBytes[c] = (size_t)L.ownerStride[c] * ((ph + unit - 1) / unit) * sizeof(int);
     if (int rc = g_hw.misc[c].reserve(L.ownerBytes[c])) return rc;
     L.owner[c] = g_hw.misc[c].as<int>();
+  }
+  if (int rc = g_hw.misc[6].reserve((numTus + 2) * sizeof(int))) return rc;
+  if (int rc = g_hw.misc[8].reserve(intra_dep_ints(numTus) * sizeof(int))) return rc;
+  L.sync = g_hw.misc[6].as<int>(); L.deps = g_hw.misc[8].as<int>();
+  return 0;
+}
+
+B200_API int b200_intra_reconstruct(const b200_geom* g, int16_t* const planes[3], const int16_t* const resi[3], const b200_intra_tu* tus, size_t numTus)
+{
+  B200_CHECK(g && planes && (tus || !numTus), "b200_intra_reconstruct: null argument");
+  B200_CHECK(g->bitDepth >= 8 && g->bitDepth <= 12, "b200_intra_reconstruct: bit depth %d unsupported", g->bitDepth);
+  const int nPl = g->chromaFormat ? 3 : 1;
+  if (int rc = intra_check_records(g, tus, numTus)) return rc;
+  if (int rc = ensure_device()) return rc;
+  if (int rc = g_hw.init()) return rc;
+  cudaStream_t s = g_hw.stream;
+  IntraLaunch L; L.geom = *g; L.numTus = numTus;
+  if (int rc = upload_planes(g, planes, L.planes, s)) return rc;
+  if (int rc = intra_scratch(g, numTus, L)) return rc;
+  for (int c = 0; c < nPl; c++) {
+    const int ph = c ? g->height >> 1 : g->height;
     if (resi && resi[c]) {
       const size_t bytes = (size_t)g->stride[c] * ph * sizeof(int16_t);
       if (int rc = g_hw.misc[3 + c].reserve(bytes)) return rc;
@@ -228,17 +248,49 @@
     }
   }
   if (int rc = g_hw.tus.reserve(numTus * sizeof(b200_intra_tu) + 16)) return rc;
-  if (int rc = g_hw.misc[6].reserve((numTus + 2) * sizeof(int))) return rc;
   if (int rc = g_hw.misc[7].reserve(intra_order_ints(*g, numTus) * sizeof(int))) return rc;
   if (numTus) B200_CUDA(cudaMemcpyAsync(g_hw.tus.p, tus, numTus * sizeof(b200_intra_tu), cudaMemcpyHostToDevice, s));
-  L.tus = g_hw.tus.as<b200_intra_tu>(); L.sync = g_hw.misc[6].as<int>(); L.order = g_hw.misc[7].as<int>();
+  L.tus = g_hw.tus.as<b200_intra_tu>(); L.order = g_hw.misc[7].as<int>();
   if (int rc = launch_intra(L, s)) return rc;
   int err = 0;
   if (numTus) B200_CUDA(cudaMemcpyAsync(&err, L.sync + numTus + 1, sizeof(int), cudaMemcpyDeviceToHost, s));
   if (int rc = download_planes(g, planes, L.planes, s)) return rc;
   B200_CUDA(cudaStreamSynchronize(s));
   B200_CHECK(!(err & INTRA_ERR_CTU_BLOCKS), "b200_intra_reconstruct: a CTU holds more than %d intra block records (overlapping records?)", INTRA_MAX_CTU_BLOCKS);
+  B200_CHECK(!(err & INTRA_ERR_DEPS), "b200_intra_reconstruct: the blocks wait for more than %d earlier blocks each on average (overlapping records?)", INTRA_DEP_SLOTS);
   B200_CHECK(!err, "b200_intra_reconstruct: a block waited for a neighbour that never finished, or the blocks of a CTU are not contiguous (list not in decoding order?)");
+  return 0;
+}
+
+B200_API int b200_intra_deps(const b200_geom* g, const b200_intra_tu* tus, size_t numTus, int32_t* counts, int32_t* deps, size_t capacity)
+{
+  B200_CHECK(g && (tus || !numTus) && (counts || !numTus), "b200_intra_deps: null argument");
+  if (int rc = intra_check_records(g, tus, numTus)) return rc;
+  if (!numTus) return 0;
+  if (int rc = ensure_device()) return rc;
+  if (int rc = g_hw.init()) return rc;
+  cudaStream_t s = g_hw.stream;
+  IntraLaunch L; L.geom = *g; L.numTus = numTus; memset(&L.planes, 0, sizeof(L.planes));
+  if (int rc = intra_scratch(g, numTus, L)) return rc;
+  if (int rc = g_hw.tus.reserve(numTus * sizeof(b200_intra_tu) + 16)) return rc;
+  B200_CUDA(cudaMemcpyAsync(g_hw.tus.p, tus, numTus * sizeof(b200_intra_tu), cudaMemcpyHostToDevice, s));
+  L.tus = g_hw.tus.as<b200_intra_tu>();
+  B200_CUDA(cudaMemsetAsync(L.sync, 0, (numTus + 2) * sizeof(int), s));
+  if (int rc = launch_intra_prepare(L, nullptr, L.sync + numTus + 1, INTRA_ERR_DEPS, s)) return rc;
+  std::vector<int32_t> h(intra_dep_ints(numTus));
+  int err = 0;
+  B200_CUDA(cudaMemcpyAsync(h.data(), L.deps, h.size() * sizeof(int32_t), cudaMemcpyDeviceToHost, s));
+  B200_CUDA(cudaMemcpyAsync(&err, L.sync + numTus + 1, sizeof(int), cudaMemcpyDeviceToHost, s));
+  B200_CUDA(cudaStreamSynchronize(s));
+  B200_CHECK(!(err & INTRA_ERR_DEPS), "b200_intra_deps: the blocks wait for more than %d earlier blocks each on average (overlapping records?)", INTRA_DEP_SLOTS);
+  const int32_t* range = h.data() + 2; const int32_t* pool = range + 2 * numTus;
+  size_t n = 0;
+  for (size_t i = 0; i < numTus; i++) {
+    counts[i] = range[2 * i + 1];
+    B200_CHECK(n + counts[i] <= capacity, "b200_intra_deps: more than %zu dependencies", capacity);
+    if (counts[i]) memcpy(deps + n, pool + range[2 * i], counts[i] * sizeof(int32_t));
+    n += counts[i];
+  }
   return 0;
 }
 
diff --git a/vvdec_b200/csrc/common.cuh b/vvdec_b200/csrc/common.cuh
--- a/vvdec_b200/csrc/common.cuh
+++ b/vvdec_b200/csrc/common.cuh
@@ -155,8 +155,12 @@
 struct IntraLaunch { b200_geom geom; DevPlanes planes; const int16_t* resi[3]; const b200_intra_tu* tus; size_t numTus; int* owner[3]; int ownerStride[3]; size_t ownerBytes[3]; int* sync;
                      int* order = nullptr;
                      int compSel = 0;
+                     int* deps = nullptr;
+                     bool prepared = false;
                    };
 inline size_t intra_order_ints(const b200_geom& g, size_t numTus) { return numTus + 8 + 3 * (size_t)((g.width + g.ctuSize - 1) / g.ctuSize) * ((g.height + g.ctuSize - 1) / g.ctuSize); }
+constexpr int INTRA_DEP_SLOTS = 16;
+inline size_t intra_dep_ints(size_t numTus) { return 2 + 2 * numTus + (size_t)INTRA_DEP_SLOTS * numTus; }
 inline int intra_ctu_log2(const b200_geom& g) { return g.ctuSize == 128 ? 7 : g.ctuSize == 64 ? 6 : 5; }
 __host__ __device__ inline bool intra_record_in_ctu(const b200_intra_tu& t, int ctuLog2)
 {
@@ -180,7 +184,9 @@
 int launch_intra(const IntraLaunch& L, cudaStream_t s);
 int launch_intra_ciip_clear(const b200_intra_tu* tus, size_t numTus, int16_t* const resi[3], const int stride[3], cudaStream_t s);
 int launch_intra_validate(const b200_intra_tu* tus, size_t numTus, const b200_geom& g, int* meta, cudaStream_t s);
-constexpr int INTRA_ERR_ORDER = 2, INTRA_ERR_CTU_BLOCKS = 4, INTRA_MAX_CTU_BLOCKS = 3072;
+constexpr int INTRA_ERR_ORDER = 2, INTRA_ERR_CTU_BLOCKS = 4, INTRA_ERR_DEPS = 8, INTRA_MAX_CTU_BLOCKS = 3072;
+int launch_intra_prepare(const IntraLaunch& L, const int* skip, int* err, int errBit, cudaStream_t s);
+constexpr int LM_ERR_INTRA_DEPS = 16;
 int launch_film_grain(const DevPlanes& src, const DevPlanes& dst, const b200_geom& g, const int8_t* pattern, const uint8_t* sLUT, const uint8_t* pLUT,
                       const uint32_t* lineSeeds, uint32_t* seeds, int scaleShift, const uint8_t present[3], cudaStream_t s);
 int launch_hash(const DevPlanes& src, const b200_geom& g, int method, uint32_t* acc, uint8_t* digest, cudaStream_t s);
diff --git a/vvdec_b200/csrc/k6_intra.cu b/vvdec_b200/csrc/k6_intra.cu
--- a/vvdec_b200/csrc/k6_intra.cu
+++ b/vvdec_b200/csrc/k6_intra.cu
@@ -24,6 +24,8 @@
   const int* perm;
   int* ctuCnt; int* ctuFirst; int* ctuBase; int ctuLog2, ctusW, ctusH;
   int compSel;
+  int2* depRange; int* depPool; int* depCursor; int depCap;
+  const int* skip; int* depErr; int depErrBit;
 };
 
 __device__ __forceinline__ int wide_angle(int w, int h, int mode)
@@ -40,6 +42,7 @@
 __global__ void __launch_bounds__(256) intra_owner_kernel(const IntraParams P)
 {
   const int i = blockIdx.x;
+  if (P.skip && (*(const volatile int*)P.skip & 8)) return;
   const b200_intra_tu t = P.tus[i];
   const int c = t.comp, unit = c ? 2 : 4, uw = max(1, (1 << t.log2w) / unit), uh = max(1, (1 << t.log2h) / unit);
   for (int k = threadIdx.x; k < uw * uh; k += blockDim.x) atomicMax(&P.owner[c][(t.y / unit + k / uw) * P.ownerStride[c] + t.x / unit + k % uw], i);
@@ -116,67 +119,122 @@
       return PIXR(x0 - 1, y0 + min(i - 1, h - 1)); \
     };
 
+__device__ __forceinline__ void v2_cp4(void* smemDst, const void* gmemSrc)
+{
+  const unsigned d = (unsigned)__cvta_generic_to_shared(smemDst);
+  asm volatile("cp.async.ca.shared.global [%0], [%1], 4;\n" :: "r"(d), "l"(gmemSrc));
+}
+__device__ __forceinline__ void v2_cp16(void* smemDst, const void* gmemSrc)
+{
+  const unsigned d = (unsigned)__cvta_generic_to_shared(smemDst);
+  asm volatile("cp.async.cg.shared.global [%0], [%1], 16;\n" :: "r"(d), "l"(gmemSrc));
+}
+__device__ __forceinline__ void v2_cp_wait() { asm volatile("cp.async.wait_all;\n" ::: "memory"); }
+
+__device__ __forceinline__ void v1_cp8(void* smemDst, const void* gmemSrc)
+{
+  const unsigned d = (unsigned)__cvta_generic_to_shared(smemDst);
+  asm volatile("cp.async.ca.shared.global [%0], [%1], 8;\n" :: "r"(d), "l"(gmemSrc));
+}
+__device__ __forceinline__ int k6_ld_acquire(const int* p) { int v; asm volatile("ld.acquire.gpu.global.b32 %0, [%1];" : "=r"(v) : "l"(p) : "memory"); return v; }
+__device__ __forceinline__ void k6_st_release(int* p, int v) { asm volatile("st.release.gpu.global.b32 [%0], %1;" :: "l"(p), "r"(v) : "memory"); }
+
+constexpr int DEP_THREADS = 128, DEP_CAND = 97 + 34 * 34;
+__global__ void __launch_bounds__(DEP_THREADS) intra_deps_kernel(const IntraParams P)
+{
+  __shared__ int sCand[DEP_CAND]; __shared__ uint8_t sFirst[DEP_CAND]; __shared__ int sN, sD, sOff;
+  const int me = blockIdx.x, tid = threadIdx.x;
+  if (P.skip && (*(const volatile int*)P.skip & 8)) return;
+  const b200_intra_tu t = P.tus[me];
+  const int c = t.comp, w = 1 << t.log2w, h = 1 << t.log2h, unit = c ? 2 : 4, x0 = t.x, y0 = t.y;
+  const int availTL = (t.flags & B200_INTRA_AVAIL_TL) ? 1 : 0, numAbove = t.numAbove, numLeft = t.numLeft;
+  int bx = x0, by = y0, ispK = 0;
+  if (t.flags & B200_INTRA_ISP) { ispK = (t.mip >> 2) & 3; if ((t.mip & 3) == 1) by = y0 - ispK * h; else bx = x0 - ispK * w; }
+  if (tid == 0) { sN = 0; sD = 0; }
+  __syncthreads();
+  auto add = [&](int o) { if (o >= 0 && o < me) sCand[atomicAdd(&sN, 1)] = o; };
+  if (ispK && tid == 0) add(me - 1);
+  for (int dep = tid; dep < 96; dep += DEP_THREADS) {
+    int ux = -1, uy = -1;
+    if (dep == 0) { if (availTL) { ux = bx - 1; uy = by - 1; } }
+    else if (dep <= numAbove) { ux = bx + (dep - 1) * unit; uy = by - 1; }
+    else if (dep - 64 >= 0 && dep - 64 < numLeft) { ux = bx - 1; uy = by + (dep - 64) * unit; }
+    if (ux >= 0 && uy >= 0) add(P.owner[c][(uy / unit) * P.ownerStride[c] + ux / unit]);
+  }
+  if (t.mode >= B200_INTRA_LM) {
+    const bool aCu = t.flags & B200_INTRA_LM_ABOVE, lCu = t.flags & B200_INTRA_LM_LEFT;
+    const int nA = max(w, aCu ? (t.mode == B200_INTRA_MDLM_T ? 2 * t.lmAbove : w) : 0), nL = max(h, lCu ? (t.mode == B200_INTRA_MDLM_L ? 2 * t.lmLeft : h) : 0);
+    const int ux0 = max(0, (2 * x0 - (lCu ? 4 : 0)) >> 2), ux1 = min(P.W - 1, 2 * x0 + 2 * nA - 1) >> 2;
+    const int uy0 = max(0, (2 * y0 - (aCu ? 4 : 0)) >> 2), uy1 = min(P.H - 1, 2 * y0 + 2 * nL - 1) >> 2;
+    const int uw = ux1 - ux0 + 1, nU = uw * (uy1 - uy0 + 1);
+    for (int u = tid; u < nU; u += DEP_THREADS) add(P.owner[0][(uy0 + u / uw) * P.ownerStride[0] + ux0 + u % uw]);
+  }
+  __syncthreads();
+  const int n = sN;
+  for (int i = tid; i < n; i += DEP_THREADS) {
+    const int v = sCand[i]; bool first = true;
+    for (int j = 0; j < i && first; j++) first = sCand[j] != v;
+    sFirst[i] = first;
+    if (first) atomicAdd(&sD, 1);
+  }
+  __syncthreads();
+  const int d = sD;
+  if (tid == 0) {
+    int off = 0;
+    if (d) { off = atomicAdd(P.depCursor, d); if (off + d > P.depCap) { atomicOr(P.depErr, P.depErrBit); off = -1; } }
+    P.depRange[me] = make_int2(max(off, 0), off < 0 ? 0 : d);
+    sOff = off;
+  }
+  __syncthreads();
+  if (sOff < 0) return;
+  for (int i = tid; i < n; i += DEP_THREADS) {
+    if (!sFirst[i]) continue;
+    const int v = sCand[i]; int rank = 0;
+    for (int j = 0; j < n; j++) rank += sFirst[j] && sCand[j] < v;
+    P.depPool[sOff + rank] = v;
+  }
+}
+
 __global__ void __launch_bounds__(IT_THREADS, 12) intra_kernel(const IntraParams P)
 {
   __shared__ int16_t sT[2][IT_REF], sL[2][IT_REF];
   __shared__ int16_t sM[IT_ARR], sS[IT_ARR];
-  __shared__ int sTicket, sSum;
+  __shared__ int sSum;
   __shared__ int16_t sLm[32 * 32], sLmTop[64], sLmLeft[64];
   __shared__ int sLmPar[3];
+  __shared__ __align__(16) b200_intra_tu sRec[2]; __shared__ int2 sRng[2]; __shared__ int sMe[2];
   const int tid = threadIdx.x;
-  for (;;) {
-    __syncthreads();
-    if (tid == 0) { sTicket = atomicAdd(P.ticket, 1); sSum = 0; }
-    __syncthreads();
-    if (sTicket >= P.numTus) return;
-    if (P.perm && (*(volatile int*)P.err & 2)) return;
-    const int me = P.perm ? P.perm[sTicket] : sTicket;
-    const b200_intra_tu t = P.tus[me];
-    if ((P.compSel == 1 && t.comp != 0) || (P.compSel == 2 && t.comp == 0)) continue;
+  if (*(volatile int*)P.err & (INTRA_ERR_ORDER | INTRA_ERR_DEPS)) return;
+  auto fetch = [&](int tk, int slot) {
+    const int m = tk < P.numTus ? (P.perm ? P.perm[tk] : tk) : -1;
+    sMe[slot] = m;
+    if (m >= 0) { v2_cp16(&sRec[slot], P.tus + m); v1_cp8(&sRng[slot], P.depRange + m); }
+  };
+  if (tid == 0) { fetch(atomicAdd(P.ticket, 1), 0); v2_cp_wait(); }
+  __syncthreads();
+  for (int slot = 0;; slot ^= 1) {
+    const int me = sMe[slot];
+    if (me < 0) return;
+    int nTk = 0;
+    const b200_intra_tu t = sRec[slot];
+    const bool run = !((P.compSel == 1 && t.comp != 0) || (P.compSel == 2 && t.comp == 0));
+    if (!run && tid == 0) fetch(atomicAdd(P.ticket, 1), slot ^ 1);
+    if (run) {
+    const int2 rng = sRng[slot];
     const int c = t.comp, w = 1 << t.log2w, h = 1 << t.log2h, mrl = c ? 0 : t.multiRefIdx, unit = c ? 2 : 4;
     const int x0 = t.x, y0 = t.y, ps = P.stride[c], pmax = (1 << P.bitDepth) - 1;
     const int16_t* plane = P.planes[c];
     const int availTL = (t.flags & B200_INTRA_AVAIL_TL) ? 1 : 0, numAbove = t.numAbove, numLeft = t.numLeft;
     ISP_GEOMETRY
 
-    {
-      if (ispK && tid == 0) {
-        const volatile int* d = P.done + me - 1; const volatile int* e = P.err; int spins = 0;
-        while (*d == 0) { __nanosleep(64); if (*e || ++spins > (1 << 22)) { atomicOr(P.err, 1); break; } }
-      }
-      for (int dep = tid; dep < 96; dep += IT_THREADS) {
-      int ux = -1, uy = -1;
-      if (dep == 0) { if (availTL) { ux = bx - 1; uy = by - 1; } }
-      else if (dep <= numAbove) { ux = bx + (dep - 1) * unit; uy = by - 1; }
-      else if (dep - 64 >= 0 && dep - 64 < numLeft) { ux = bx - 1; uy = by + (dep - 64) * unit; }
-      if (ux >= 0 && uy >= 0) {
-        const int o = P.owner[c][(uy / unit) * P.ownerStride[c] + ux / unit];
-        if (o >= 0 && o < me) {
-          const volatile int* d = P.done + o;
-          int spins = 0;
-          const volatile int* e = P.err;
-          while (*d == 0) { __nanosleep(64); if (*e || ++spins > (1 << 22)) { atomicOr(P.err, 1); break; } }
-        }
-      }
-      }
-      if (t.mode >= B200_INTRA_LM) {
-        const bool aCu = t.flags & B200_INTRA_LM_ABOVE, lCu = t.flags & B200_INTRA_LM_LEFT;
-        const int nA = max(w, aCu ? (t.mode == B200_INTRA_MDLM_T ? 2 * t.lmAbove : w) : 0), nL = max(h, lCu ? (t.mode == B200_INTRA_MDLM_L ? 2 * t.lmLeft : h) : 0);
-        const int ux0 = max(0, (2 * x0 - (lCu ? 4 : 0)) >> 2), ux1 = min(P.W - 1, 2 * x0 + 2 * nA - 1) >> 2;
-        const int uy0 = max(0, (2 * y0 - (aCu ? 4 : 0)) >> 2), uy1 = min(P.H - 1, 2 * y0 + 2 * nL - 1) >> 2;
-        const int uw = ux1 - ux0 + 1, nU = uw * (uy1 - uy0 + 1);
-        for (int u = tid; u < nU; u += IT_THREADS) {
-          const int o = P.owner[0][(uy0 + u / uw) * P.ownerStride[0] + ux0 + u % uw];
-          if (o >= 0 && o < me) {
-            const volatile int* d = P.done + o; const volatile int* e = P.err;
-            int spins = 0;
-            while (*d == 0) { __nanosleep(64); if (*e || ++spins > (1 << 22)) { atomicOr(P.err, 1); break; } }
-          }
-        }
-      }
-      __threadfence();
+    if (rng.y) {
+      for (int d = tid; d < rng.y; d += IT_THREADS) {
+        const int* dw = P.done + P.depPool[rng.x + d]; const volatile int* e = P.err; int spins = 0;
+        while (k6_ld_acquire(dw) == 0) { __nanosleep(32); if (*e || ++spins > (1 << 22)) { atomicOr(P.err, 1); break; } }
+      }
+      __syncthreads();
     }
-    __syncthreads();
+    if (tid == 0) { nTk = atomicAdd(P.ticket, 1); sSum = 0; }
 
     const int predSize = 2 * bw, predHSize = 2 * bh;
     const int totalUnits = (predSize + unit - 1) / unit + (predHSize + unit - 1) / unit + 1, n = availTL + numAbove + numLeft;
@@ -184,11 +242,25 @@
     int16_t *T = sT[0], *L = sL[0];
 #define PIXR(x, y) pix(plane, ps, (x), (y))
     ISP_REFERENCE_LAMBDAS
-    for (int j = tid; j <= topLen + mrl; j += IT_THREADS) T[j] = (int16_t)regT(j);
-    for (int i = tid + 1; i <= sideLen + mrl; i += IT_THREADS) L[i] = (int16_t)regL(i);
+    if (!isp && n == totalUnits) {
+      const int16_t* r = plane + (size_t)(by - 1 - mrl) * ps + bx - 1 - mrl;
+      for (int j = tid; j <= max(topLen, sideLen) + mrl; j += IT_THREADS) {
+        const bool doT = j <= topLen + mrl, doL = j <= sideLen + mrl;
+        const int vt = doT ? __ldcg(r + j) : 0, vl = doL ? __ldcg(r + (size_t)j * ps) : 0;
+        if (doT) T[j] = (int16_t)vt;
+        if (doL) L[j] = (int16_t)vl;
+      }
+    } else {
+      for (int j = tid; j <= max(topLen, sideLen) + mrl; j += IT_THREADS) {
+        const bool doT = j <= topLen + mrl, doL = j >= 1 && j <= sideLen + mrl;
+        const int vt = doT ? regT(j) : 0, vl = doL ? regL(j) : 0;
+        if (doT) T[j] = (int16_t)vt;
+        if (doL) L[j] = (int16_t)vl;
+        if (j == 0) L[0] = (int16_t)vt;
+      }
+    }
 #undef PIXR
-    __syncthreads();
-    if (tid == 0) L[0] = T[0];
+    if (tid == 0) fetch(nTk, slot ^ 1);
     __syncthreads();
     if ((t.flags & B200_INTRA_FILTER_REF) && !c && !mrl) {
       int16_t *FT = sT[1], *FL = sL[1];
@@ -363,17 +435,15 @@
       const int invAngle = cInvAng[absMode], absAng = cAng[absMode], angle = angMode < 0 ? -absAng : absAng;
       const int16_t *mainSrc = ver ? T : L, *sideSrc = ver ? L : T;
       const int mw = ver ? w : h, mh = ver ? h : w;
-      int16_t *M = sM + IT_ORG, *S = sS + IT_ORG;
+      const int16_t *Mp, *Sp = sideSrc + mrl;
+      int mEnd;
       if (angle < 0) {
+        int16_t* M = sM + IT_ORG;
         for (int k = tid - mh; k <= mw + 1 + mrl; k += IT_THREADS) M[k] = k >= 0 ? mainSrc[k] : sideSrc[min((-k * invAngle + 256) >> 9, mh)];
-        for (int k = tid; k <= mh + 1 + mrl; k += IT_THREADS) S[k] = sideSrc[k];
-      } else {
-        const int l2r = (31 - __clz(mw)) - (31 - __clz(mh)), s = max(0, l2r), maxIndex = (mrl << s) + 2, refLength = ver ? topLen : sideLen;
-        for (int k = tid; k <= refLength + mrl + maxIndex; k += IT_THREADS) M[k] = mainSrc[min(k, refLength + mrl)];
-        for (int k = tid; k <= (ver ? sideLen : topLen) + mrl; k += IT_THREADS) S[k] = sideSrc[k];
-      }
-      __syncthreads();
-      const int16_t *Mp = M + mrl, *Sp = S + mrl;
+        __syncthreads();
+        Mp = M + mrl; mEnd = 1 << 20;
+      } else { Mp = mainSrc + mrl; mEnd = ver ? topLen : sideLen; }
+#define MAIN(i) Mp[min((i), mEnd)]
       const int l2mw = 31 - __clz(mw), l2mh = 31 - __clz(mh);
       const int topLeft = T[0];
       const int scale0 = (l2mw - 2 + l2mh - 2 + 2) >> 2;
@@ -387,18 +457,18 @@
         const int yy = k >> l2mw, xx = k & (mw - 1);
         int v;
         if (angle == 0) {
-          if (doPDPC && xx < lev) { const int wL = 32 >> min(31, (xx << 1) >> scale0); v = clip3(0, pmax, (wL * (Sp[yy + 1] - topLeft) + Mp[xx + 1] * 64 + 32) >> 6); }
-          else v = Mp[xx + 1];
+          if (doPDPC && xx < lev) { const int wL = 32 >> min(31, (xx << 1) >> scale0); v = clip3(0, pmax, (wL * (Sp[yy + 1] - topLeft) + MAIN(xx + 1) * 64 + 32) >> 6); }
+          else v = MAIN(xx + 1);
         } else {
           const int deltaPos = angle * (1 + mrl + yy), dI = deltaPos >> 5, dF = deltaPos & 31;
-          if (!frac) v = Mp[dI + 1 + xx];
-          else if (c) v = (int16_t)(((32 - dF) * Mp[dI + 1 + xx] + dF * Mp[dI + 2 + xx] + 16) >> 5);
+          if (!frac) v = MAIN(dI + 1 + xx);
+          else if (c) v = (int16_t)(((32 - dF) * MAIN(dI + 1 + xx) + dF * MAIN(dI + 2 + xx) + 16) >> 5);
           else {
-            const int16_t* p = Mp + dI + xx;
+            const int p = dI + xx;
             int f0, f1, f2, f3;
             if (cubic) { f0 = kIfChroma[dF * 4]; f1 = kIfChroma[dF * 4 + 1]; f2 = kIfChroma[dF * 4 + 2]; f3 = kIfChroma[dF * 4 + 3]; }
             else { f0 = 16 - (dF >> 1); f1 = 32 - (dF >> 1); f2 = 16 + (dF >> 1); f3 = dF >> 1; }
-            v = (int16_t)((f0 * p[0] + f1 * p[1] + f2 * p[2] + f3 * p[3] + 32) >> 6);
+            v = (int16_t)((f0 * MAIN(p) + f1 * MAIN(p + 1) + f2 * MAIN(p + 2) + f3 * MAIN(p + 3) + 32) >> 6);
             if (cubic) v = clip3(0, pmax, v);
           }
           if (angularScale >= 0 && xx < min(3 << angularScale, mw)) {
@@ -408,11 +478,13 @@
         }
         if (ver) IT_STORE(xx, yy, v); else IT_STORE(yy, xx, v);
       }
+#undef MAIN
     }
 #undef IT_STORE
-    __threadfence();
+    }
+    if (tid == 0) v2_cp_wait();
     __syncthreads();
-    if (tid == 0) atomicExch(P.done + me, 1);
+    if (run && tid == 0) k6_st_release(P.done + me, 1);
   }
 }
 
@@ -423,20 +495,7 @@
 constexpr int V2_FLAGS = 128 * 128 / 16 + 2 * (64 * 64 / 4);
 static_assert(V2_FLAGS == INTRA_MAX_CTU_BLOCKS, "the documented per-CTU block limit is the number of done bytes");
 struct V2Scratch { int16_t T[2][IT_REF], L[2][IT_REF], M[IT_ARR], S[IT_ARR], Lm[32 * 32], LmTop[64], LmLeft[64]; int LmPar[4]; int next[2], sum; };
-constexpr int V2_OWN = 3 * 32 * 32;
-constexpr size_t v2_smem(int groups) { return (size_t)2 * V2_TILE * sizeof(int16_t) + groups * sizeof(V2Scratch) + V2_RECS * sizeof(b200_intra_tu) + V2_OWN * sizeof(int) + V2_FLAGS + 64; }
-__device__ __forceinline__ void v2_cp4(void* smemDst, const void* gmemSrc)
-{
-  const unsigned d = (unsigned)__cvta_generic_to_shared(smemDst);
-  asm volatile("cp.async.ca.shared.global [%0], [%1], 4;\n" :: "r"(d), "l"(gmemSrc));
-}
-__device__ __forceinline__ void v2_cp16(void* smemDst, const void* gmemSrc)
-{
-  const unsigned d = (unsigned)__cvta_generic_to_shared(smemDst);
-  asm volatile("cp.async.cg.shared.global [%0], [%1], 16;\n" :: "r"(d), "l"(gmemSrc));
-}
-__device__ __forceinline__ void v2_cp_wait() { asm volatile("cp.async.wait_all;\n" ::: "memory"); }
-
+constexpr size_t v2_smem(int groups) { return (size_t)2 * V2_TILE * sizeof(int16_t) + groups * sizeof(V2Scratch) + V2_RECS * (sizeof(b200_intra_tu) + sizeof(int2)) + V2_FLAGS + 64; }
 __device__ __forceinline__ int v2_tile_off(int c) { return c == 0 ? 0 : c == 1 ? 128 * V2_LS : 128 * V2_LS + 64 * V2_CS; }
 
 __global__ void __launch_bounds__(1024) intra_ctu_order_kernel(const IntraParams P, int* ctuOrder, int* counters)
@@ -463,8 +522,6 @@
   if (i == P.ctuFirst[c] && P.ctuCnt[c] > V2_FLAGS) atomicOr(P.err, INTRA_ERR_CTU_BLOCKS);
 }
 
-__device__ __forceinline__ int v2_ld_acquire(const int* p) { int v; asm volatile("ld.acquire.gpu.global.b32 %0, [%1];" : "=r"(v) : "l"(p) : "memory"); return v; }
-__device__ __forceinline__ void v2_st_release(int* p, int v) { asm volatile("st.release.gpu.global.b32 [%0], %1;" :: "l"(p), "r"(v) : "memory"); }
 
 __device__ __forceinline__ void v2_wait(const IntraParams& P, const volatile uint8_t* sflag, int o, int me, int first)
 {
@@ -476,7 +533,7 @@
     return;
   }
   const volatile int* e = P.err;
-  while (v2_ld_acquire(P.done + o) == 0) { __nanosleep(32); if (*e || ++spins > (1 << 22)) { atomicOr(P.err, 1); break; } }
+  while (k6_ld_acquire(P.done + o) == 0) { __nanosleep(32); if (*e || ++spins > (1 << 22)) { atomicOr(P.err, 1); break; } }
 }
 
 #ifdef B200_K6_PROF
@@ -496,8 +553,8 @@
   int16_t* tileRes = tileRec + V2_TILE;
   V2Scratch* scratch = reinterpret_cast<V2Scratch*>(tileRes + V2_TILE);
   b200_intra_tu* srec = reinterpret_cast<b200_intra_tu*>(scratch + V2_GROUPS);
-  int* sown = reinterpret_cast<int*>(srec + V2_RECS);
-  volatile uint8_t* sflag = reinterpret_cast<volatile uint8_t*>(sown + V2_OWN);
+  int* srng = reinterpret_cast<int*>(srec + V2_RECS);
+  volatile uint8_t* sflag = reinterpret_cast<volatile uint8_t*>(srng + 2 * V2_RECS);
   __shared__ int sCtu, sNext;
   const int tid = threadIdx.x, lane = tid & (V2_GROUP - 1), grp = tid / V2_GROUP;
   const int nComp = P.planes[1] ? 3 : 1;
@@ -506,7 +563,7 @@
     __syncthreads();
     if (tid == 0) { sCtu = atomicAdd(&counters[1], 1); sNext = V2_GROUPS; }
     __syncthreads();
-    if (sCtu >= counters[0] || (*(volatile int*)P.err & (INTRA_ERR_ORDER | INTRA_ERR_CTU_BLOCKS))) return;
+    if (sCtu >= counters[0] || (*(volatile int*)P.err & (INTRA_ERR_ORDER | INTRA_ERR_CTU_BLOCKS | INTRA_ERR_DEPS))) return;
     const int ctu = ctuOrder[sCtu], first = P.ctuFirst[ctu], cnt = P.ctuCnt[ctu];
     long long tp = clock64(); (void)tp;
     const int cx = (ctu % P.ctusW) << P.ctuLog2, cy = (ctu / P.ctusW) << P.ctuLog2, cw = min(ctuSize, P.W - cx), ch = min(ctuSize, P.H - cy);
@@ -530,11 +587,9 @@
           if (rsrc) v2_cp4(res + y * ts + x, rsrc + (size_t)y * P.stride[c] + x);
         }
       }
-      const int unit = c ? 2 : 4, uw = tw / unit, uh = th / unit;
-      const int* osrc = P.owner[c] + (size_t)(oy / unit) * P.ownerStride[c] + ox / unit;
-      for (int k = tid; k < uw * uh; k += V2_THREADS) { const int y = k / uw, x = k - y * uw; v2_cp4(sown + c * 1024 + y * 32 + x, osrc + (size_t)y * P.ownerStride[c] + x); }
     }
     for (int k = tid; k < min(cnt, V2_RECS) * 4; k += V2_THREADS) v2_cp4(reinterpret_cast<uint32_t*>(srec) + k, reinterpret_cast<const uint32_t*>(P.tus + first) + k);
+    for (int k = tid; k < min(cnt, V2_RECS) * 2; k += V2_THREADS) v2_cp4(reinterpret_cast<uint32_t*>(srng) + k, reinterpret_cast<const uint32_t*>(P.depRange + first) + k);
     for (int k = tid; k < cnt; k += V2_THREADS) sflag[k] = P.compSel == 2 ? (uint8_t)(P.tus[first + k].comp == 0) : 0;
     v2_cp_wait();
     __syncthreads();
@@ -558,30 +613,8 @@
       auto pixC = [&](int x, int y) -> int {
         return ((unsigned)(x - tox) < (unsigned)ttw && (unsigned)(y - toy) < (unsigned)tth) ? (int)trec[(y - toy) * tts + (x - tox)] : (int)__ldcg(tplane + (size_t)y * ps + x);
       };
-      if (ispK && lane == 0) v2_wait(P, sflag, me - 1, me, first);
-      for (int dep = lane; dep < 96; dep += V2_GROUP) {
-        int ux = -1, uy = -1;
-        if (dep == 0) { if (availTL) { ux = bx - 1; uy = by - 1; } }
-        else if (dep <= numAbove) { ux = bx + (dep - 1) * unit; uy = by - 1; }
-        else if (dep - 64 >= 0 && dep - 64 < numLeft) { ux = bx - 1; uy = by + (dep - 64) * unit; }
-        if (ux >= 0 && uy >= 0) {
-          const int ush = c ? 1 : 2, ox = (ux >> ush) - (tox >> ush), oy = (uy >> ush) - (toy >> ush);
-          const int o = ((unsigned)ox < 32u && (unsigned)oy < 32u && ux < tox + ttw && uy < toy + tth) ? sown[c * 1024 + oy * 32 + ox] : __ldcg(P.owner[c] + (size_t)(uy >> ush) * P.ownerStride[c] + (ux >> ush));
-          v2_wait(P, sflag, o, me, first);
-        }
-      }
-      if (t.mode >= B200_INTRA_LM) {
-        const bool aCu = t.flags & B200_INTRA_LM_ABOVE, lCu = t.flags & B200_INTRA_LM_LEFT;
-        const int nA = max(w, aCu ? (t.mode == B200_INTRA_MDLM_T ? 2 * t.lmAbove : w) : 0), nL = max(h, lCu ? (t.mode == B200_INTRA_MDLM_L ? 2 * t.lmLeft : h) : 0);
-        const int ux0 = max(0, (2 * x0 - (lCu ? 4 : 0)) >> 2), ux1 = min(P.W - 1, 2 * x0 + 2 * nA - 1) >> 2;
-        const int uy0 = max(0, (2 * y0 - (aCu ? 4 : 0)) >> 2), uy1 = min(P.H - 1, 2 * y0 + 2 * nL - 1) >> 2;
-        const int uw = ux1 - ux0 + 1, nU = uw * (uy1 - uy0 + 1);
-        for (int u = lane; u < nU; u += V2_GROUP) {
-          const int gx = ux0 + u % uw, gy = uy0 + u / uw, ox = gx - cx / 4, oy = gy - cy / 4;
-          const int o = ((unsigned)ox < 32u && (unsigned)oy < 32u && gx * 4 < cx + cw && gy * 4 < cy + ch) ? sown[oy * 32 + ox] : __ldcg(P.owner[0] + (size_t)gy * P.ownerStride[0] + gx);
-          v2_wait(P, sflag, o, me, first);
-        }
-      }
+      const int2 rng = k < V2_RECS ? make_int2(srng[2 * k], srng[2 * k + 1]) : P.depRange[me];
+      for (int d = lane; d < rng.y; d += V2_GROUP) v2_wait(P, sflag, P.depPool[rng.x + d], me, first);
       V2_SYNC();
       const int pb = c ? 16 : 0; (void)pb;
       K6P(pb + 1, tp); tp = clock64();
@@ -842,7 +875,7 @@
       if (lane == 0) {
         __threadfence_block();
         sflag[k] = 1;
-        if (x0 + w == tox + ttw || y0 + h == toy + tth) v2_st_release(P.done + me, 1);
+        if (x0 + w == tox + ttw || y0 + h == toy + tth) k6_st_release(P.done + me, 1);
       }
       K6P(pb + 4, tp); K6C(pb + 9); K6P(pb + 10 + min(4, max(0, ((int)t.log2w + (int)t.log2h - 4) >> 1)), tb0);
     }
@@ -913,28 +946,48 @@
 
 constexpr int kWaveCtasPerDiag2 = 6;
 
-int launch_intra(const IntraLaunch& L, cudaStream_t s)
-{
-  if (!L.numTus) return 0;
+static IntraParams intra_params(const IntraLaunch& L)
+{
   IntraParams P;
   for (int c = 0; c < 3; c++) { P.planes[c] = L.planes.p[c]; P.resi[c] = L.resi[c]; P.stride[c] = L.planes.stride[c]; P.owner[c] = L.owner[c]; P.ownerStride[c] = L.ownerStride[c]; }
   if (!L.geom.chromaFormat) { P.planes[1] = P.planes[2] = nullptr; }
   P.W = L.geom.width; P.H = L.geom.height; P.bitDepth = L.geom.bitDepth; P.tus = L.tus; P.numTus = (int)L.numTus;
   P.done = L.sync; P.ticket = L.sync + L.numTus; P.err = L.sync + L.numTus + 1; P.compSel = L.compSel;
+  P.depCursor = L.deps; P.depRange = reinterpret_cast<int2*>(L.deps + 2); P.depPool = L.deps + 2 + 2 * L.numTus; P.depCap = INTRA_DEP_SLOTS * (int)L.numTus;
+  P.perm = nullptr; P.ctuCnt = P.ctuFirst = P.ctuBase = nullptr;
+  P.skip = nullptr; P.depErr = P.err; P.depErrBit = INTRA_ERR_DEPS;
+  return P;
+}
+
+int launch_intra_prepare(const IntraLaunch& L, const int* skip, int* err, int errBit, cudaStream_t s)
+{
+  if (!L.numTus) return 0;
+  IntraParams P = intra_params(L);
+  P.skip = skip; P.depErr = err; P.depErrBit = errBit;
+  B200_CUDA(cudaMemsetAsync(L.deps, 0, 2 * sizeof(int), s));
+  for (int c = 0; c < (L.geom.chromaFormat ? 3 : 1); c++) B200_CUDA(cudaMemsetAsync(L.owner[c], 0xff, L.ownerBytes[c], s));
+  intra_owner_kernel<<<(unsigned)L.numTus, 64, 0, s>>>(P);
+  intra_deps_kernel<<<(unsigned)L.numTus, DEP_THREADS, 0, s>>>(P);
+  B200_CUDA(cudaGetLastError());
+  return 0;
+}
+
+int launch_intra(const IntraLaunch& L, cudaStream_t s)
+{
+  if (!L.numTus) return 0;
+  IntraParams P = intra_params(L);
   const bool cont = L.compSel == 2;
   if (cont) B200_CUDA(cudaMemsetAsync(P.ticket, 0, sizeof(int), s));
   else {
     B200_CUDA(cudaMemsetAsync(L.sync, 0, (L.numTus + 2) * sizeof(int), s));
-    for (int c = 0; c < (L.geom.chromaFormat ? 3 : 1); c++) B200_CUDA(cudaMemsetAsync(L.owner[c], 0xff, L.ownerBytes[c], s));
-  }
-  P.perm = nullptr; P.ctuCnt = P.ctuFirst = P.ctuBase = nullptr;
+    if (!L.prepared) if (int rc = launch_intra_prepare(L, nullptr, P.err, INTRA_ERR_DEPS, s)) return rc;
+  }
   P.ctuLog2 = intra_ctu_log2(L.geom); P.ctusW = (L.geom.width + L.geom.ctuSize - 1) / L.geom.ctuSize; P.ctusH = (L.geom.height + L.geom.ctuSize - 1) / L.geom.ctuSize;
   const char* variant = getenv("B200_INTRA_KERNEL");
   const bool force1 = variant && !strcmp(variant, "v1"), force2 = variant && !strcmp(variant, "v2");
   const bool dense = L.numTus >= 48 * std::max<size_t>(1, (size_t)L.geom.width * L.geom.height >> 14);
   const bool v1 = !L.order || force1 || (!force2 && !dense) || ((P.stride[0] | P.stride[1] | P.stride[2]) & 1);
   const unsigned grid = (unsigned)((L.numTus + 255) / 256);
-  if (!cont) intra_owner_kernel<<<(unsigned)L.numTus, 64, 0, s>>>(P);
   if (!v1) {
     const size_t nCtu = (size_t)P.ctusW * P.ctusH;
     int* base = L.order; P.ctuCnt = base; P.ctuFirst = base + nCtu; int* ctuOrder = base + 2 * nCtu; int* counters = base + 3 * nCtu;
diff --git a/vvdec_b200/csrc/picture.cu b/vvdec_b200/csrc/picture.cu
--- a/vvdec_b200/csrc/picture.cu
+++ b/vvdec_b200/csrc/picture.cu
@@ -18,7 +18,7 @@
   const b200_wp* wp = nullptr;
   const b200_lmcs* lmcs = nullptr; const int16_t* lmcsInv = nullptr; const b200_lmcs_vpdu* lmcsVpdus = nullptr; int* lmcsScale = nullptr; bool lmcsChromaAdj = false;
   int16_t* given[3] = {nullptr, nullptr, nullptr};
-  const b200_intra_tu* intraTus = nullptr; size_t numIntraTus = 0; int* intraOwner[3] = {nullptr, nullptr, nullptr}; int intraOwnerStride[3] = {0, 0, 0}; size_t intraOwnerBytes[3] = {0, 0, 0}; int* intraSync = nullptr; int* intraOrder = nullptr;
+  const b200_intra_tu* intraTus = nullptr; size_t numIntraTus = 0; int* intraOwner[3] = {nullptr, nullptr, nullptr}; int intraOwnerStride[3] = {0, 0, 0}; size_t intraOwnerBytes[3] = {0, 0, 0}; int* intraSync = nullptr; int* intraOrder = nullptr; int* intraDeps = nullptr;
   int dstSlot = 0, flags = 0;
   bool ciipResi = false;
   bool valid = false;
@@ -175,6 +175,7 @@
   const size_t oGiven = take(hasGiven ? c->picBytes : 0);
   size_t oOwn[3] = {0, 0, 0}, ownBytes[3] = {0, 0, 0}; int ownStride[3] = {0, 0, 0};
   const size_t oIntra = take(p->numIntraTus * sizeof(b200_intra_tu)), oSync = take(p->numIntraTus ? (p->numIntraTus + 2) * sizeof(int) : 0), oOrder = take(p->numIntraTus ? intra_order_ints(g, p->numIntraTus) * sizeof(int) : 0);
+  const size_t oDeps = take(p->numIntraTus ? intra_dep_ints(p->numIntraTus) * sizeof(int) : 0);
   for (int k = 0; k < (g.chromaFormat ? 3 : 1) && p->numIntraTus; k++) {
     const int pw = k ? g.width >> 1 : g.width, ph = k ? g.height >> 1 : g.height, unit = k ? 2 : 4;
     ownStride[k] = (pw + unit - 1) / unit; ownBytes[k] = (size_t)ownStride[k] * ((ph + unit - 1) / unit) * sizeof(int); oOwn[k] = take(ownBytes[k]);
@@ -235,7 +236,7 @@
   A.dmvrMv = p->numDmvr ? reinterpret_cast<int32_t*>(base + oDm) : nullptr; A.numDmvr = p->numDmvr;
   if (p->numDmvr) B200_CUDA(cudaMemsetAsync(base + oDm, 0, p->numDmvr * 8, s));
   if (int rc = h2d(oIntra, p->intraTus, p->numIntraTus * sizeof(b200_intra_tu))) return rc;
-  A.intraTus = reinterpret_cast<const b200_intra_tu*>(base + oIntra); A.numIntraTus = p->numIntraTus; A.intraSync = reinterpret_cast<int*>(base + oSync); A.intraOrder = reinterpret_cast<int*>(base + oOrder);
+  A.intraTus = reinterpret_cast<const b200_intra_tu*>(base + oIntra); A.numIntraTus = p->numIntraTus; A.intraSync = reinterpret_cast<int*>(base + oSync); A.intraOrder = reinterpret_cast<int*>(base + oOrder); A.intraDeps = reinterpret_cast<int*>(base + oDeps);
   for (int k = 0; k < 3; k++) { A.intraOwner[k] = ownBytes[k] ? reinterpret_cast<int*>(base + oOwn[k]) : nullptr; A.intraOwnerStride[k] = ownStride[k]; A.intraOwnerBytes[k] = ownBytes[k]; }
   A.ciipResi = false;
   for (size_t i = 0; i < p->numIntraTus && !A.ciipResi; i++) { const b200_intra_tu& t = p->intraTus[i]; A.ciipResi = t.ciip && !(t.flags & B200_INTRA_ISP) && (t.flags & B200_INTRA_ADD_RESI); }
@@ -253,7 +254,13 @@
     if (int rc = launch_ctu_validate((p->flags & B200_PIC_SAO) ? A.sao : nullptr, alfOn ? A.alf : nullptr, (p->flags & B200_PIC_DEBLOCK) ? A.ctuSlice : nullptr, (int)nCtu, lim, A.mcMeta, s)) return rc;
     if (any) c->launches += 1;
   }
-  if (A.numIntraTus) { if (int rc = launch_intra_validate(A.intraTus, A.numIntraTus, g, A.mcMeta, s)) return rc; c->launches += 1; }
+  if (A.numIntraTus) {
+    if (int rc = launch_intra_validate(A.intraTus, A.numIntraTus, g, A.mcMeta, s)) return rc;
+    IntraLaunch L; L.geom = g; L.tus = A.intraTus; L.numTus = A.numIntraTus; L.deps = A.intraDeps;
+    for (int k = 0; k < 3; k++) { L.owner[k] = A.intraOwner[k]; L.ownerStride[k] = A.intraOwnerStride[k]; L.ownerBytes[k] = A.intraOwnerBytes[k]; }
+    if (int rc = launch_intra_prepare(L, A.mcMeta + LM_ERR, A.mcMeta + LM_ERR, LM_ERR_INTRA_DEPS, s)) return rc;
+    c->launches += 3;
+  }
   B200_CUDA(cudaMemcpyAsync(A.hMeta, A.mcMeta, 2 * LM_INTS * sizeof(int), cudaMemcpyDeviceToHost, s));
   B200_CUDA(cudaEventRecord(A.uploaded, s));
   return ai;
@@ -269,6 +276,7 @@
   B200_CHECK(!(A.hMeta[LM_ERR] & 1), "b200_pic_run: the picture's PU list holds an invalid record (reference slots, block size or flag combination)");
   B200_CHECK(!(A.hMeta[LM_ERR] & 2), "b200_pic_run: more MC tiles than the picture can hold (overlapping PUs?)");
   B200_CHECK(!(A.hMeta[LM_ERR] & 8), "b200_pic_run: an intra block record is invalid (geometry, mode, or availability reaching outside the picture)");
+  B200_CHECK(!(A.hMeta[LM_ERR] & LM_ERR_INTRA_DEPS), "b200_pic_run: the intra blocks wait for more than %d earlier blocks each on average (overlapping records?)", INTRA_DEP_SLOTS);
   B200_CHECK(!(A.hMeta[LM_ERR] & 4), "b200_pic_run: a CTU record (SAO type / band, ALF filter index, slice index) is out of range");
   B200_CHECK(!A.hMeta[LM_INTS + LM_ERR], "b200_pic_run: the picture's TU list holds an invalid record");
   B200_CUDA(cudaStreamWaitEvent(s, A.uploaded, 0));
@@ -310,12 +318,12 @@
   };
   auto runK6 = [&](int compSel) -> int {
     if (!A.numIntraTus) return 0;
-    IntraLaunch L; L.geom = g; L.planes = P; L.tus = A.intraTus; L.numTus = A.numIntraTus; L.sync = A.intraSync; L.order = A.intraOrder; L.compSel = compSel;
+    IntraLaunch L; L.geom = g; L.planes = P; L.tus = A.intraTus; L.numTus = A.numIntraTus; L.sync = A.intraSync; L.order = A.intraOrder; L.deps = A.intraDeps; L.prepared = true; L.compSel = compSel;
     for (int k = 0; k < 3; k++) { L.resi[k] = resiPl[k]; L.owner[k] = A.intraOwner[k]; L.ownerStride[k] = A.intraOwnerStride[k]; L.ownerBytes[k] = A.intraOwnerBytes[k]; }
     if (c->profiling) c->prof.begin(B200_KF_INTRA, s);
     if (int rc = launch_intra(L, s)) return rc;
     if (c->profiling) c->prof.end(B200_KF_INTRA, s);
-    c->launches += compSel == 2 ? 1 : 5;
+    c->launches += compSel == 2 ? 1 : 4;
     return 0;
   };
   if (twoPass) {
```

After: 1213, median of 6. 1.07x the previous value.
